# IBM/TM-GCN

Measured on AMD Instinct MI355X. Metric: TM-GCN layer fwd+bwd throughput (edges x T)/s, higher is better.
Workload: dtype f32

## Files before the change

include/tmgcn.h:

```cpp
#ifndef TMGCN_H
#define TMGCN_H

#include <stdint.h>

#ifdef __cplusplus
extern "C" {
#endif

typedef enum {
  TMGCN_OK = 0,
  TMGCN_ERR_INVALID = -1,
  TMGCN_ERR_LAUNCH = -2,
  TMGCN_ERR_WORKSPACE = -3
} tmgcn_status;

enum { TMGCN_ACT_NONE = 0, TMGCN_ACT_RELU = 1, TMGCN_ACT_LEAKY = 2, TMGCN_ACT_SELU = 3 };

int tmgcn_abi_version(void);
const char* tmgcn_last_error(void);
int tmgcn_pool_stats(int64_t* out, int32_t n);

enum {
  TMGCN_GEMM_AUTO = 0,
  TMGCN_GEMM_F32MFMA = 1
};

enum {
  TMGCN_DW_AUTO = 0,
  TMGCN_DW_F32MFMA = 1
};

int tmgcn_mtransform_f32(const float* M, int32_t Tm, int32_t ldm, int32_t transpose,
                         int32_t row_off, int32_t col_off, int32_t T_out, int32_t T_in,
                         int32_t band_lo, int32_t band_hi,
                         const float* X, float* Y, int64_t C,
                         int32_t x_group_rows, int32_t y_group_rows, void* stream);
int tmgcn_mtransform_ld_f32(const float* M, int32_t Tm, int32_t ldm, int32_t transpose,
                            int32_t row_off, int32_t col_off, int32_t T_out, int32_t T_in,
                            int32_t band_lo, int32_t band_hi,
                            const float* X, int64_t ldx, float* Y, int64_t ldy, int64_t C,
                            int32_t x_group_rows, int32_t y_group_rows, void* stream);

#define TMGCN_GIANT_ROW 32768
#define TMGCN_GIANT_CHUNK 4096
int64_t tmgcn_spmm_giant_workspace_bytes(int32_t n_giant_chunks, int32_t F);
int tmgcn_spmm_csr_batched_f32(const int64_t* rowptr, const int32_t* col, const float* val,
                               const float* X, float* Y, int64_t n_rows, int32_t N, int32_t F,
                               void* stream);
int tmgcn_spmm_csr_batched_f32_hint(const int64_t* rowptr, const int32_t* col, const float* val,
                                    const float* X, float* Y, int64_t n_rows, int32_t N,
                                    int32_t F, float avg_nnz_per_row, void* stream);
int tmgcn_spmm_csr_batched_f32_plan(const int64_t* rowptr, const int32_t* col, const float* val,
                                    const float* X, float* Y, int64_t n_rows, int32_t N,
                                    int32_t F, float avg_nnz_per_row, const int64_t* giant_rows,
                                    const int32_t* giant_chunks, int32_t n_giant, int32_t n_giant_chunks,
                                    float* giant_ws, int64_t giant_ws_bytes, void* stream);

int tmgcn_spmm_gemm_supported(int32_t K, int32_t Nf);
int tmgcn_spmm_gemm_f32(const int64_t* rowptr, const int32_t* col, const float* val,
                        const float* X, int64_t n_rows, int32_t N, int32_t K,
                        const float* W, int32_t Nf, int32_t trans_w,
                        int64_t rows_per_batch, int64_t w_batch_stride, int32_t act,
                        float* Y, float* AX, float* pre_act, int32_t grid_reserve, void* stream);
int tmgcn_spmm_gemm_f32_hint(const int64_t* rowptr, const int32_t* col, const float* val,
                             const float* X, int64_t n_rows, int32_t N, int32_t K,
                             const float* W, int32_t Nf, int32_t trans_w,
                             int64_t rows_per_batch, int64_t w_batch_stride, int32_t act,
                             float* Y, float* AX, float* pre_act, int32_t grid_reserve,
                             float avg_nnz_per_row, void* stream);
int tmgcn_spmm_gemm_f32_plan(const int64_t* rowptr, const int32_t* col, const float* val,
                             const float* X, int64_t n_rows, int32_t N, int32_t K,
                             const float* W, int32_t Nf, int32_t trans_w,
                             int64_t rows_per_batch, int64_t w_batch_stride, int32_t act,
                             float* Y, float* AX, float* pre_act, int32_t grid_reserve,
                             float avg_nnz_per_row, const int64_t* giant_rows, const int32_t* giant_chunks,
                             int32_t n_giant, int32_t n_giant_chunks, float* giant_ws, int64_t giant_ws_bytes,
                             void* stream);

int tmgcn_spmm_gemm_bf16_supported(int32_t K, int32_t Nf);
int tmgcn_spmm_gemm_bf16(const int64_t* rowptr, const int32_t* col, const float* val,
                         const uint16_t* X_bf16, int64_t n_rows, int32_t N, int32_t K,
                         const float* W, int32_t Nf, int32_t trans_w,
                         int64_t rows_per_batch, int64_t w_batch_stride, int32_t act,
                         void* Y, int32_t y_bf16, float* AX, float* pre_act, int32_t grid_reserve,
                         float avg_nnz_per_row, void* stream);

int tmgcn_gemm_f32(const float* A, const float* W, float* Y, float* pre_act,
                   int64_t R, int32_t K, int32_t Nf, int32_t trans_w,
                   int64_t rows_per_batch, int64_t w_batch_stride, int32_t act, int32_t algo, void* stream);

int tmgcn_gemm_bf16w_f32(const float* A, const uint16_t* W_bf16, float* Y, float* pre_act,
                         int64_t R, int32_t K, int32_t Nf, int32_t trans_w,
                         int64_t rows_per_batch, int64_t w_batch_stride, int32_t act, int32_t algo,
                         void* stream);

int64_t tmgcn_gemm_dw_workspace_bytes(int64_t R, int32_t K, int32_t Nf, int64_t rows_per_batch);
int tmgcn_gemm_dw_f32(const float* A, const float* dY, float* dW,
                      int64_t R, int32_t K, int32_t Nf, int64_t rows_per_batch, int32_t algo,
                      void* workspace, int64_t workspace_bytes, void* stream);
int tmgcn_gemm_dw_act_supported(int32_t K, int32_t Nf);
int tmgcn_gemm_dw_act_f32(const float* A, const float* dY, const float* pre_act, int32_t act, float* dW,
                          int64_t R, int32_t K, int32_t Nf, int64_t rows_per_batch,
                          void* workspace, int64_t workspace_bytes, void* stream);

#define TMGCN_L12_RUNS 16
int tmgcn_layer12_supported(int32_t K0, int32_t F, int32_t Nf);
int tmgcn_layer12_fwd_f32(const int64_t* rowptr, const int32_t* col, const float* val, const float* H,
                          const float* W1, int32_t act1, const float* W2, int32_t act2, int64_t n_rows,
                          int32_t N, int32_t K0, int32_t F, int32_t Nf, float* Z, float* AX, float* pre2,
                          float avg_nnz_per_row, const int64_t* row_blocks, int32_t n_row_blocks, void* stream);
int tmgcn_layer12_fwd_pays(int64_t n_rows, int32_t N, int32_t F, float avg_nnz_per_row);
int64_t tmgcn_layer12_bwd_workspace_bytes(int32_t K0, int32_t F, int32_t Nf, int64_t n_rows, int32_t n_row_blocks);
int tmgcn_layer12_bwd_forms_dw2(int64_t n_rows, int32_t N, int32_t F, int32_t Nf, float avg_nnz_per_row, int32_t n_row_blocks);
int tmgcn_layer12_bwd_f32(const int64_t* t_rowptr, const int32_t* t_col, const float* t_val, const float* dZ,
                          const float* pre2, const float* H, const float* W1, int32_t act1, const float* W2,
                          int32_t act2, int64_t n_rows, int32_t N, int32_t K0, int32_t F, int32_t Nf,
                          float* dW1, const float* AX, float* dW2, float avg_nnz_per_row, const int64_t* row_blocks,
                          int32_t n_row_blocks, void* workspace, int64_t workspace_bytes, void* stream);

int tmgcn_act_fwd_f32(const float* x, float* y, int64_t n, int32_t act, void* stream);
int tmgcn_act_bwd_f32(const float* x, const float* dy, float* dx, int64_t n, int32_t act,
                      void* stream);

int tmgcn_edge_head_supported(int32_t F, int32_t C);
int tmgcn_edge_head_fwd_f32(const float* Z, const int64_t* src, const int64_t* dst,
                            const float* U, float* out, int64_t E, int32_t F, int32_t C,
                            void* stream);
int64_t tmgcn_edge_head_bwd_workspace_bytes(int64_t E, int32_t F, int32_t C);
int tmgcn_edge_head_bwd_f32(const float* Z, const int64_t* src, const int64_t* dst,
                            const float* U, const float* dout,
                            const int64_t* eptr, const int64_t* eidx,
                            float* dZ, float* dU, int64_t R, int64_t E, int32_t F, int32_t C,
                            void* workspace, int64_t workspace_bytes, void* stream);
int tmgcn_edge_head_fwd_i32_f32(const float* Z, const int32_t* src, const int32_t* dst,
                                const float* U, float* out, int64_t E, int32_t F, int32_t C,
                                void* stream);
int tmgcn_edge_head_bwd_i32_f32(const float* Z, const int32_t* src, const int32_t* dst,
                                const float* U, const float* dout,
                                const int32_t* eptr, const int32_t* eidx,
                                float* dZ, float* dU, int64_t R, int64_t E, int32_t F, int32_t C,
                                void* workspace, int64_t workspace_bytes, void* stream);

int64_t tmgcn_wce_workspace_bytes(int64_t E);
int tmgcn_wce_fwd_f32(const float* logits, const int64_t* target, const float* weight, int64_t E,
                      int32_t C, int64_t ignore_index, float* loss_out, double* stats_out, void* workspace,
                      int64_t workspace_bytes, void* stream);
int tmgcn_wce_bwd_f32(const float* logits, const int64_t* target, const float* weight,
                      const double* stats, const float* grad_loss, int64_t E, int32_t C,
                      int64_t ignore_index, float* dlogits, void* stream);

#define TMGCN_SYNC_INTS 272
int tmgcn_head_loss_supported(int32_t F, int32_t C, int32_t K);
int tmgcn_head_loss_lanes(int64_t E, int64_t n_active);
int tmgcn_head_loss_combine_f32(const int32_t* srow, int32_t n_split, float* dZ, int64_t R, int32_t F, void* stream);
int64_t tmgcn_head_loss_workspace_bytes(int32_t F, int32_t C, int32_t K);
int tmgcn_head_loss_f32(const float* Z, const float* W_fold, int32_t K, const float* U,
                        const int32_t* eptr, const int32_t* arow, int64_t n_active, const int32_t* ent,
                        const int32_t* other, const uint8_t* meta, const int64_t* class_count,
                        const float* weight, const float* grad_scale, int64_t R, int64_t E, int32_t F,
                        int32_t C, float* logits, float* loss, float* dZ, float* dU, float* dW,
                        void* workspace, int64_t workspace_bytes, int32_t* sync, void* stream);
typedef struct TmgcnSgd {
  float* buf_U;
  float* buf_W;
  float lr, momentum, dampening, weight_decay;
  int32_t nesterov, maximize, first_step;
} TmgcnSgd;
int tmgcn_head_loss_sgd_f32(const float* Z, float* W_fold, int32_t K, float* U, const int32_t* eptr, const int32_t* arow,
                            int64_t n_active, const int32_t* other, const uint8_t* meta, const int64_t* class_count,
                            const float* weight, int64_t R, int64_t E, int32_t F, int32_t C, float* loss, float* dU,
                            float* dW, const TmgcnSgd* sgd, void* workspace, int64_t workspace_bytes, int32_t* sync,
                            void* stream);

int tmgcn_sgd_step(void* const* params, const void* const* grads, void* const* momentum_bufs, const int64_t* numel,
                   int32_t n, int32_t bf16, float lr, float momentum, float dampening, float weight_decay,
                   int32_t nesterov, int32_t maximize, int32_t first_step, void* stream);
int tmgcn_cast_multi(const void* const* src, void* const* dst, const int64_t* numel, int32_t n, int32_t to_bf16,
                     void* stream);
int tmgcn_scale2_f32(const float* g, const float* a, float* out_a, int64_t na, const float* b, float* out_b,
                     int64_t nb, void* stream);

int tmgcn_adj_make_keys(const int64_t* slice, const int64_t* row, const int64_t* col, int64_t n,
                        int64_t N, uint64_t* key, void* stream);
int64_t tmgcn_coo_sort_reduce_workspace_bytes(int64_t n);
int tmgcn_coo_sort_reduce(const uint64_t* keys_in, const float* vals_in, int64_t n, int32_t key_bits,
                          uint64_t* keys_out, float* vals_out, int64_t* n_out_dev,
                          void* workspace, int64_t workspace_bytes, void* stream);
int tmgcn_adj_symmetrise(const uint64_t* key, const float* val, int64_t n, int64_t N,
                         uint64_t* okey, float* oval, void* stream);
int tmgcn_adj_edge_life(const uint64_t* key, const float* val, int64_t n, int64_t N, int32_t T,
                        int32_t window, uint64_t* okey, float* oval, void* stream);
int tmgcn_adj_identity(int64_t TN, int64_t N, uint64_t* okey, float* oval, void* stream);
int tmgcn_adj_normalise(const uint64_t* key, float* val, int64_t n, int64_t N, int64_t TN,
                        int64_t* rowptr, float* dinv, void* stream);
int tmgcn_adj_mproduct_expand(const uint64_t* key, const float* val, int64_t n, int64_t N, int32_t T,
                              const float* M, int32_t ldm, int32_t band_lo, int32_t band_hi,
                              uint64_t* okey, float* oval, void* stream);
int tmgcn_adj_mproduct_merge_count(const int64_t* rowptr, const int32_t* col, int64_t TN, int32_t N, int32_t T,
                                   const float* M, int32_t ldm, int32_t band_lo, int32_t band_hi,
                                   int64_t* out_count, void* stream);
int tmgcn_adj_mproduct_merge_fill(const int64_t* rowptr, const int32_t* col, const float* val, int64_t TN,
                                  int32_t N, int32_t T, const float* M, int32_t ldm, int32_t band_lo,
                                  int32_t band_hi, const int64_t* out_rowptr, int32_t* out_col, float* out_val,
                                  void* stream);
int tmgcn_adj_keys_to_csr(const uint64_t* key, int64_t n, int64_t N, int64_t TN, int64_t* rowptr,
                          int32_t* col, void* stream);
int tmgcn_adj_transpose_keys(const int64_t* rowptr, const int32_t* col, int64_t TN, int64_t N,
                             uint64_t* okey, void* stream);

int tmgcn_wdgcn_supported(int32_t F0, int32_t H);
int64_t tmgcn_wdgcn_param_count(int32_t F0, int32_t H);
int tmgcn_wdgcn_fwd_f32(const float* AX, const float* P, const float* h0, const float* c0, float* Z, float* C,
                        int64_t N, int32_t T_run, int32_t F0, int32_t H, void* stream);
int64_t tmgcn_wdgcn_bwd_workspace_bytes(int64_t N, int32_t F0, int32_t H);
int tmgcn_wdgcn_bwd_f32(const float* AX, const float* P, const float* h0, const float* c0, const float* Z,
                        const float* C, const float* dZ, float* dP, int64_t N, int32_t T_run, int32_t F0,
                        int32_t H, void* workspace, int64_t workspace_bytes, void* stream);

int tmgcn_wdgcn_wide_supported(int32_t F0, int32_t H);
int64_t tmgcn_wdgcn_wide_saved_bytes(int64_t N, int32_t T_run, int32_t F0, int32_t H);
int tmgcn_wdgcn_wide_fwd_f32(const float* AX, const float* P, const float* h0, const float* c0, float* Z, void* saved,
                             int64_t N, int32_t T_run, int32_t F0, int32_t H, void* stream);
int64_t tmgcn_wdgcn_wide_bwd_workspace_bytes(int64_t N, int32_t T_run, int32_t F0, int32_t H);
int tmgcn_wdgcn_wide_bwd_f32(const float* AX, const float* P, const float* h0, const float* c0, const float* Z,
                             const void* saved, const float* dZ, float* dP, int64_t N, int32_t T_run, int32_t F0,
                             int32_t H, void* workspace, int64_t workspace_bytes, void* stream);

int tmgcn_egcn_supported(int32_t F, int32_t k);
int64_t tmgcn_egcn_param_count(int32_t F, int32_t k);
int64_t tmgcn_egcn_fwd_workspace_bytes(int64_t N, int32_t T_run, int32_t F, int32_t k);
// ... 27 lines not shown
```

tm-gcn_amd/_lib.py:

```python
import ctypes as C
import os

_HERE = os.path.dirname(os.path.abspath(__file__))
LIB_PATH = os.path.join(_HERE, "libtmgcn_hip.so")
HEADER_PATH = os.path.join(os.path.dirname(_HERE), "include", "tmgcn.h")

ACT_IDS = {None: 0, "none": 0, "relu": 1, "leaky": 2, "selu": 3}
DW_ALGOS = {None: 0, "auto": 0, "f32mfma": 1}
GEMM_ALGOS = {None: 0, "auto": 0, "f32mfma": 1}
ABI_VERSION = 5
SYNC_INTS = 272


class TmgcnLibraryError(RuntimeError):
    pass


_p = C.c_void_p
_i32 = C.c_int32
_i64 = C.c_int64

SIGNATURES = {
    "tmgcn_abi_version": (C.c_int, []),
    "tmgcn_last_error": (C.c_char_p, []),
    "tmgcn_pool_stats": (C.c_int, [_p, _i32]),
    "tmgcn_mtransform_f32": (C.c_int, [_p, _i32, _i32, _i32, _i32, _i32, _i32, _i32, _i32, _i32, _p, _p, _i64, _i32, _i32, _p]),
    "tmgcn_mtransform_ld_f32": (C.c_int, [_p, _i32, _i32, _i32, _i32, _i32, _i32, _i32, _i32, _i32, _p, _i64, _p, _i64, _i64, _i32, _i32, _p]),
    "tmgcn_spmm_csr_batched_f32": (C.c_int, [_p, _p, _p, _p, _p, _i64, _i32, _i32, _p]),
    "tmgcn_spmm_csr_batched_f32_hint": (C.c_int, [_p, _p, _p, _p, _p, _i64, _i32, _i32, C.c_float, _p]),
    "tmgcn_spmm_giant_workspace_bytes": (_i64, [_i32, _i32]),
    "tmgcn_spmm_csr_batched_f32_plan": (C.c_int, [_p, _p, _p, _p, _p, _i64, _i32, _i32, C.c_float, _p, _p, _i32, _i32, _p, _i64, _p]),
    "tmgcn_spmm_gemm_f32_plan": (C.c_int, [_p, _p, _p, _p, _i64, _i32, _i32, _p, _i32, _i32, _i64, _i64, _i32, _p, _p, _p, _i32, C.c_float,
                                           _p, _p, _i32, _i32, _p, _i64, _p]),
    "tmgcn_spmm_gemm_supported": (C.c_int, [_i32, _i32]),
    "tmgcn_spmm_gemm_f32": (C.c_int, [_p, _p, _p, _p, _i64, _i32, _i32, _p, _i32, _i32, _i64, _i64, _i32, _p, _p, _p, _i32, _p]),
    "tmgcn_spmm_gemm_f32_hint": (C.c_int, [_p, _p, _p, _p, _i64, _i32, _i32, _p, _i32, _i32, _i64, _i64, _i32, _p, _p, _p, _i32, C.c_float, _p]),
    "tmgcn_spmm_gemm_bf16_supported": (C.c_int, [_i32, _i32]),
    "tmgcn_spmm_gemm_bf16": (C.c_int, [_p, _p, _p, _p, _i64, _i32, _i32, _p, _i32, _i32, _i64, _i64, _i32, _p, _i32, _p, _p, _i32,
                                       C.c_float, _p]),
    "tmgcn_gemm_f32": (C.c_int, [_p, _p, _p, _p, _i64, _i32, _i32, _i32, _i64, _i64, _i32, _i32, _p]),
    "tmgcn_gemm_bf16w_f32": (C.c_int, [_p, _p, _p, _p, _i64, _i32, _i32, _i32, _i64, _i64, _i32, _i32, _p]),
    "tmgcn_gemm_dw_workspace_bytes": (_i64, [_i64, _i32, _i32, _i64]),
    "tmgcn_gemm_dw_f32": (C.c_int, [_p, _p, _p, _i64, _i32, _i32, _i64, _i32, _p, _i64, _p]),
    "tmgcn_gemm_dw_act_supported": (C.c_int, [_i32, _i32]),
    "tmgcn_gemm_dw_act_f32": (C.c_int, [_p, _p, _p, _i32, _p, _i64, _i32, _i32, _i64, _p, _i64, _p]),
    "tmgcn_layer12_supported": (C.c_int, [_i32, _i32, _i32]),
    "tmgcn_layer12_fwd_f32": (C.c_int, [_p, _p, _p, _p, _p, _i32, _p, _i32, _i64, _i32, _i32, _i32, _i32, _p, _p, _p, C.c_float, _p, _i32, _p]),
    "tmgcn_layer12_fwd_pays": (C.c_int, [_i64, _i32, _i32, C.c_float]),
    "tmgcn_layer12_bwd_workspace_bytes": (_i64, [_i32, _i32, _i32, _i64, _i32]),
    "tmgcn_layer12_bwd_forms_dw2": (C.c_int, [_i64, _i32, _i32, _i32, C.c_float, _i32]),
    "tmgcn_layer12_bwd_f32": (C.c_int, [_p, _p, _p, _p, _p, _p, _p, _i32, _p, _i32, _i64, _i32, _i32, _i32, _i32, _p, _p, _p, C.c_float, _p, _i32, _p, _i64, _p]),
    "tmgcn_edge_head_supported": (C.c_int, [_i32, _i32]),
    "tmgcn_edge_head_fwd_f32": (C.c_int, [_p, _p, _p, _p, _p, _i64, _i32, _i32, _p]),
    "tmgcn_edge_head_bwd_workspace_bytes": (_i64, [_i64, _i32, _i32]),
    "tmgcn_edge_head_bwd_f32": (C.c_int, [_p, _p, _p, _p, _p, _p, _p, _p, _p, _i64, _i64, _i32, _i32, _p, _i64, _p]),
    "tmgcn_edge_head_fwd_i32_f32": (C.c_int, [_p, _p, _p, _p, _p, _i64, _i32, _i32, _p]),
    "tmgcn_edge_head_bwd_i32_f32": (C.c_int, [_p, _p, _p, _p, _p, _p, _p, _p, _p, _i64, _i64, _i32, _i32, _p, _i64, _p]),
    "tmgcn_wce_workspace_bytes": (_i64, [_i64]),
    "tmgcn_wce_fwd_f32": (C.c_int, [_p, _p, _p, _i64, _i32, _i64, _p, _p, _p, _i64, _p]),
    "tmgcn_wce_bwd_f32": (C.c_int, [_p, _p, _p, _p, _p, _i64, _i32, _i64, _p, _p]),
    "tmgcn_head_loss_supported": (C.c_int, [_i32, _i32, _i32]),
    "tmgcn_head_loss_combine_f32": (C.c_int, [_p, _i32, _p, _i64, _i32, _p]),
    "tmgcn_head_loss_lanes": (C.c_int, [_i64, _i64]),
    "tmgcn_head_loss_workspace_bytes": (_i64, [_i32, _i32, _i32]),
    "tmgcn_head_loss_sgd_f32": (C.c_int, [_p, _p, _i32, _p, _p, _p, _i64, _p, _p, _p, _p, _i64, _i64, _i32, _i32, _p, _p, _p, _p, _p, _i64, _p, _p]),
    "tmgcn_head_loss_f32": (C.c_int, [_p, _p, _i32, _p, _p, _p, _i64, _p, _p, _p, _p, _p, _p, _i64, _i64, _i32, _i32, _p, _p, _p, _p, _p, _p, _i64, _p, _p]),
    "tmgcn_sgd_step": (C.c_int, [_p, _p, _p, _p, _i32, _i32, C.c_float, C.c_float, C.c_float, C.c_float, _i32, _i32, _i32, _p]),
    "tmgcn_cast_multi": (C.c_int, [_p, _p, _p, _i32, _i32, _p]),
    "tmgcn_scale2_f32": (C.c_int, [_p, _p, _p, _i64, _p, _p, _i64, _p]),
    "tmgcn_adj_make_keys": (C.c_int, [_p, _p, _p, _i64, _i64, _p, _p]),
    "tmgcn_coo_sort_reduce_workspace_bytes": (_i64, [_i64]),
    "tmgcn_coo_sort_reduce": (C.c_int, [_p, _p, _i64, _i32, _p, _p, _p, _p, _i64, _p]),
    "tmgcn_adj_symmetrise": (C.c_int, [_p, _p, _i64, _i64, _p, _p, _p]),
    "tmgcn_adj_edge_life": (C.c_int, [_p, _p, _i64, _i64, _i32, _i32, _p, _p, _p]),
    "tmgcn_adj_identity": (C.c_int, [_i64, _i64, _p, _p, _p]),
    "tmgcn_adj_normalise": (C.c_int, [_p, _p, _i64, _i64, _i64, _p, _p, _p]),
    "tmgcn_adj_mproduct_expand": (C.c_int, [_p, _p, _i64, _i64, _i32, _p, _i32, _i32, _i32, _p, _p, _p]),
    "tmgcn_adj_mproduct_merge_count": (C.c_int, [_p, _p, _i64, _i32, _i32, _p, _i32, _i32, _i32, _p, _p]),
    "tmgcn_adj_mproduct_merge_fill": (C.c_int, [_p, _p, _p, _i64, _i32, _i32, _p, _i32, _i32, _i32, _p, _p, _p, _p]),
    "tmgcn_adj_keys_to_csr": (C.c_int, [_p, _i64, _i64, _i64, _p, _p, _p]),
    "tmgcn_adj_transpose_keys": (C.c_int, [_p, _p, _i64, _i64, _p, _p]),
    "tmgcn_act_fwd_f32": (C.c_int, [_p, _p, _i64, _i32, _p]),
    "tmgcn_act_bwd_f32": (C.c_int, [_p, _p, _p, _i64, _i32, _p]),
    "tmgcn_wdgcn_supported": (C.c_int, [_i32, _i32]),
    "tmgcn_wdgcn_param_count": (_i64, [_i32, _i32]),
    "tmgcn_wdgcn_fwd_f32": (C.c_int, [_p, _p, _p, _p, _p, _p, _i64, _i32, _i32, _i32, _p]),
    "tmgcn_wdgcn_bwd_workspace_bytes": (_i64, [_i64, _i32, _i32]),
    "tmgcn_wdgcn_bwd_f32": (C.c_int, [_p, _p, _p, _p, _p, _p, _p, _p, _i64, _i32, _i32, _i32, _p, _i64, _p]),
    "tmgcn_wdgcn_wide_supported": (C.c_int, [_i32, _i32]),
    "tmgcn_wdgcn_wide_saved_bytes": (_i64, [_i64, _i32, _i32, _i32]),
    "tmgcn_wdgcn_wide_fwd_f32": (C.c_int, [_p, _p, _p, _p, _p, _p, _i64, _i32, _i32, _i32, _p]),
    "tmgcn_wdgcn_wide_bwd_workspace_bytes": (_i64, [_i64, _i32, _i32, _i32]),
    "tmgcn_wdgcn_wide_bwd_f32": (C.c_int, [_p, _p, _p, _p, _p, _p, _p, _p, _i64, _i32, _i32, _i32, _p, _i64, _p]),
    "tmgcn_egcn_supported": (C.c_int, [_i32, _i32]),
    "tmgcn_egcn_param_count": (_i64, [_i32, _i32]),
    "tmgcn_egcn_fwd_workspace_bytes": (_i64, [_i64, _i32, _i32, _i32]),
    "tmgcn_egcn_fwd": (C.c_int, [_p, _p, _p, _p, _p, _p, _p, _p, _i32, _p, _p, _p, _p, _p, _p, _p, _i64, _i32, _i32, _i32,
                                 _p, _i64, _p]),
    "tmgcn_egcn_bwd_workspace_bytes": (_i64, [_i32, _i32, _i32]),
    "tmgcn_egcn_bwd": (C.c_int, [_p, _p, _p, _p, _p, _p, _p, _p, _p, _p, _p, _p, _i64, _i32, _i32, _i32, _p, _i64, _p]),
    "tmgcn_egcn_wide_supported": (C.c_int, [_i32, _i32]),
    "tmgcn_egcn_wide_fwd_workspace_bytes": (_i64, [_i64, _i32, _i32, _i32]),
    "tmgcn_egcn_wide_fwd": (C.c_int, [_p, _p, _p, _p, _p, _p, _p, _p, _i32, _p, _p, _p, _p, _p, _p, _p, _i64, _i32, _i32,
                                      _i32, _p, _i64, _p]),
    "tmgcn_egcn_wide_bwd_workspace_bytes": (_i64, [_i32, _i32, _i32]),
    "tmgcn_egcn_wide_bwd": (C.c_int, [_p, _p, _p, _p, _p, _p, _p, _p, _p, _p, _p, _p, _i64, _i32, _i32, _i32, _p, _i64,
                                      _p]),
}

_lib = None


def load():
    global _lib
    if _lib is not None:
        return _lib
    if not os.path.exists(LIB_PATH):
        raise TmgcnLibraryError(
            f"{LIB_PATH} not found: build the HIP library first "
            "(make -C tm-gcn_amd/csrc, or __graft_entry__.build()). "
            "There is no CPU fallback for the TM-GCN layer."
        )
    try:
        lib = C.CDLL(LIB_PATH)
    except OSError as e:
        raise TmgcnLibraryError(f"cannot load {LIB_PATH}: {e}") from e
    for name, (res, args) in SIGNATURES.items():
        try:
            fn = getattr(lib, name)
        except AttributeError as e:
            raise TmgcnLibraryError(f"{LIB_PATH} does not export {name}") from e
        fn.restype = res
        fn.argtypes = args
    _lib = lib
    return lib


TORCH_LIB_PATH = os.path.join(_HERE, "libtmgcn_torch.so")
_torch_ops = None


def load_torch_ops():
    global _torch_ops
    if _torch_ops is not None:
        return _torch_ops
    load()
    if not os.path.exists(TORCH_LIB_PATH):
        raise TmgcnLibraryError(
            f"{TORCH_LIB_PATH} not found: build the torch extension layer first "
            "(make -C tm-gcn_amd/csrc torch, or __graft_entry__.build()).")
    import torch
    try:
        torch.ops.load_library(TORCH_LIB_PATH)
    except OSError as e:
        raise TmgcnLibraryError(f"cannot load {TORCH_LIB_PATH}: {e}") from e
    ops = torch.ops.tmgcn
    if int(ops.abi_version()) != ABI_VERSION:
        raise TmgcnLibraryError(f"{TORCH_LIB_PATH} was built against ABI {int(ops.abi_version())}, expected {ABI_VERSION}")
    _torch_ops = ops
    return ops


def check(rc, what):
    if rc != 0:
        msg = load().tmgcn_last_error().decode("utf-8", "replace")
        raise RuntimeError(f"{what} failed (status {rc}): {msg}")
```

tm-gcn_amd/csrc/common.h:

```cpp
#pragma once
#include <hip/hip_runtime.h>
#include <stdint.h>
#include <stdio.h>
#include <type_traits>
#include "tmgcn.h"

namespace tmgcn {

void set_error(const char* fmt, ...);

inline int check_launch(const char* what) {
  hipError_t e = hipGetLastError();
  if (e != hipSuccess) {
    set_error("%s: %s", what, hipGetErrorString(e));
    return TMGCN_ERR_LAUNCH;
  }
  return TMGCN_OK;
}

const char* pool_error();
unsigned int* acquire_tile_counters(hipStream_t stream, int n);
inline unsigned int* acquire_tile_counter(hipStream_t stream) { return acquire_tile_counters(stream, 1); }

int32_t* acquire_sync_word(hipStream_t stream);

constexpr int kSyncGroups = 16, kSyncStride = 16;
constexpr int kSyncInts = (1 + kSyncGroups) * kSyncStride;
static_assert(kSyncInts == TMGCN_SYNC_INTS, "include/tmgcn.h states the size of a hand-off block");
__device__ __forceinline__ bool last_block_ticket(int32_t* sync, int n_blocks, int* lds_flag) {
  asm volatile("s_waitcnt vmcnt(0)" ::: "memory");
  __syncthreads();
  if (threadIdx.x == 0) {
    const int g = blockIdx.x % kSyncGroups;
    const int members = (n_blocks - g + kSyncGroups - 1) / kSyncGroups;
    int32_t* mine = sync + (1 + g) * kSyncStride;
    bool last = false;
    if (__hip_atomic_fetch_add(mine, 1, __ATOMIC_RELAXED, __HIP_MEMORY_SCOPE_AGENT) == members - 1) {
      __hip_atomic_store(mine, 0, __ATOMIC_RELAXED, __HIP_MEMORY_SCOPE_AGENT);
      const int groups = n_blocks < kSyncGroups ? n_blocks : kSyncGroups;
      last = __hip_atomic_fetch_add(sync, 1, __ATOMIC_RELAXED, __HIP_MEMORY_SCOPE_AGENT) == groups - 1;
    }
    *lds_flag = last;
  }
  __syncthreads();
  return *lds_flag != 0;
}

int launch_giant_partial(const char* who, const int64_t* rowptr, const int32_t* col, const float* val, const float* X, int32_t N,
                         int32_t F, const int64_t* giant_rows, const int32_t* giant_chunks, int32_t n_giant, int32_t n_giant_chunks,
                         float* ws, int64_t ws_bytes, hipStream_t st);

#define TMGCN_REQUIRE(cond, ...)            \
  do {                                      \
    if (!(cond)) {                          \
      ::tmgcn::set_error(__VA_ARGS__);      \
      return TMGCN_ERR_INVALID;             \
    }                                       \
  } while (0)

constexpr int kWave = 64;


inline int device_cu_count(int dev) {
  thread_local int cus[16] = {0};
  if (dev >= 0 && dev < 16 && cus[dev]) return cus[dev];
  int n = 0;
  if (hipDeviceGetAttribute(&n, hipDeviceAttributeMultiprocessorCount, dev) != hipSuccess || n <= 0) n = 256;
  if (dev >= 0 && dev < 16) cus[dev] = n;
  return n;
}

template <typename K>
inline int persistent_grid(K kernel, int block_threads, size_t dyn_smem = 0, int max_per_cu = 4) {
  struct Entry { const void* k; int dev, threads, blocks_per_cu; };
  constexpr int kSlots = 16;
  thread_local Entry table[kSlots] = {};
  thread_local int next = 0;
  const void* key = reinterpret_cast<const void*>(kernel);
  int dev = 0;
  if (hipGetDevice(&dev) != hipSuccess) dev = 0;
  const int cus = device_cu_count(dev);
  if (dyn_smem == 0)
    for (int i = 0; i < kSlots; ++i)
      if (table[i].k == key && table[i].dev == dev && table[i].threads == block_threads)
        return cus * table[i].blocks_per_cu;
  int per_cu = 1;
  if (hipOccupancyMaxActiveBlocksPerMultiprocessor(&per_cu, kernel, block_threads, dyn_smem) != hipSuccess ||
      per_cu < 1)
    per_cu = 1;
  if (per_cu > max_per_cu) per_cu = max_per_cu;
  (void)hipGetLastError();
  if (dyn_smem == 0) {
    table[next] = Entry{key, dev, block_threads, per_cu};
    next = (next + 1) % kSlots;
  }
  return cus * per_cu;
}

template <typename K>
inline int persistent_grid_reserved(K kernel, int block_threads, int reserve, size_t dyn_smem = 0) {
  int g = persistent_grid(kernel, block_threads, dyn_smem) - reserve;
  return g < 64 ? 64 : g;
}

inline int check_workspace(const char* who, const void* workspace, int64_t bytes, int64_t need) {
  if (workspace && bytes >= need) return TMGCN_OK;
  set_error("%s: workspace of %lld bytes, %lld needed", who, (long long)bytes, (long long)need);
  return TMGCN_ERR_WORKSPACE;
}

template <typename K>
inline int allow_large_lds(K kernel, size_t bytes, const char* what) {
  if (bytes <= 64 * 1024) return TMGCN_OK;
  struct Entry { const void* k; int dev; size_t bytes; };
  constexpr int kSlots = 32;
  thread_local Entry table[kSlots] = {};
  thread_local int next = 0;
  const void* key = reinterpret_cast<const void*>(kernel);
  int dev = 0;
  if (hipGetDevice(&dev) != hipSuccess) dev = 0;
  Entry* e = nullptr;
  for (int i = 0; i < kSlots && !e; ++i)
    if (table[i].k == key && table[i].dev == dev) e = &table[i];
  if (e && e->bytes >= bytes) return TMGCN_OK;
  if (hipFuncSetAttribute(key, hipFuncAttributeMaxDynamicSharedMemorySize, (int)bytes) != hipSuccess) {
    (void)hipGetLastError();
    set_error("%s: %zu bytes of LDS per block refused", what, bytes);
    return TMGCN_ERR_LAUNCH;
  }
  if (!e) {
    e = &table[next];
    next = (next + 1) % kSlots;
  }
  *e = Entry{key, dev, bytes};
  return TMGCN_OK;
}

__device__ __forceinline__ void quad_transpose4(float (&v)[4], int j) {
  const bool odd = j & 1, hi = j & 2;
  {
    const float s0 = odd ? v[0] : v[1], s1 = odd ? v[2] : v[3];
    const float r0 = __builtin_bit_cast(float, __builtin_amdgcn_mov_dpp(__builtin_bit_cast(int, s0), 0xB1, 0xF, 0xF, true));
    const float r1 = __builtin_bit_cast(float, __builtin_amdgcn_mov_dpp(__builtin_bit_cast(int, s1), 0xB1, 0xF, 0xF, true));
    if (odd) {
      v[0] = r0;
      v[2] = r1;
    } else {
      v[1] = r0;
      v[3] = r1;
    }
  }
  {
    const float s0 = hi ? v[0] : v[2], s1 = hi ? v[1] : v[3];
    const float r0 = __builtin_bit_cast(float, __builtin_amdgcn_mov_dpp(__builtin_bit_cast(int, s0), 0x4E, 0xF, 0xF, true));
    const float r1 = __builtin_bit_cast(float, __builtin_amdgcn_mov_dpp(__builtin_bit_cast(int, s1), 0x4E, 0xF, 0xF, true));
    if (hi) {
      v[0] = r0;
      v[1] = r1;
    } else {
      v[2] = r0;
      v[3] = r1;
    }
  }
}

__device__ __forceinline__ int64_t readlane64(int64_t v, int l) {
  const unsigned lo = (unsigned)__builtin_amdgcn_readlane((int)(unsigned)(v & 0xffffffff), l);
  const int hi = __builtin_amdgcn_readlane((int)(v >> 32), l);
  return ((int64_t)hi << 32) | lo;
}

template <int N, typename T>
__device__ __forceinline__ T pick(const T (&v)[N], int i) {
  T r = v[0];
#pragma unroll
  for (int q = 1; q < N; ++q) r = (i == q) ? v[q] : r;
  return r;
}

template <int CTRL>
__device__ __forceinline__ float dpp_lane_f32(float v) {
  return __builtin_bit_cast(float, __builtin_amdgcn_mov_dpp(__builtin_bit_cast(int, v), CTRL, 0xF, 0xF, true));
}
__device__ __forceinline__ float wave_sum_f32(float v) {
  v += dpp_lane_f32<0xB1>(v);
  v += dpp_lane_f32<0x4E>(v);
  v += dpp_lane_f32<0x141>(v);
  v += dpp_lane_f32<0x140>(v);
  const float r0 = __builtin_bit_cast(float, __builtin_amdgcn_readlane(__builtin_bit_cast(int, v), 0));
  const float r1 = __builtin_bit_cast(float, __builtin_amdgcn_readlane(__builtin_bit_cast(int, v), 16));
  const float r2 = __builtin_bit_cast(float, __builtin_amdgcn_readlane(__builtin_bit_cast(int, v), 32));
  const float r3 = __builtin_bit_cast(float, __builtin_amdgcn_readlane(__builtin_bit_cast(int, v), 48));
  return ((r0 + r1) + r2) + r3;
}

template <int CTRL>
__device__ __forceinline__ double dpp_add_f64(double x) {
  const long long b = __builtin_bit_cast(long long, x);
  const int lo = __builtin_amdgcn_mov_dpp((int)b, CTRL, 0xF, 0xF, true);
// ... 214 lines not shown
```

tm-gcn_amd/csrc/gemm.hip:

```cpp
#include <type_traits>
#include "common.h"
#include "async_stage.h"

namespace tmgcn {

typedef float f32x16 __attribute__((ext_vector_type(16)));
typedef float f32x4 __attribute__((ext_vector_type(4)));

constexpr int BM = 64;
constexpr int KC = 128;
constexpr int LDA = KC + 4;

struct GemmArgs {
  const float* A;
  const float* W;
  float* Y;
  float* pre;
  int64_t R;
  int32_t K, Nf;
  int32_t trans_w;
  int64_t rows_per_batch;
  int64_t w_batch_stride;
  int32_t act;
  int64_t tiles_per_batch;
// ... 1104 lines not shown
  const bool x3 = algo == TMGCN_GEMM_AUTO && K % 4 == 0 && K >= 16 && K <= 128 &&
                  reinterpret_cast<uintptr_t>(A) % 16 == 0;
  const bool x3_chunked = algo == TMGCN_GEMM_AUTO && K % 4 == 0 && K > 128 && K <= 512 &&
                          reinterpret_cast<uintptr_t>(A) % 16 == 0;
  if (x3_chunked) {
    int64_t gx = w_bf16 ? persistent_grid(gemm_bf16x3_kernel<1, true>, 256) : persistent_grid(gemm_bf16x3_kernel<3, true>, 256);
    if (gx > a.n_tiles) gx = a.n_tiles;
    for (int k0 = 0; k0 < K; k0 += 128) {
      GemmArgs c = a;
      const bool last = k0 + 128 >= K;
      c.K = last ? K - k0 : 128;
      c.lda = K;
      c.k0 = k0;
      c.accum = k0 > 0;
      c.act = last ? act : TMGCN_ACT_NONE;
      c.pre = last ? pre_act : nullptr;
      if (w_bf16)
        hipLaunchKernelGGL((gemm_bf16x3_kernel<1, true>), dim3((unsigned)gx, gy), dim3(256), 0, st, c);
      else
        hipLaunchKernelGGL((gemm_bf16x3_kernel<3, true>), dim3((unsigned)gx, gy), dim3(256), 0, st, c);
    }
    return check_launch("gemm_bf16x3 (k-chunks)");
  }
  if (x3) {
    int64_t gx = w_bf16 ? persistent_grid(gemm_bf16x3_kernel<1>, 256) : persistent_grid(gemm_bf16x3_kernel<3>, 256);
    if (gx > a.n_tiles) gx = a.n_tiles;
    if (w_bf16)
      hipLaunchKernelGGL(gemm_bf16x3_kernel<1>, dim3((unsigned)gx, gy), dim3(256), 0, st, a);
    else
      hipLaunchKernelGGL(gemm_bf16x3_kernel<3>, dim3((unsigned)gx, gy), dim3(256), 0, st, a);
    return check_launch("gemm_bf16x3");
  }
  a.tile_counter = acquire_tile_counters(st, (int)gy);
  TMGCN_REQUIRE(a.tile_counter, "gemm: no tile counters: %s", pool_error());
  int64_t gx = persistent_grid(gemm_mfma_kernel, 256);
  if (gx > a.n_tiles) gx = a.n_tiles;
  hipLaunchKernelGGL(gemm_mfma_kernel, dim3((unsigned)gx, gy), dim3(256), 0, st, a);
  return check_launch("gemm_mfma");
}

extern "C" int tmgcn_gemm_f32(const float* A, const float* W, float* Y, float* pre_act, int64_t R,
                               int32_t K, int32_t Nf, int32_t trans_w, int64_t rows_per_batch,
                               int64_t w_batch_stride, int32_t act, int32_t algo, void* stream) {
  return gemm_launch(A, W, false, Y, pre_act, R, K, Nf, trans_w, rows_per_batch, w_batch_stride, act, algo, stream);
}

extern "C" int tmgcn_gemm_bf16w_f32(const float* A, const uint16_t* W_bf16, float* Y, float* pre_act, int64_t R,
                                     int32_t K, int32_t Nf, int32_t trans_w, int64_t rows_per_batch,
                                     int64_t w_batch_stride, int32_t act, int32_t algo, void* stream) {
  return gemm_launch(A, W_bf16, true, Y, pre_act, R, K, Nf, trans_w, rows_per_batch, w_batch_stride, act, algo,
                     stream);
}

extern "C" int64_t tmgcn_gemm_dw_workspace_bytes(int64_t R, int32_t K, int32_t Nf,
                                                  int64_t rows_per_batch) {
  if (R <= 0 || K <= 0 || Nf <= 0) return 0;
  int64_t nb, rpc;
  int chunks;
  dw_plan(R, rows_per_batch, &nb, &chunks, &rpc);
  return (nb * chunks + kSyncGroups) * (int64_t)K * Nf * (int64_t)sizeof(float);
}

static int gemm_dw_launch(const float* A, const float* dY, const float* pre, int32_t act, float* dW, int64_t R, int32_t K,
                          int32_t Nf, int64_t rows_per_batch, int32_t algo, void* workspace, int64_t workspace_bytes,
                          void* stream) {
  TMGCN_REQUIRE(R >= 0 && K > 0 && Nf > 0, "gemm_dw: bad shape");
  TMGCN_REQUIRE(algo == TMGCN_DW_AUTO || algo == TMGCN_DW_F32MFMA, "gemm_dw: unknown algo %d", algo);
  TMGCN_REQUIRE(rows_per_batch >= 0, "gemm_dw: negative rows_per_batch");
  TMGCN_REQUIRE(dW, "gemm_dw: null dW");
  hipStream_t st = (hipStream_t)stream;
  int64_t nb, rpc;
  int chunks;
  dw_plan(R, rows_per_batch, &nb, &chunks, &rpc);
  if (R == 0) {
    (void)hipMemsetAsync(dW, 0, (size_t)K * Nf * sizeof(float), st);
    return check_launch("gemm_dw memset");
  }
  TMGCN_REQUIRE(A && dY, "gemm_dw: null pointer");
  const int64_t need = (nb * chunks + kSyncGroups) * (int64_t)K * Nf * (int64_t)sizeof(float);
  if (!workspace || workspace_bytes < need) {
    set_error("gemm_dw: workspace %lld B < required %lld B", (long long)workspace_bytes,
              (long long)need);
    return TMGCN_ERR_WORKSPACE;
  }
  const bool narrow = K % 2 == 0 && Nf % 2 == 0 && K <= 8 && Nf <= 8 && reinterpret_cast<uintptr_t>(A) % 8 == 0 &&
                      reinterpret_cast<uintptr_t>(dY) % 8 == 0;
  TMGCN_REQUIRE(!pre || narrow, "gemm_dw_act: the fused activation gradient needs the narrow kernel (even K, Nf <= 8, 8-byte "
                                 "aligned operands); use tmgcn_act_bwd_f32 + tmgcn_gemm_dw_f32");
  if (narrow) {
    const int64_t br = rows_per_batch ? rows_per_batch : R;
    int64_t target = (R < (4ll << 20) ? 512 : 1024) / nb;
    if (target < 1) target = 1;
    int64_t fat = (br + target - 1) / target;
    fat = (fat + 31) & ~(int64_t)31;
    if (fat < 256) fat = 256;
    if (fat > rpc) {
      rpc = fat;
      chunks = (int)((br + rpc - 1) / rpc);
    }
  }
  DwArgs a{A, dY, (float*)workspace, R, K, Nf, rows_per_batch ? rows_per_batch : R, chunks, rpc};
  const unsigned gx = (unsigned)(nb * chunks);
  if (narrow) {
    a.dW = dW;
    a.pre = pre;
    a.act = act;
    a.n_batch = (int32_t)nb;
    a.sync = acquire_sync_word(st);
    TMGCN_REQUIRE(a.sync, "gemm_dw: no hand-off block: %s", pool_error());
#define TMGCN_DWN_L(KT_, NT_)                                                                          \
  if (pre) hipLaunchKernelGGL((gemm_dw_narrow_kernel<KT_, NT_, true>), dim3(gx), dim3(256), 0, st, a); \
  else hipLaunchKernelGGL((gemm_dw_narrow_kernel<KT_, NT_, false>), dim3(gx), dim3(256), 0, st, a);
#define TMGCN_DWN_N(KT_)                \
  switch (Nf) {                         \
    case 2: TMGCN_DWN_L(KT_, 2) break;  \
    case 4: TMGCN_DWN_L(KT_, 4) break;  \
    case 6: TMGCN_DWN_L(KT_, 6) break;  \
    default: TMGCN_DWN_L(KT_, 8)        \
  }
    switch (K) {
      case 2: TMGCN_DWN_N(2) break;
      case 4: TMGCN_DWN_N(4) break;
      case 6: TMGCN_DWN_N(6) break;
      default: TMGCN_DWN_N(8)
    }
#undef TMGCN_DWN_N
#undef TMGCN_DWN_L
    return check_launch("gemm_dw_narrow");
  } else if (use_small(K, Nf)) {
    const size_t smem = (size_t)DW_ROWS * (K + Nf) * sizeof(float);
    hipLaunchKernelGGL(gemm_dw_small_kernel, dim3(gx), dim3(256), smem, st, a);
  } else {
    const unsigned gy = (unsigned)(((K + 127) / 128) * ((Nf + 127) / 128));
    const bool x3 = algo == TMGCN_DW_AUTO && K % 4 == 0 && Nf % 4 == 0 &&
                    reinterpret_cast<uintptr_t>(A) % 16 == 0 && reinterpret_cast<uintptr_t>(dY) % 16 == 0;
    if (x3)
      hipLaunchKernelGGL(gemm_dw_bf16x3_kernel, dim3(gx, gy), dim3(256), 0, st, a);
    else
      hipLaunchKernelGGL(gemm_dw_lds_kernel, dim3(gx, gy), dim3(256), 0, st, a);
  }
  int rc = check_launch("gemm_dw");
  if (rc) return rc;
  const int64_t n_out = (int64_t)K * Nf;
  const int64_t total = nb * n_out;
  if (total <= 1024 && chunks >= 64)
    hipLaunchKernelGGL(gemm_dw_reduce_narrow_kernel, dim3((unsigned)total), dim3(256), 0, st, (const float*)workspace,
                       dW, n_out, chunks);
  else
    hipLaunchKernelGGL(gemm_dw_reduce_kernel, dim3((unsigned)((total + 63) / 64)), dim3(DWR_WAVES * 64), 0, st,
                       (const float*)workspace, dW, n_out, chunks, total);
  return check_launch("gemm_dw_reduce");
}

extern "C" int tmgcn_gemm_dw_f32(const float* A, const float* dY, float* dW, int64_t R, int32_t K, int32_t Nf,
                                  int64_t rows_per_batch, int32_t algo, void* workspace, int64_t workspace_bytes,
                                  void* stream) {
  return gemm_dw_launch(A, dY, nullptr, TMGCN_ACT_NONE, dW, R, K, Nf, rows_per_batch, algo, workspace, workspace_bytes, stream);
}

extern "C" int tmgcn_gemm_dw_act_supported(int32_t K, int32_t Nf) {
  return (K >= 2 && Nf >= 2 && K % 2 == 0 && Nf % 2 == 0 && K <= 8 && Nf <= 8) ? 1 : 0;
}

extern "C" int tmgcn_gemm_dw_act_f32(const float* A, const float* dY, const float* pre_act, int32_t act, float* dW,
                                      int64_t R, int32_t K, int32_t Nf, int64_t rows_per_batch, void* workspace,
                                      int64_t workspace_bytes, void* stream) {
  TMGCN_REQUIRE(tmgcn_gemm_dw_act_supported(K, Nf), "gemm_dw_act: even K, Nf <= 8 only (got %d x %d)", K, Nf);
  TMGCN_REQUIRE(act >= TMGCN_ACT_NONE && act <= TMGCN_ACT_SELU, "gemm_dw_act: unknown activation %d", act);
  TMGCN_REQUIRE(pre_act && reinterpret_cast<uintptr_t>(pre_act) % 8 == 0, "gemm_dw_act: pre_act must be given, 8-byte aligned");
  return gemm_dw_launch(A, dY, pre_act, act, dW, R, K, Nf, rows_per_batch, TMGCN_DW_AUTO, workspace, workspace_bytes, stream);
}
```

tm-gcn_amd/csrc/spmm_gemm.hip:

```cpp
#include "common.h"
#include "spmm_row.h"
#include "spmm_gemm_tile.h"

namespace tmgcn {

#ifndef TMGCN_FUSED_US
#define TMGCN_FUSED_US 1
#endif
#ifndef TMGCN_BX3_US
#define TMGCN_BX3_US 4
#endif
#ifndef TMGCN_BX3_MAX_DEG
#define TMGCN_BX3_MAX_DEG 14
#endif

struct FusedArgs {
  const int64_t* rowptr;
  const int32_t* col;
  const float* val;
  const float4* X;
  int64_t n_rows;
  int32_t N;
  int32_t K;
  const float* W;
  int32_t Nf;
  int32_t trans_w;
  int64_t rows_per_batch;
  int64_t w_batch_stride;
  float* Y;
  float* AX;
  float* pre;
  int32_t act;
  TileMap tiles;
  int64_t n_tiles;
  unsigned int* tile_counter;
  GiantPlan giant;
};

#ifdef TMGCN_FUSED_TRACE
__device__ unsigned long long fused_trace_words[4096 * 16];
#define FT_WORDS fused_trace_words
#else
#define FT_WORDS nullptr
#endif

template <int LPR, int U, int NJ, int US = TMGCN_FUSED_US * U>
__global__ __launch_bounds__(256, TMGCN_FUSED_OCC) void spmm_gemm_kernel(FusedArgs a) {
  __shared__ float As[FBM * FLDA];
  __shared__ float4 s_part[4 * LPR];
  __shared__ unsigned int s_tile, s_row;
  fused_tile_loop<FusedF32, LPR, U, NJ, US, false>(a, As, s_part, &s_tile, &s_row, FT_WORDS);
}


typedef __bf16 bx_bf16x8 __attribute__((ext_vector_type(8)));
typedef __bf16 bx_bf16x2 __attribute__((ext_vector_type(2)));
typedef float bx_f32x2 __attribute__((ext_vector_type(2)));
typedef float bx_f32x4 __attribute__((ext_vector_type(4)));
constexpr int BX_PITCH = 272;
constexpr int BX_PLANE = FBM * BX_PITCH;
constexpr int BX_YPITCH = 132;

__device__ __forceinline__ unsigned bx_pack(float a, float b) {
  bx_f32x2 v = {a, b};
  return __builtin_bit_cast(unsigned, __builtin_convertvector(v, bx_bf16x2));
}
__device__ __forceinline__ void bx_split3(float a, float b, unsigned& h, unsigned& m, unsigned& l) {
  h = bx_pack(a, b);
  a -= __uint_as_float(h << 16);
  b -= __uint_as_float(h & 0xffff0000u);
  m = bx_pack(a, b);
  a -= __uint_as_float(m << 16);
  b -= __uint_as_float(m & 0xffff0000u);
  l = bx_pack(a, b);
}

template <int LPR, int U, int NKS, int US>
__global__ __launch_bounds__(512, 4) void spmm_gemm_bx3_kernel(FusedArgs a) {
  __shared__ __attribute__((aligned(16))) unsigned char sm[3 * BX_PLANE];
  __shared__ float4 s_part[4 * LPR];
  __shared__ unsigned int s_tile, s_row;
  const int lane0 = threadIdx.x & 63;
  const int wave = __builtin_amdgcn_readfirstlane(threadIdx.x >> 6);
  const int n0 = wave * 16;
  const int F4 = a.K / 4;
  const TileMap tm = a.tiles;
  unsigned bw[NKS][3][4];
  int64_t cur_batch = -1;
  if (threadIdx.x == 0) s_row = 8;
  const bool staged = a.Nf % 4 == 0 && reinterpret_cast<uintptr_t>(a.Y) % 16 == 0 && reinterpret_cast<uintptr_t>(a.pre) % 16 == 0;
  HeavyScan heavy;
  heavy.init(a.rowptr, tm);
  bool have_next = false;
  for (;;) {
    int lane = lane0;
    asm volatile("" : "+v"(lane));
    int64_t tile = -1;
    if (heavy.scanning) tile = heavy.next(a.rowptr, tm, a.tile_counter + 1, &s_tile, lane);
    const bool scanning = heavy.scanning;
    if (!scanning) {
      if (!have_next) {
        if (threadIdx.x == 0) s_tile = atomicAdd(a.tile_counter, 1u);
        __syncthreads();
      }
      tile = s_tile;
      have_next = false;
      if (tile >= a.n_tiles) break;
    }
    int64_t unit, row0, row_end;
    tile_extent(tm, tile, unit, row0, row_end);
    const int64_t batch = a.rows_per_batch ? row0 / a.rows_per_batch : 0;
    TileRows rows;
    rows.load(a.rowptr, row0, row_end, lane);
    if (!scanning && rows.entries > heavy.thr) {
      __syncthreads();
      continue;
    }
    const int n_tile_rows = row_end - row0 < FBM ? (int)(row_end - row0) : FBM;
    const int64_t slice0 = row0 / a.N;
    const float4* Xs = a.X + slice0 * (int64_t)a.N * F4;
    auto flush = [&](int rr, const float4& acc, int fl) __attribute__((always_inline)) {
      if (fl < F4) {
        unsigned h0, m0, l0, h1, m1, l1;
        bx_split3(acc.x, acc.y, h0, m0, l0);
        bx_split3(acc.z, acc.w, h1, m1, l1);
        unsigned char* w = sm + rr * BX_PITCH + fl * 8;
        *reinterpret_cast<uint2*>(w) = make_uint2(h0, h1);
        *reinterpret_cast<uint2*>(w + BX_PLANE) = make_uint2(m0, m1);
        *reinterpret_cast<uint2*>(w + 2 * BX_PLANE) = make_uint2(l0, l1);
        if (a.AX && rr < n_tile_rows) store_f4(&reinterpret_cast<float4*>(a.AX)[(row0 + rr) * F4 + fl], acc);
      }
    };
    if (short_tile(rows, row0 + n_tile_rows <= (slice0 + 1) * a.N)) {
      gather_short_tile<LPR, US, 8>(a.col, a.val, Xs, rows, n_tile_rows, F4, lane, wave, F4, flush);
    } else {
      for (int rr = wave; rr < FBM;) {
        unsigned int nxt = 0;
        if (lane == 0) nxt = atomicAdd(&s_row, 1u);
        const bool lng = (rows.long_mask >> rr) & 1;
        if (!lng) {
          float4 acc = make_float4(0.f, 0.f, 0.f, 0.f);
          if (rr < n_tile_rows) acc = gather_row<LPR, U>(a.col, a.val, Xs, readlane64(rows.beg, rr), readlane64(rows.end, rr), F4, lane);
          if (lane < LPR) flush(rr, acc, lane);
        }
        rr = (int)__builtin_amdgcn_readfirstlane(nxt);
      }
      for (uint64_t m = rows.long_mask; m; m &= m - 1) {
        const int rr = __builtin_ctzll(m);
        const int64_t beg = readlane64(rows.beg, rr), end = readlane64(rows.end, rr);
        if (wave < 4) {
          const float4 acc = gather_long_row<LPR, U>(a.col, a.val, Xs, beg, end, F4, lane, wave, s_part);
          if (wave == (rr & 3) && lane < LPR) flush(rr, acc, lane);
        } else {
          __syncthreads();
          __syncthreads();
        }
      }
    }
    if (batch != cur_batch) {
      const float* Wb = a.W + (a.rows_per_batch ? batch * a.w_batch_stride : 0);
      const int n = n0 + (lane & 15);
      const int nc = n < a.Nf ? n : 0;
      const float zn = n < a.Nf ? 1.f : 0.f;
      const int64_t sk = a.trans_w ? 1 : a.Nf, sn = a.trans_w ? a.K : 1;
      const float* Wl = Wb + (int64_t)nc * sn + (int64_t)(8 * (lane >> 4)) * sk;
#pragma unroll
      for (int ks = 0; ks < NKS; ++ks)
#pragma unroll
        for (int j = 0; j < 4; ++j) {
          const float w0 = Wl[(int64_t)(32 * ks + 2 * j) * sk] * zn;
          const float w1 = Wl[(int64_t)(32 * ks + 2 * j + 1) * sk] * zn;
          bx_split3(w0, w1, bw[ks][0][j], bw[ks][1][j], bw[ks][2][j]);
        }
      cur_batch = batch;
    }
    __syncthreads();
    if (threadIdx.x == 0) s_row = 8;
    unsigned int drawn = 0;
    if (!scanning && threadIdx.x == 0) drawn = atomicAdd(a.tile_counter, 1u);
    __builtin_amdgcn_s_setprio(TMGCN_FUSED_MFMA_PRIO);
    int lane_p = lane0;
    asm volatile("" : "+v"(lane_p));
    const int lm = lane_p & 15, lg = lane_p >> 4;
    bx_f32x4 acc[4];
#pragma unroll
    for (int rb = 0; rb < 4; ++rb) acc[rb] = bx_f32x4{0.f, 0.f, 0.f, 0.f};
    if (n0 < a.Nf) {
      const unsigned char* rd = sm + lm * BX_PITCH + lg * 16;
#pragma unroll
      for (int ks = 0; ks < NKS; ++ks) {
        const bx_bf16x8 bh = __builtin_bit_cast(bx_bf16x8, make_uint4(bw[ks][0][0], bw[ks][0][1], bw[ks][0][2], bw[ks][0][3]));
        const bx_bf16x8 bm = __builtin_bit_cast(bx_bf16x8, make_uint4(bw[ks][1][0], bw[ks][1][1], bw[ks][1][2], bw[ks][1][3]));
        const bx_bf16x8 bl = __builtin_bit_cast(bx_bf16x8, make_uint4(bw[ks][2][0], bw[ks][2][1], bw[ks][2][2], bw[ks][2][3]));
#pragma unroll
        for (int rb = 0; rb < 4; ++rb) {
          const unsigned char* p = rd + rb * 16 * BX_PITCH + ks * 64;
          const bx_bf16x8 ah = __builtin_bit_cast(bx_bf16x8, *reinterpret_cast<const uint4*>(p));
          const bx_bf16x8 am = __builtin_bit_cast(bx_bf16x8, *reinterpret_cast<const uint4*>(p + BX_PLANE));
          const bx_bf16x8 al = __builtin_bit_cast(bx_bf16x8, *reinterpret_cast<const uint4*>(p + 2 * BX_PLANE));
          bx_f32x4 c = acc[rb];
          c = __builtin_amdgcn_mfma_f32_16x16x32_bf16(al, bh, c, 0, 0, 0);
          c = __builtin_amdgcn_mfma_f32_16x16x32_bf16(ah, bl, c, 0, 0, 0);
          c = __builtin_amdgcn_mfma_f32_16x16x32_bf16(am, bm, c, 0, 0, 0);
          c = __builtin_amdgcn_mfma_f32_16x16x32_bf16(am, bh, c, 0, 0, 0);
          c = __builtin_amdgcn_mfma_f32_16x16x32_bf16(ah, bm, c, 0, 0, 0);
          c = __builtin_amdgcn_mfma_f32_16x16x32_bf16(ah, bh, c, 0, 0, 0);
          acc[rb] = c;
        }
      }
    }
    __builtin_amdgcn_s_setprio(0);
    if (!staged) {
      const int n = n0 + lm;
      if (n < a.Nf) {
        const ActApply act(a.act);
#pragma unroll
        for (int rb = 0; rb < 4; ++rb)
#pragma unroll
          for (int i = 0; i < 4; ++i) {
            const int rr = 16 * rb + 4 * lg + i;
            if (rr < n_tile_rows) {
              const float v = acc[rb][i];
              const int64_t o = (row0 + rr) * a.Nf + n;
              if (a.pre) store_f1(&a.pre[o], v);
              store_f1(&a.Y[o], a.act == TMGCN_ACT_NONE ? v : act(v));
            }
          }
      }
    } else {
      __syncthreads();
      float* yt = reinterpret_cast<float*>(sm);
      if (n0 < a.Nf) {
#pragma unroll
        for (int rb = 0; rb < 4; ++rb)
#pragma unroll
          for (int i = 0; i < 4; ++i) yt[(16 * rb + 4 * lg + i) * BX_YPITCH + n0 + lm] = acc[rb][i];
      }
      __syncthreads();
      int lane_s = lane0;
      asm volatile("" : "+v"(lane_s));
      const int c4 = lane_s & 31;
      if (4 * c4 < a.Nf) {
        const ActApply act(a.act);
        float* __restrict__ Yb = a.Y + row0 * a.Nf;
        float* __restrict__ Pb = a.pre ? a.pre + row0 * a.Nf : nullptr;
#pragma unroll
        for (int k = 0; k < FBM / 16; ++k) {
          const int rr = 16 * k + 2 * wave + (lane_s >> 5);
          if (rr < n_tile_rows) {
            float4 v = *reinterpret_cast<const float4*>(&yt[rr * BX_YPITCH + 4 * c4]);
            if (Pb) store_f4(reinterpret_cast<float4*>(&Pb[rr * a.Nf + 4 * c4]), v);
            if (a.act != TMGCN_ACT_NONE) v = make_float4(act(v.x), act(v.y), act(v.z), act(v.w));
            store_f4(reinterpret_cast<float4*>(&Yb[rr * a.Nf + 4 * c4]), v);
          }
        }
      }
    }
    if (!scanning) {
      if (threadIdx.x == 0) s_tile = drawn;
      have_next = true;
    }
    __syncthreads();
  }
}

template <int F, int G>
__global__ __launch_bounds__(256) void spmm_gemm_small_kernel(FusedArgs a) {
  const int64_t gid = (int64_t)blockIdx.x * blockDim.x + threadIdx.x;
  const int64_t r = gid / G;
  const int gl = (int)(gid % G);
  const bool live = r < a.n_rows;
  const float* X = reinterpret_cast<const float*>(a.X);
  const ActApply act(a.act);
  float acc[F];
#pragma unroll
  for (int f = 0; f < F; ++f) acc[f] = 0.f;
  int64_t beg = 0, end = 0;
  if (live) {
    beg = a.rowptr[r];
    end = a.rowptr[r + 1];
  }
  const bool is_long = G < kWave && end - beg > (int64_t)kNarrowLong * G;
  if (live && !is_long) {
    const int64_t xoff = (r / a.N) * (int64_t)a.N;
    for (int64_t p = beg + gl; p < end; p += G) {
      const float* x = X + (xoff + a.col[p]) * F;
      const float v = a.val[p];
#pragma unroll
      for (int f = 0; f < F; ++f) acc[f] = fmaf(v, x[f], acc[f]);
    }
  }
#pragma unroll
  for (int o = G >> 1; o > 0; o >>= 1)
#pragma unroll
    for (int f = 0; f < F; ++f) acc[f] += __shfl_xor(acc[f], o);
  auto epilogue = [&](int64_t row, int first, int lanes) {
    if (a.AX && first == 0) {
#pragma unroll
      for (int f = 0; f < F; ++f) a.AX[row * F + f] = acc[f];
    }
    const float* Wb = a.W + (a.rows_per_batch ? (row / a.rows_per_batch) * a.w_batch_stride : 0);
    for (int n = first; n < a.Nf; n += lanes) {
      float s = 0.f;
#pragma unroll
      for (int f = 0; f < F; ++f) s = fmaf(acc[f], a.trans_w ? Wb[(int64_t)n * F + f] : Wb[(int64_t)f * a.Nf + n], s);
      if (a.pre) a.pre[row * a.Nf + n] = s;
      a.Y[row * a.Nf + n] = act(s);
    }
  };
  if (live && !is_long) epilogue(r, gl, G);
  if constexpr (G < kWave) {
    const int lane = threadIdx.x & 63;
    for (uint64_t m = __ballot(is_long && gl == 0); m; m &= m - 1) {
      const int src = __builtin_ctzll(m);
      const int64_t r2 = readlane64(r, src), b2 = readlane64(beg, src), e2 = readlane64(end, src);
      narrow_wave_row<F>(acc, a.col, a.val, X, (r2 / a.N) * (int64_t)a.N, b2, e2, lane);
      epilogue(r2, lane, kWave);
    }
  }
}

template <int F>
static int launch_fused_small(const FusedArgs& a, int G, hipStream_t st) {
  const unsigned grid = (unsigned)((a.n_rows * G + 255) / 256);
  switch (G) {
    case 1: hipLaunchKernelGGL((spmm_gemm_small_kernel<F, 1>), dim3(grid), dim3(256), 0, st, a); break;
    case 2: hipLaunchKernelGGL((spmm_gemm_small_kernel<F, 2>), dim3(grid), dim3(256), 0, st, a); break;
    case 4: hipLaunchKernelGGL((spmm_gemm_small_kernel<F, 4>), dim3(grid), dim3(256), 0, st, a); break;
    case 8: hipLaunchKernelGGL((spmm_gemm_small_kernel<F, 8>), dim3(grid), dim3(256), 0, st, a); break;
    case 16: hipLaunchKernelGGL((spmm_gemm_small_kernel<F, 16>), dim3(grid), dim3(256), 0, st, a); break;
    case 32: hipLaunchKernelGGL((spmm_gemm_small_kernel<F, 32>), dim3(grid), dim3(256), 0, st, a); break;
    default: hipLaunchKernelGGL((spmm_gemm_small_kernel<F, 64>), dim3(grid), dim3(256), 0, st, a);
  }
  return check_launch("spmm_gemm_small");
}

static bool fused_small_ok(int K, int Nf) {
  return (K == 1 || K == 2 || K == 3 || K == 4 || K == 6 || K == 8) && Nf >= 1 && Nf <= 16;
}

}

using namespace tmgcn;

extern "C" int tmgcn_spmm_gemm_supported(int32_t K, int32_t Nf) {
  return ((K % 8 == 0 && K >= 16 && K <= FKC && Nf >= 1 && Nf <= 128) || fused_small_ok(K, Nf)) ? 1 : 0;
}

extern "C" int tmgcn_spmm_gemm_f32_plan(const int64_t* rowptr, const int32_t* col, const float* val,
                                         const float* X, int64_t n_rows, int32_t N, int32_t K,
                                         const float* W, int32_t Nf, int32_t trans_w,
                                         int64_t rows_per_batch, int64_t w_batch_stride, int32_t act,
                                         float* Y, float* AX, float* pre_act, int32_t grid_reserve,
                                         float avg_nnz_per_row, const int64_t* giant_rows, const int32_t* giant_chunks,
                                         int32_t n_giant, int32_t n_giant_chunks, float* giant_ws, int64_t giant_ws_bytes,
                                         void* stream) {
  const int bad = fused_check_args("spmm_gemm", grid_reserve, n_rows, N, K, Nf, tmgcn_spmm_gemm_supported(K, Nf),
                                   "(need K a multiple of 8 in [16,128] with Nf <= 128, or K in {1,2,3,4,6,8} with Nf <= 16); "
                                   "use tmgcn_spmm_csr_batched_f32 + tmgcn_gemm_f32", act, 0, rows_per_batch);
  if (bad) return bad;
  if (n_rows == 0) return TMGCN_OK;
  TMGCN_REQUIRE(rowptr && X && W && Y, "spmm_gemm: null pointer");
  TMGCN_REQUIRE(n_rows % N == 0, "spmm_gemm: n_rows=%lld is not a multiple of N=%d", (long long)n_rows, N);
  if (fused_small_ok(K, Nf)) {
    FusedArgs s{rowptr, col, val, reinterpret_cast<const float4*>(X), n_rows, N, K, W, Nf, trans_w,
                rows_per_batch, w_batch_stride, Y, AX, pre_act, act, TileMap{0, 0, 0, 0}, 0, nullptr, GiantPlan{nullptr, nullptr, nullptr, 0}};
    int G = 8;
    if (avg_nnz_per_row >= 0.f) {
      G = 1;
      while (G < 64 && (float)(2 * G) <= avg_nnz_per_row) G <<= 1;
    }
    hipStream_t st2 = (hipStream_t)stream;
    switch (K) {
      case 1: return launch_fused_small<1>(s, G, st2);
      case 2: return launch_fused_small<2>(s, G, st2);
      case 3: return launch_fused_small<3>(s, G, st2);
      case 4: return launch_fused_small<4>(s, G, st2);
      case 6: return launch_fused_small<6>(s, G, st2);
      default: return launch_fused_small<8>(s, G, st2);
    }
  }
  TMGCN_REQUIRE(reinterpret_cast<uintptr_t>(X) % 16 == 0 && (!AX || reinterpret_cast<uintptr_t>(AX) % 16 == 0),
                "spmm_gemm: X / AX must be 16-byte aligned");
  FusedArgs a{rowptr, col, val, reinterpret_cast<const float4*>(X), n_rows, N, K, W, Nf, trans_w,
              rows_per_batch, w_batch_stride, Y, AX, pre_act, act, TileMap{0, 0, 0, 0}, 0, nullptr, GiantPlan{nullptr, nullptr, nullptr, 0}};
  if (n_giant > 0) {
    const int rc = launch_giant_partial("spmm_gemm (giant rows)", rowptr, col, val, X, N, K, giant_rows, giant_chunks, n_giant,
                                        n_giant_chunks, giant_ws, giant_ws_bytes, (hipStream_t)stream);
    if (rc != TMGCN_OK) return rc;
    a.giant = GiantPlan{giant_rows, giant_chunks, reinterpret_cast<const float4*>(giant_ws), n_giant};
  }
  hipStream_t st = (hipStream_t)stream;
  const int no_tiles = fused_plan_tiles("spmm_gemm", a, st);
  if (no_tiles) return no_tiles;
  if (avg_nnz_per_row >= 0.f && avg_nnz_per_row < (float)TMGCN_BX3_MAX_DEG && n_giant == 0 && (K == 128 || K == 64)) {
    if (K == 128) {
      int64_t gx = persistent_grid(spmm_gemm_bx3_kernel<32, TMGCN_FUSED_U, 4, TMGCN_BX3_US>, 512, 0, 2) - grid_reserve / 2;
      if (gx < 64) gx = 64;
      if (gx > a.n_tiles) gx = a.n_tiles;
      hipLaunchKernelGGL((spmm_gemm_bx3_kernel<32, TMGCN_FUSED_U, 4, TMGCN_BX3_US>), dim3((unsigned)gx), dim3(512), 0, st, a);
    } else {
      int64_t gx = persistent_grid(spmm_gemm_bx3_kernel<16, TMGCN_FUSED_U, 2, TMGCN_BX3_US>, 512, 0, 2) - grid_reserve / 2;
      if (gx < 64) gx = 64;
      if (gx > a.n_tiles) gx = a.n_tiles;
      hipLaunchKernelGGL((spmm_gemm_bx3_kernel<16, TMGCN_FUSED_U, 2, TMGCN_BX3_US>), dim3((unsigned)gx), dim3(512), 0, st, a);
    }
    return check_launch("spmm_gemm (bf16-split products)");
  }
#define TMGCN_FUSED_CASE(KK, L, UU)                                                              \
  case KK: {                                                                                     \
    int64_t gx = persistent_grid_reserved(spmm_gemm_kernel<L, UU, KK / 8>, 256, grid_reserve);                 \
    if (gx > a.n_tiles) gx = a.n_tiles;                                                          \
    hipLaunchKernelGGL((spmm_gemm_kernel<L, UU, KK / 8>), dim3((unsigned)gx), dim3(256), 0, st, a); \
    break;                                                                                       \
  }
  switch (K) {
    TMGCN_FUSED_CASE(16, 4, 2)
    TMGCN_FUSED_CASE(24, 8, 2)
    TMGCN_FUSED_CASE(32, 8, 2)
    TMGCN_FUSED_CASE(40, 16, TMGCN_FUSED_U)
    TMGCN_FUSED_CASE(48, 16, TMGCN_FUSED_U)
    TMGCN_FUSED_CASE(56, 16, TMGCN_FUSED_U)
    TMGCN_FUSED_CASE(64, 16, TMGCN_FUSED_U)
    TMGCN_FUSED_CASE(72, 32, TMGCN_FUSED_U)
    TMGCN_FUSED_CASE(80, 32, TMGCN_FUSED_U)
    TMGCN_FUSED_CASE(88, 32, TMGCN_FUSED_U)
    TMGCN_FUSED_CASE(96, 32, TMGCN_FUSED_U)
    TMGCN_FUSED_CASE(104, 32, TMGCN_FUSED_U)
    TMGCN_FUSED_CASE(112, 32, TMGCN_FUSED_U)
    TMGCN_FUSED_CASE(120, 32, TMGCN_FUSED_U)
    TMGCN_FUSED_CASE(128, 32, TMGCN_FUSED_U)
  }
#undef TMGCN_FUSED_CASE
  return check_launch("spmm_gemm");
}

extern "C" int tmgcn_spmm_gemm_f32_hint(const int64_t* rowptr, const int32_t* col, const float* val,
                                         const float* X, int64_t n_rows, int32_t N, int32_t K,
                                         const float* W, int32_t Nf, int32_t trans_w,
                                         int64_t rows_per_batch, int64_t w_batch_stride, int32_t act,
                                         float* Y, float* AX, float* pre_act, int32_t grid_reserve,
                                         float avg_nnz_per_row, void* stream) {
  return tmgcn_spmm_gemm_f32_plan(rowptr, col, val, X, n_rows, N, K, W, Nf, trans_w, rows_per_batch, w_batch_stride, act, Y, AX,
                                  pre_act, grid_reserve, avg_nnz_per_row, nullptr, nullptr, 0, 0, nullptr, 0, stream);
}

extern "C" int tmgcn_spmm_gemm_f32(const int64_t* rowptr, const int32_t* col, const float* val,
                                    const float* X, int64_t n_rows, int32_t N, int32_t K,
                                    const float* W, int32_t Nf, int32_t trans_w,
                                    int64_t rows_per_batch, int64_t w_batch_stride, int32_t act,
                                    float* Y, float* AX, float* pre_act, int32_t grid_reserve,
                                    void* stream) {
  return tmgcn_spmm_gemm_f32_hint(rowptr, col, val, X, n_rows, N, K, W, Nf, trans_w, rows_per_batch, w_batch_stride,
                                  act, Y, AX, pre_act, grid_reserve, -1.f, stream);
}

#ifdef TMGCN_FUSED_TRACE
extern "C" int tmgcn_debug_fused_trace(unsigned long long* dst, long n_words, int clear) {
  void* p = nullptr;
  hipError_t e = hipGetSymbolAddress(&p, HIP_SYMBOL(tmgcn::fused_trace_words));
  if (e == hipSuccess && n_words > 0) e = hipMemcpy(dst, p, (size_t)n_words * 8, hipMemcpyDeviceToHost);
  if (e == hipSuccess && clear) e = hipMemset(p, 0, sizeof(unsigned long long) * 4096 * 16);
  return (int)e;
}
#endif
```

tm-gcn_amd/csrc/spmm_gemm_tile.h:

```cpp
#pragma once
#include "common.h"
#include "spmm_row.h"

namespace tmgcn {

typedef float f32x16 __attribute__((ext_vector_type(16)));

#ifndef TMGCN_FUSED_OCC
#define TMGCN_FUSED_OCC 4
#endif
#ifndef TMGCN_FUSED_U
#define TMGCN_FUSED_U 4
#endif
#ifndef TMGCN_FUSED_MFMA_PRIO
#define TMGCN_FUSED_MFMA_PRIO 3
#endif

constexpr int FBM = 64;
constexpr int FKC = 128;
constexpr int FLDA = FKC + 4;

__device__ __forceinline__ void store_y(float* p, float v) { store_f1(p, v); }
__device__ __forceinline__ void store_y(uint16_t* p, float v) {
  __builtin_nontemporal_store(__builtin_bit_cast(uint16_t, (__bf16)v), p);
}

template <int NJ, class Args>
__device__ __forceinline__ void fused_load_w(const Args& a, int64_t batch, int n0, int li, int lh, float (&wreg)[NJ][4]) {
  const float* Wb = a.W + (a.rows_per_batch ? batch * a.w_batch_stride : 0);
  const int n = n0 + li;
  const int nc = n < a.Nf ? n : 0;
  const float* Wl = a.trans_w ? Wb + (int64_t)nc * a.K + 4 * lh : Wb + (int64_t)(4 * lh) * a.Nf + nc;
  const int64_t sk = a.trans_w ? 1 : a.Nf;
#pragma unroll
  for (int j = 0; j < NJ; ++j)
#pragma unroll
    for (int s = 0; s < 4; ++s) {
      const float w = Wl[(int64_t)(8 * j + s) * sk];
      wreg[j][s] = n < a.Nf ? w : 0.f;
    }
}

template <bool GUARD, bool PRE, bool ACT, class YT>
__device__ __forceinline__ void fused_store_half(const f32x16& acc, const ActApply& act, YT* __restrict__ Yb, float* __restrict__ Pb,
                                                 int Nf, int lane_off, int rows_left) {
#pragma unroll
  for (int i = 0; i < 16; ++i) {
    const int k = (i & 3) + 8 * (i >> 2);
    const float s = acc[i];
    if (GUARD && k >= rows_left) continue;
    if (PRE) store_f1(&Pb[k * Nf + lane_off], s);
    store_y(&Yb[k * Nf + lane_off], ACT ? act(s) : s);
  }
}
template <bool GUARD, class YT>
__device__ __forceinline__ void fused_store_half(const f32x16& acc, int act_id, YT* __restrict__ Yb, float* __restrict__ Pb, int Nf,
                                                 int lane_off, int rows_left) {
  const ActApply act(act_id);
  if (act_id == TMGCN_ACT_NONE) {
    if (Pb) fused_store_half<GUARD, true, false>(acc, act, Yb, Pb, Nf, lane_off, rows_left);
    else fused_store_half<GUARD, false, false>(acc, act, Yb, Pb, Nf, lane_off, rows_left);
  } else {
    if (Pb) fused_store_half<GUARD, true, true>(acc, act, Yb, Pb, Nf, lane_off, rows_left);
    else fused_store_half<GUARD, false, true>(acc, act, Yb, Pb, Nf, lane_off, rows_left);
  }
}
template <int NJ, class Args>
__device__ __forceinline__ void fused_mfma_tile(const Args& a, const float* As, const float (&wreg)[NJ][4], int64_t row0,
                                                int64_t row_end, int n0, int li, int lh) {
  if (n0 >= a.Nf) return;
  const float* Arow = &As[li * FLDA + 4 * lh];
  const int n = n0 + li;
#pragma unroll
  for (int mb = 0; mb < FBM / 32; ++mb) {
    f32x16 acc;
#pragma unroll
    for (int i = 0; i < 16; ++i) acc[i] = 0.f;
    float4 av_next = *reinterpret_cast<const float4*>(Arow + mb * 32 * FLDA);
#pragma unroll
    for (int j = 0; j < NJ; ++j) {
      const float4 av = av_next;
      if (j + 1 < NJ) av_next = *reinterpret_cast<const float4*>(Arow + mb * 32 * FLDA + 8 * (j + 1));
      acc = __builtin_amdgcn_mfma_f32_32x32x2f32(av.x, wreg[j][0], acc, 0, 0, 0);
      acc = __builtin_amdgcn_mfma_f32_32x32x2f32(av.y, wreg[j][1], acc, 0, 0, 0);
      acc = __builtin_amdgcn_mfma_f32_32x32x2f32(av.z, wreg[j][2], acc, 0, 0, 0);
      acc = __builtin_amdgcn_mfma_f32_32x32x2f32(av.w, wreg[j][3], acc, 0, 0, 0);
      __builtin_amdgcn_sched_barrier(0);
    }
    if (n < a.Nf) {
      const int64_t rbase = row0 + mb * 32;
      if constexpr (std::is_same<decltype(a.Y), float*>::value) {
        float* __restrict__ Yb = a.Y + rbase * a.Nf;
        float* __restrict__ Pb = a.pre ? a.pre + rbase * a.Nf : nullptr;
        const int lane_off = (4 * lh) * a.Nf + n;
        if (rbase + 32 <= row_end) fused_store_half<false>(acc, a.act, Yb, Pb, a.Nf, lane_off, 32);
        else fused_store_half<true>(acc, a.act, Yb, Pb, a.Nf, lane_off, (int)(row_end - rbase) - 4 * lh);
      } else {
        float* __restrict__ Pb = a.pre ? a.pre + rbase * a.Nf : nullptr;
        const int lane_off = (4 * lh) * a.Nf + n;
        const int rows_left = rbase + 32 <= row_end ? 32 : (int)(row_end - rbase) - 4 * lh;
        if (a.y_bf16) fused_store_half<true>(acc, a.act, static_cast<uint16_t*>(a.Y) + rbase * a.Nf, Pb, a.Nf, lane_off, rows_left);
        else fused_store_half<true>(acc, a.act, static_cast<float*>(a.Y) + rbase * a.Nf, Pb, a.Nf, lane_off, rows_left);
      }
    }
  }
}

struct FusedF32 {
  using Piece = PieceF32;
  static constexpr bool kShortTiles = true, kGiantPlan = true;
};
struct FusedBf16 {
  using Piece = PieceBf16;
  static constexpr bool kShortTiles = false, kGiantPlan = false;
};

#ifdef TMGCN_FUSED_TRACE
#define FT_NOW() wall_clock64()
#define FT_WAIT() asm volatile("s_waitcnt vmcnt(0) lgkmcnt(0)" ::: "memory")
#define FT_STAMP(name) const unsigned long long name = FT_NOW()
#else
#define FT_STAMP(name) do { } while (0)
#define FT_WAIT() do { } while (0)
#endif

template <class Pol, int LPR, int U, int US, bool OFF32, class Args>
__device__ __forceinline__ void fused_gather_tile(const Args& a, float* As, typename Pol::Piece::Sum* s_part, const TileRows& rows,
                                                  int64_t row0, int64_t row_end, int lane, int wave, unsigned int* s_row) {
  using P = typename Pol::Piece;
  using Sum = typename P::Sum;
  constexpr int Q = P::kFloats / 4;
  const int F = a.K / P::kFloats;
  auto flush = [&](int rr, int64_t r, const Sum& acc, int fl, bool to_ax) __attribute__((always_inline)) {
    float4* d = reinterpret_cast<float4*>(&As[rr * FLDA + P::kFloats * fl]);
#pragma unroll
    for (int j = 0; j < Q; ++j) d[j] = P::quad(acc, j);
    if (to_ax) {
      float4* ax = &reinterpret_cast<float4*>(a.AX)[r * (Q * F) + Q * fl];
#pragma unroll
      for (int j = 0; j < Q; ++j) store_f4(ax + j, P::quad(acc, j));
    }
  };
  if constexpr (Pol::kShortTiles) {
    const int n_tile_rows = row_end - row0 < FBM ? (int)(row_end - row0) : FBM;
    const int64_t slice0 = row0 / a.N;
    const bool is_short = short_tile(rows, row0 + n_tile_rows <= (slice0 + 1) * a.N);
    if (is_short) {
      gather_short_tile<LPR, US>(a.col, a.val, a.X + slice0 * (int64_t)a.N * F, rows, n_tile_rows, F, lane, wave, F,
                                 [&](int rr, const float4& acc, int fl) {
                                   if (fl < F) {
                                     *reinterpret_cast<float4*>(&As[rr * FLDA + 4 * fl]) = acc;
                                     if (a.AX) store_f4(&reinterpret_cast<float4*>(a.AX)[(row0 + rr) * F + fl], acc);
                                   }
                                 });
      return;
    }
  }
  for (int rr = wave; rr < FBM;) {
    unsigned int nxt = 0;
    if (lane == 0) nxt = atomicAdd(s_row, 1u);
    const int64_t r = row0 + rr;
    const bool lng = (rows.long_mask >> rr) & 1;
    Sum acc = P::zero();
    if (r < row_end && !lng) {
      const int64_t slice = r / a.N;
      acc = gather_row<LPR, U, P, OFF32>(a.col, a.val, a.X + slice * (int64_t)a.N * F, readlane64(rows.beg, rr),
                                         readlane64(rows.end, rr), F, lane);
    }
    if (!lng && lane < LPR && lane < F) flush(rr, r, acc, lane, a.AX && r < row_end);
    rr = (int)__builtin_amdgcn_readfirstlane(nxt);
  }
  for (uint64_t m = rows.long_mask; m; m &= m - 1) {
    const int rr = __builtin_ctzll(m);
    const int64_t r = row0 + rr;
    const int64_t slice = r / a.N;
    const int64_t beg = readlane64(rows.beg, rr), end = readlane64(rows.end, rr);
    Sum acc;
    int gi = -1;
    if constexpr (Pol::kGiantPlan) gi = (a.giant.rows && end - beg > kGiantRow) ? giant_find(a.giant, r) : -1;
    if (gi >= 0) {
      if (wave != (rr & 3)) continue;
      if constexpr (Pol::kGiantPlan) acc = giant_row_sum(a.giant, gi, F, lane, 0, F);
    } else {
      acc = gather_long_row<LPR, U, P, OFF32>(a.col, a.val, a.X + slice * (int64_t)a.N * F, beg, end, F, lane, wave, s_part);
    }
    if (wave == (rr & 3) && lane < LPR && lane < F) flush(rr, r, acc, lane, a.AX != nullptr);
  }
}

template <class Pol, int LPR, int U, int NJ, int US, bool OFF32, class Args>
__device__ __forceinline__ void fused_tile_loop(const Args a, float* As, typename Pol::Piece::Sum* s_part, unsigned int* s_tile,
                                                unsigned int* s_row, unsigned long long* trace_words = nullptr) {
  const int lane0 = threadIdx.x & 63;
  const int wave = __builtin_amdgcn_readfirstlane(threadIdx.x >> 6);
  const int n0 = wave * 32;
  const TileMap tm = a.tiles;

  float wreg[NJ][4];
  int64_t cur_batch = -1;
  if (threadIdx.x == 0) *s_row = 4;
  HeavyScan heavy;
  heavy.init(a.rowptr, tm);

#ifdef TMGCN_FUSED_TRACE
  unsigned long long ft[16] = {0};
#endif
  for (;;) {
    int lane = lane0;
    asm volatile("" : "+v"(lane));
    FT_STAMP(ft_a);
    int64_t tile = -1;
    if (heavy.scanning) tile = heavy.next(a.rowptr, tm, a.tile_counter + 1, s_tile, lane);
    const bool scanning = heavy.scanning;
    if (!scanning) {
      if (threadIdx.x == 0) *s_tile = atomicAdd(a.tile_counter, 1u);
      __syncthreads();
      tile = *s_tile;
      if (tile >= a.n_tiles) break;
    }
    int64_t unit, row0, row_end;
    tile_extent(tm, tile, unit, row0, row_end);
    const int64_t batch = a.rows_per_batch ? row0 / a.rows_per_batch : 0;
    FT_STAMP(ft_b);
    TileRows rows;
    rows.load(a.rowptr, row0, row_end, lane);
    if (!scanning && rows.entries > heavy.thr) {
      __syncthreads();
      continue;
    }
    FT_WAIT();
    FT_STAMP(ft_c);
    if (batch != cur_batch) {
      fused_load_w<NJ>(a, batch, n0, lane & 31, lane >> 5, wreg);
      cur_batch = batch;
    }
    fused_gather_tile<Pol, LPR, U, US, OFF32>(a, As, s_part, rows, row0, row_end, lane, wave, s_row);
    FT_WAIT();
    FT_STAMP(ft_d);
    __syncthreads();
    if (threadIdx.x == 0) *s_row = 4;
    FT_STAMP(ft_e);
    __builtin_amdgcn_s_setprio(TMGCN_FUSED_MFMA_PRIO);
    {
      int lane_p = lane0;
      asm volatile("" : "+v"(lane_p));
      fused_mfma_tile<NJ>(a, As, wreg, row0, row_end, n0, lane_p & 31, lane_p >> 5);
    }
    __builtin_amdgcn_s_setprio(0);
    FT_STAMP(ft_f);
    __syncthreads();
#ifdef TMGCN_FUSED_TRACE
    {
      const int n_tile_rows = row_end - row0 < FBM ? (int)(row_end - row0) : FBM;
      const int k = Pol::kShortTiles && short_tile(rows, row0 + n_tile_rows <= (row0 / a.N + 1) * a.N) ? 8 : 0;
      const unsigned long long ft_g = FT_NOW();
      ft[k + 0] += ft_b - ft_a;
      ft[k + 1] += ft_c - ft_b;
      ft[k + 2] += ft_d - ft_c;
      ft[k + 3] += ft_e - ft_d;
      ft[k + 4] += ft_f - ft_e;
      ft[k + 5] += ft_g - ft_f;
      ft[k + 6] += 1;
    }
#endif
  }
#ifdef TMGCN_FUSED_TRACE
  if (trace_words && threadIdx.x == 0 && blockIdx.x < 4096)
    for (int i = 0; i < 16; ++i) trace_words[blockIdx.x * 16 + i] = ft[i];
#endif
}

inline int fused_check_args(const char* who, int32_t grid_reserve, int64_t n_rows, int32_t N, int32_t K, int32_t Nf, bool widths_ok,
                            const char* widths_need, int32_t act, int32_t y_bf16, int64_t rows_per_batch) {
  TMGCN_REQUIRE(grid_reserve >= 0 && grid_reserve <= 4096, "%s: grid_reserve %d out of range [0, 4096]", who, grid_reserve);
  TMGCN_REQUIRE(n_rows >= 0 && N > 0, "%s: bad shape n_rows=%lld N=%d", who, (long long)n_rows, N);
  TMGCN_REQUIRE(widths_ok, "%s: unsupported widths K=%d Nf=%d %s", who, K, Nf, widths_need);
  TMGCN_REQUIRE(act >= TMGCN_ACT_NONE && act <= TMGCN_ACT_SELU, "%s: unknown activation %d", who, act);
  TMGCN_REQUIRE(y_bf16 == 0 || y_bf16 == 1, "%s: y_bf16=%d is neither 0 (fp32 Y) nor 1 (bf16 Y)", who, y_bf16);
  TMGCN_REQUIRE(rows_per_batch >= 0, "%s: negative rows_per_batch", who);
  return TMGCN_OK;
}

template <class Args>
inline int fused_plan_tiles(const char* who, Args& a, hipStream_t st) {
  a.tiles = make_tile_map(a.n_rows, (a.rows_per_batch == 0 || a.rows_per_batch % a.N == 0) ? (int64_t)a.N : a.rows_per_batch);
  a.n_tiles = a.tiles.n_tiles;
  TMGCN_REQUIRE(a.n_tiles < (int64_t)0x7fffffff, "%s: too many row tiles", who);
  a.tile_counter = acquire_tile_counters(st, 2);
  TMGCN_REQUIRE(a.tile_counter, "%s: no tile counter: %s", who, pool_error());
  return TMGCN_OK;
}

}
```

tm-gcn_amd/csrc/torch_ops.cpp:

```cpp
#include <ATen/ATen.h>
#include <c10/core/DeviceGuard.h>
#include <c10/hip/HIPStream.h>
#include <torch/csrc/autograd/custom_function.h>
#include <torch/library.h>

#include <mutex>
#include <tuple>
#include <vector>

#include "tmgcn.h"

namespace {

using at::Tensor;
using torch::autograd::AutogradContext;
using torch::autograd::variable_list;
using OptTensor = c10::optional<Tensor>;

inline void* ptr(const Tensor& t) {
  return (t.defined() && t.numel()) ? const_cast<void*>(t.const_data_ptr()) : nullptr;
}
inline void* stream_of(const Tensor& t) {
  return (void*)c10::hip::getCurrentHIPStream(t.device().index()).stream();
}
// ... 11 lines not shown
inline Tensor aligned16(const Tensor& t) {
  return (!t.defined() || reinterpret_cast<uintptr_t>(t.const_data_ptr()) % 16 == 0) ? t : t.clone();
}
inline bool has(const Tensor& t) { return t.defined() && t.numel() > 0; }

Tensor mtransform(const Tensor& M, const Tensor& X, bool transpose, int64_t row_off, int64_t col_off,
                  int64_t T_out, int64_t band_lo, int64_t band_hi, int64_t x_group_rows,
                  int64_t y_group_rows) {
  want(M, "mtransform M");
  want(X, "mtransform X");
  TORCH_CHECK(M.dim() == 2 && M.size(0) == M.size(1), "mtransform: M must be square");
  TORCH_CHECK(X.dim() >= 1, "mtransform: X needs a leading time mode");
  c10::DeviceGuard g(X.device());
  const int64_t T_in = X.size(0);
  if (T_out < 0) T_out = T_in;
  const int64_t C = T_in ? X.numel() / T_in : 0;
  auto sizes = X.sizes().vec();
  sizes[0] = T_out;
  Tensor Y = at::empty(sizes, X.options());
  ok(tmgcn_mtransform_f32((const float*)ptr(M), (int32_t)M.size(0), (int32_t)M.size(0), transpose ? 1 : 0,
                          (int32_t)row_off, (int32_t)col_off, (int32_t)T_out, (int32_t)T_in,
                          (int32_t)band_lo, (int32_t)band_hi, (const float*)ptr(X), (float*)ptr(Y), C,
                          (int32_t)x_group_rows, (int32_t)y_group_rows, stream_of(X)),
     "tmgcn_mtransform_f32");
  return Y;
}

void mtransform_out(const Tensor& M, const Tensor& X, Tensor Y, bool transpose, int64_t row_off, int64_t col_off,
                    int64_t band_lo, int64_t band_hi, int64_t x_group_rows, int64_t y_group_rows) {
  want(M, "mtransform M");
  auto window = [](const Tensor& t, const char* name) {
    TORCH_CHECK(t.defined() && t.is_cuda() && t.scalar_type() == at::kFloat, name, ": expected an fp32 ROCm tensor");
    TORCH_CHECK(t.dim() == 3, name, ": expected [T, n, F]");
    TORCH_CHECK(t.size(0) == 0 || t.numel() == 0 ||
                    (t.stride(2) == 1 && t.stride(1) == t.size(2) && (t.size(0) == 1 || t.stride(0) >= t.size(1) * t.size(2))),
                name, ": slices must be dense [n, F] blocks (strides ", t.strides(), ")");
  };
  window(X, "mtransform_out X");
  window(Y, "mtransform_out Y");
  TORCH_CHECK(M.dim() == 2 && M.size(0) == M.size(1), "mtransform: M must be square");
  TORCH_CHECK(X.size(1) == Y.size(1) && X.size(2) == Y.size(2), "mtransform_out: X ", X.sizes(), " and Y ", Y.sizes(),
              " differ in their column extent");
  c10::DeviceGuard g(X.device());
  const int64_t T_in = X.size(0), T_out = Y.size(0), C = X.size(1) * X.size(2);
  const int64_t ldx = T_in > 1 ? X.stride(0) : C, ldy = T_out > 1 ? Y.stride(0) : C;
  ok(tmgcn_mtransform_ld_f32((const float*)ptr(M), (int32_t)M.size(0), (int32_t)M.size(0), transpose ? 1 : 0,
                             (int32_t)row_off, (int32_t)col_off, (int32_t)T_out, (int32_t)T_in, (int32_t)band_lo,
                             (int32_t)band_hi, (const float*)ptr(X), ldx, (float*)ptr(Y), ldy, C, (int32_t)x_group_rows,
                             (int32_t)y_group_rows, stream_of(X)),
     "tmgcn_mtransform_ld_f32");
}

void check_csr(const Tensor& rowptr, const Tensor& col, const Tensor& val, const Tensor& X, int64_t N,
               const char* who) {
  want(rowptr, "rowptr", at::kLong);
  want(col, "col", at::kInt);
  want(val, "val");
  TORCH_CHECK(X.dim() == 3 && X.size(1) == N && (X.size(0) * N + 1) == rowptr.numel(), who, ": X ",
              X.sizes(), " does not match adjacency T=", N ? (rowptr.numel() - 1) / N : 0, " N=", N);
  TORCH_CHECK(val.device() == X.device(), who, ": adjacency and X live on different devices");
}

struct Giant {
  const int64_t* rows = nullptr;
  const int32_t* chunks = nullptr;
  int32_t n = 0, m = 0;
  Tensor ws;
  float* ws_ptr() const { return ws.defined() ? (float*)ws.data_ptr() : nullptr; }
  int64_t ws_bytes() const { return ws.defined() ? ws.numel() * 4 : 0; }
};
Giant giant_of(const OptTensor& g_rows, const OptTensor& g_chunks, const Tensor& X, const char* who) {
  Giant g;
  if (!g_rows.has_value() || !g_chunks.has_value() || g_rows->numel() == 0) return g;
  TORCH_CHECK(g_rows->is_cuda() && g_chunks->is_cuda() && g_rows->scalar_type() == at::kLong && g_chunks->scalar_type() == at::kInt &&
                  g_rows->is_contiguous() && g_chunks->is_contiguous() && g_chunks->numel() > 2 * g_rows->numel(),
              who, ": a giant-row plan is (int64 rows [n], int32 chunks [n + 1 + m]) on the device");
  g.rows = (const int64_t*)g_rows->const_data_ptr();
  g.chunks = (const int32_t*)g_chunks->const_data_ptr();
  g.n = (int32_t)g_rows->numel();
  g.m = (int32_t)(g_chunks->numel() - g_rows->numel() - 1);
  g.ws = at::empty({(int64_t)g.m, X.size(2)}, X.options());
  return g;
}

Tensor spmm_csr_batched(const Tensor& rowptr, const Tensor& col, const Tensor& val, const Tensor& X,
                        int64_t N, double avg_nnz_per_row, const OptTensor& giant_rows, const OptTensor& giant_chunks) {
  want(X, "spmm X");
  check_csr(rowptr, col, val, X, N, "spmm");
  c10::DeviceGuard g(X.device());
  Tensor Y = at::empty_like(X);
  const Giant gi = giant_of(giant_rows, giant_chunks, X, "spmm");
  ok(tmgcn_spmm_csr_batched_f32_plan((const int64_t*)ptr(rowptr), (const int32_t*)ptr(col),
                                     (const float*)ptr(val), (const float*)ptr(X), (float*)ptr(Y),
                                     X.size(0) * N, (int32_t)N, (int32_t)X.size(2), (float)avg_nnz_per_row,
                                     gi.rows, gi.chunks, gi.n, gi.m, gi.ws_ptr(), gi.ws_bytes(), stream_of(X)),
     "tmgcn_spmm_csr_batched_f32");
  return Y;
}

struct WShape {
  bool per_slice;
  int64_t wk, wn, stride;
};
WShape w_shape(const Tensor& W, bool trans_w, int64_t T, int64_t K, const char* who) {
  TORCH_CHECK(W.dim() == 2 || W.dim() == 3, who, ": W must be [K,Nf] or [T,K,Nf]");
  WShape s;
  s.per_slice = W.dim() == 3;
  const int64_t a = W.size(-2), b = W.size(-1);
  s.wk = trans_w ? b : a;
  s.wn = trans_w ? a : b;
  s.stride = s.per_slice ? a * b : 0;
  TORCH_CHECK(s.wk == K && (!s.per_slice || W.size(0) == T), who, ": size mismatch, operand [", T, ",*,", K,
              "] W ", W.sizes(), " trans_w=", trans_w);
  return s;
}

void spmm_gemm_launch(const Tensor& rowptr, const Tensor& col, const Tensor& val, const Tensor& X, int64_t N,
                      const Tensor& W, bool trans_w, int64_t act, const Tensor& Y, const Tensor& AX,
                      const Tensor& pre, int64_t grid_reserve, double avg_nnz_per_row, const OptTensor& giant_rows,
                      const OptTensor& giant_chunks) {
  const WShape s = w_shape(W, trans_w, X.size(0), X.size(2), "spmm_gemm");
  const Giant gi = giant_of(giant_rows, giant_chunks, X, "spmm_gemm");
  const int64_t n_rows = X.size(0) * N;
  const float avg = (float)avg_nnz_per_row;
  ok(tmgcn_spmm_gemm_f32_plan((const int64_t*)ptr(rowptr), (const int32_t*)ptr(col), (const float*)ptr(val),
                              (const float*)ptr(X), n_rows, (int32_t)N, (int32_t)X.size(2),
                              (const float*)ptr(W), (int32_t)s.wn, trans_w ? 1 : 0, s.per_slice ? N : 0, s.stride,
                              (int32_t)act, (float*)ptr(Y), (float*)ptr(AX), (float*)ptr(pre), (int32_t)grid_reserve,
                              avg, gi.rows, gi.chunks, gi.n, gi.m, gi.ws_ptr(), gi.ws_bytes(), stream_of(X)),
     "tmgcn_spmm_gemm_f32");
}

static std::tuple<Tensor, Tensor, Tensor> fused_outputs(const Tensor& X, int64_t N, int64_t wn, at::ScalarType y_dt, bool want_ax,
                                                        bool want_pre) {
  const auto f32 = X.options().dtype(at::kFloat);
  return {at::empty({X.size(0), N, wn}, f32.dtype(y_dt)), want_ax ? at::empty(X.sizes(), f32) : at::empty({0}, f32),
          want_pre ? at::empty({X.size(0), N, wn}, f32) : at::empty({0}, f32)};
}

std::tuple<Tensor, Tensor, Tensor> spmm_gemm(const Tensor& rowptr, const Tensor& col, const Tensor& val,
                                             const Tensor& X, int64_t N, const Tensor& W, bool trans_w,
                                             int64_t act, bool want_ax, bool want_pre, int64_t grid_reserve,
                                             double avg_nnz_per_row, const OptTensor& giant_rows,
                                             const OptTensor& giant_chunks) {
  want(X, "spmm_gemm X");
  want(W, "spmm_gemm W");
  check_csr(rowptr, col, val, X, N, "spmm_gemm");
  c10::DeviceGuard g(X.device());
  const WShape s = w_shape(W, trans_w, X.size(0), X.size(2), "spmm_gemm");
  auto [Y, AX, pre] = fused_outputs(X, N, s.wn, at::kFloat, want_ax, want_pre && act != TMGCN_ACT_NONE);
  spmm_gemm_launch(rowptr, col, val, aligned16(X), N, W, trans_w, act, Y, AX, pre, grid_reserve, avg_nnz_per_row, giant_rows,
                   giant_chunks);
  return {Y, AX, pre};
}

void spmm_gemm_out(const Tensor& rowptr, const Tensor& col, const Tensor& val, const Tensor& X, int64_t N,
                   const Tensor& W, bool trans_w, int64_t act, Tensor Y, const OptTensor& AX,
                   const OptTensor& pre, int64_t grid_reserve, double avg_nnz_per_row, const OptTensor& giant_rows,
                   const OptTensor& giant_chunks) {
  want(X, "spmm_gemm X");
  want(W, "spmm_gemm W");
  want(Y, "spmm_gemm out Y");
  check_csr(rowptr, col, val, X, N, "spmm_gemm");
  c10::DeviceGuard g(X.device());
  const WShape s = w_shape(W, trans_w, X.size(0), X.size(2), "spmm_gemm");
  TORCH_CHECK(Y.dim() == 3 && Y.size(0) == X.size(0) && Y.size(1) == N && Y.size(2) == s.wn,
              "spmm_gemm: out Y ", Y.sizes(), " != [", X.size(0), ",", N, ",", s.wn, "]");
  Tensor ax = AX.has_value() ? *AX : Tensor(), pr = pre.has_value() ? *pre : Tensor();
  if (ax.defined()) want(ax, "spmm_gemm out AX");
  if (pr.defined()) want(pr, "spmm_gemm out pre");
  TORCH_CHECK(!ax.defined() || reinterpret_cast<uintptr_t>(ax.const_data_ptr()) % 16 == 0,
              "spmm_gemm: the AX output view must start 16-byte aligned");
  spmm_gemm_launch(rowptr, col, val, aligned16(X), N, W, trans_w, act, Y, ax, pr, grid_reserve, avg_nnz_per_row, giant_rows,
                   giant_chunks);
}

std::tuple<Tensor, Tensor> bgemm(const Tensor& A, const Tensor& W, bool trans_w, int64_t act, bool want_pre,
                                 int64_t algo) {
  want(A, "gemm A");
  const bool w_bf16 = W.defined() && W.scalar_type() == at::kBFloat16;
  want(W, "gemm W", w_bf16 ? at::kBFloat16 : at::kFloat);
  TORCH_CHECK(A.dim() == 3, "gemm: A must be [T,N,K]");
  c10::DeviceGuard g(A.device());
  const int64_t T = A.size(0), N = A.size(1), K = A.size(2);
  const WShape s = w_shape(W, trans_w, T, K, "gemm");
  Tensor Y = at::empty({T, N, s.wn}, A.options());
  Tensor pre = (want_pre && act != TMGCN_ACT_NONE) ? at::empty_like(Y) : Tensor();
  if (w_bf16)
    ok(tmgcn_gemm_bf16w_f32((const float*)ptr(A), (const uint16_t*)ptr(W), (float*)ptr(Y), (float*)ptr(pre), T * N,
                            (int32_t)K, (int32_t)s.wn, trans_w ? 1 : 0, s.per_slice ? N : 0, s.stride,
                            (int32_t)act, (int32_t)algo, stream_of(A)),
       "tmgcn_gemm_bf16w_f32");
  else
    ok(tmgcn_gemm_f32((const float*)ptr(A), (const float*)ptr(W), (float*)ptr(Y), (float*)ptr(pre), T * N,
                      (int32_t)K, (int32_t)s.wn, trans_w ? 1 : 0, s.per_slice ? N : 0, s.stride, (int32_t)act,
                      (int32_t)algo, stream_of(A)),
       "tmgcn_gemm_f32");
  return {Y, pre.defined() ? pre : none_like(A)};
}

Tensor bgemm_dW(const Tensor& A, const Tensor& dY, bool per_slice, int64_t algo) {
  want(A, "gemm_dw A");
  want(dY, "gemm_dw dY");
  TORCH_CHECK(A.dim() == 3 && dY.dim() == 3 && A.size(0) == dY.size(0) && A.size(1) == dY.size(1),
              "gemm_dw: A ", A.sizes(), " and dY ", dY.sizes(), " do not match");
  c10::DeviceGuard g(A.device());
  const int64_t T = A.size(0), N = A.size(1), K = A.size(2), Nf = dY.size(2), R = T * N;
  const int64_t rpb = per_slice ? N : 0;
  const int64_t need = tmgcn_gemm_dw_workspace_bytes(R, (int32_t)K, (int32_t)Nf, rpb);
  Tensor ws = at::empty({need > 0 ? need : 1}, A.options().dtype(at::kByte));
  Tensor dW = per_slice ? at::empty({T, K, Nf}, A.options()) : at::empty({K, Nf}, A.options());
  ok(tmgcn_gemm_dw_f32((const float*)ptr(A), (const float*)ptr(dY), (float*)ptr(dW), R, (int32_t)K, (int32_t)Nf,
                       rpb, (int32_t)algo, ptr(ws), ws.numel(), stream_of(A)),
     "tmgcn_gemm_dw_f32");
  return dW;
}

Tensor bgemm_dW_act(const Tensor& A, const Tensor& dY, const Tensor& pre, int64_t act, bool per_slice) {
  want(A, "gemm_dw A");
  want(dY, "gemm_dw dY");
  want(pre, "gemm_dw pre-activation");
  TORCH_CHECK(A.dim() == 3 && dY.dim() == 3 && A.size(0) == dY.size(0) && A.size(1) == dY.size(1) && pre.sizes() == dY.sizes(),
              "gemm_dw_act: A ", A.sizes(), ", dY ", dY.sizes(), " and pre ", pre.sizes(), " do not match");
  c10::DeviceGuard g(A.device());
  const int64_t T = A.size(0), N = A.size(1), K = A.size(2), Nf = dY.size(2), R = T * N;
  const int64_t rpb = per_slice ? N : 0;
  const int64_t need = tmgcn_gemm_dw_workspace_bytes(R, (int32_t)K, (int32_t)Nf, rpb);
  Tensor ws = at::empty({need > 0 ? need : 1}, A.options().dtype(at::kByte));
  Tensor dW = per_slice ? at::empty({T, K, Nf}, A.options()) : at::empty({K, Nf}, A.options());
  ok(tmgcn_gemm_dw_act_f32((const float*)ptr(A), (const float*)ptr(dY), (const float*)ptr(pre), (int32_t)act, (float*)ptr(dW), R,
                           (int32_t)K, (int32_t)Nf, rpb, ptr(ws), ws.numel(), stream_of(A)),
     "tmgcn_gemm_dw_act_f32");
  return dW;
}

Tensor edge_head_fwd(const Tensor& Z2, const Tensor& src, const Tensor& dst, const Tensor& U) {
  want(Z2, "edge_head Z");
  want(U, "edge_head U");
  const bool i32 = src.defined() && src.scalar_type() == at::kInt;
  want(src, "edge_head src", i32 ? at::kInt : at::kLong);
  want(dst, "edge_head dst", i32 ? at::kInt : at::kLong);
  TORCH_CHECK(Z2.dim() == 2 && U.dim() == 2 && U.size(0) == 2 * Z2.size(1), "edge_head: U ", U.sizes(),
              " does not match F=", Z2.size(1));
  TORCH_CHECK(src.numel() == dst.numel(), "edge_head: src and dst differ in length");
  c10::DeviceGuard g(Z2.device());
  const int64_t E = src.numel(), F = Z2.size(1), C = U.size(1);
  Tensor out = at::empty({E, C}, Z2.options());
  if (i32)
    ok(tmgcn_edge_head_fwd_i32_f32((const float*)ptr(Z2), (const int32_t*)ptr(src), (const int32_t*)ptr(dst),
                                   (const float*)ptr(U), (float*)ptr(out), E, (int32_t)F, (int32_t)C, stream_of(Z2)),
       "tmgcn_edge_head_fwd_i32_f32");
  else
    ok(tmgcn_edge_head_fwd_f32((const float*)ptr(Z2), (const int64_t*)ptr(src), (const int64_t*)ptr(dst),
                               (const float*)ptr(U), (float*)ptr(out), E, (int32_t)F, (int32_t)C, stream_of(Z2)),
       "tmgcn_edge_head_fwd_f32");
  return out;
}

std::tuple<Tensor, Tensor> edge_head_bwd(const Tensor& Z2, const Tensor& src, const Tensor& dst, const Tensor& U,
                                         const Tensor& dout, const Tensor& eptr, const Tensor& eidx, bool need_dz,
                                         bool need_du) {
  want(Z2, "edge_head Z");
  want(U, "edge_head U");
  want(dout, "edge_head dout");
  const bool i32 = src.defined() && src.scalar_type() == at::kInt;
  const auto it = i32 ? at::kInt : at::kLong;
  want(src, "edge_head src", it);
  want(dst, "edge_head dst", it);
  want(eptr, "edge_head eptr", it);
  want(eidx, "edge_head eidx", it);
  c10::DeviceGuard g(Z2.device());
  TORCH_CHECK(Z2.dim() == 2 && U.dim() == 2 && U.size(0) == 2 * Z2.size(1), "edge_head_bwd: U ", U.sizes(),
              " does not match F=", Z2.dim() == 2 ? Z2.size(1) : -1);
  TORCH_CHECK(src.numel() == dst.numel(), "edge_head_bwd: src and dst differ in length");
  const int64_t R = Z2.size(0), F = Z2.size(1), C = U.size(1), E = src.numel();
  TORCH_CHECK(dout.dim() == 2 && dout.size(0) == E && dout.size(1) == C, "edge_head_bwd: dout ", dout.sizes(),
              " is not [E=", E, ", C=", C, "]");
  TORCH_CHECK(eptr.numel() == R + 1 && eidx.numel() == 2 * E, "edge_head_bwd: inverted index does not match R=", R,
              " E=", E);
  Tensor dZ = need_dz ? at::empty_like(Z2) : Tensor();
  Tensor dU = need_du ? at::empty_like(U) : Tensor();
  const int64_t need = tmgcn_edge_head_bwd_workspace_bytes(E, (int32_t)F, (int32_t)C);
  Tensor ws = at::empty({need > 0 ? need : 1}, Z2.options().dtype(at::kByte));
  if (i32)
    ok(tmgcn_edge_head_bwd_i32_f32((const float*)ptr(Z2), (const int32_t*)ptr(src), (const int32_t*)ptr(dst),
                                   (const float*)ptr(U), (const float*)ptr(dout), (const int32_t*)ptr(eptr),
                                   (const int32_t*)ptr(eidx), (float*)ptr(dZ), (float*)ptr(dU), R, E, (int32_t)F,
                                   (int32_t)C, ptr(ws), ws.numel(), stream_of(Z2)),
       "tmgcn_edge_head_bwd_i32_f32");
  else
    ok(tmgcn_edge_head_bwd_f32((const float*)ptr(Z2), (const int64_t*)ptr(src), (const int64_t*)ptr(dst),
                               (const float*)ptr(U), (const float*)ptr(dout), (const int64_t*)ptr(eptr),
                               (const int64_t*)ptr(eidx), (float*)ptr(dZ), (float*)ptr(dU), R, E, (int32_t)F,
                               (int32_t)C, ptr(ws), ws.numel(), stream_of(Z2)),
       "tmgcn_edge_head_bwd_f32");
  return {dZ.defined() ? dZ : none_like(Z2), dU.defined() ? dU : none_like(Z2)};
}

Tensor act_fwd(const Tensor& x, int64_t act) {
  want(x, "act x");
  c10::DeviceGuard g(x.device());
  Tensor y = at::empty_like(x);
  ok(tmgcn_act_fwd_f32((const float*)ptr(x), (float*)ptr(y), x.numel(), (int32_t)act, stream_of(x)),
     "tmgcn_act_fwd_f32");
  return y;
}
// ... 493 lines not shown
    TORCH_CHECK(dW32.numel() == T_run * F * k, "egcn_bwd: dW32 ", dW32.sizes(), " must be [", T_run, ", ", F, ", ", k, "]");
  }
  c10::DeviceGuard g(H.device());
  Tensor dP = at::empty({P.numel()}, P.options()), dW0 = at::empty({F, k}, P.options());
  Tensor dH = need_dH ? (H.size(0) == T_run ? at::empty(H.sizes(), H.options()) : at::zeros(H.sizes(), H.options()))
                      : Tensor();
  const int64_t need = (wide ? tmgcn_egcn_wide_bwd_workspace_bytes : tmgcn_egcn_bwd_workspace_bytes)((int32_t)T_run, (int32_t)F,
                                                                                                      (int32_t)k);
  Tensor ws = at::empty({need > 0 ? need : 1}, H.options().dtype(at::kByte));
  ok((wide ? tmgcn_egcn_wide_bwd : tmgcn_egcn_bwd)((const double*)ptr(P), (const double*)ptr(Xg), (const int32_t*)ptr(idx), (const double*)ptr(ysel),
                    (const double*)ptr(Hsel), (const double*)ptr(Wseq), (const double*)ptr(gates),
                    dW32.defined() ? (const float*)ptr(dW32) : nullptr,
                    dWseq.defined() ? (const double*)ptr(dWseq) : nullptr, (double*)ptr(dP), (double*)ptr(dW0),
                    need_dH ? (float*)ptr(dH) : nullptr, N, (int32_t)T_run, (int32_t)F, (int32_t)k, ptr(ws), ws.numel(),
                    stream_of(H)),
     wide ? "tmgcn_egcn_wide_bwd" : "tmgcn_egcn_bwd");
  return {dP, dW0.view(W0.sizes()), dH};
}
std::tuple<Tensor, Tensor, Tensor> egcn_bwd(const Tensor& H, const Tensor& P, const Tensor& W0, const Tensor& Xg,
                                            const Tensor& idx, const Tensor& ysel, const Tensor& Hsel, const Tensor& Wseq,
                                            const Tensor& gates, const OptTensor& dWseq_, const OptTensor& dW32_,
                                            bool need_dH) {
  return egcn_bwd_any(false, H, P, W0, Xg, idx, ysel, Hsel, Wseq, gates, dWseq_, dW32_, need_dH);
}
std::tuple<Tensor, Tensor, Tensor> egcn_wide_bwd(const Tensor& H, const Tensor& P, const Tensor& W0, const Tensor& Xg,
                                                 const Tensor& idx, const Tensor& ysel, const Tensor& Hsel,
                                                 const Tensor& Wseq, const Tensor& gates, const OptTensor& dWseq_,
                                                 const OptTensor& dW32_, bool need_dH) {
  return egcn_bwd_any(true, H, P, W0, Xg, idx, ysel, Hsel, Wseq, gates, dWseq_, dW32_, need_dH);
}

bool edge_head_supported(int64_t F, int64_t C) { return tmgcn_edge_head_supported((int32_t)F, (int32_t)C) != 0; }
bool head_loss_supported(int64_t F, int64_t C, int64_t K) { return tmgcn_head_loss_supported((int32_t)F, (int32_t)C, (int32_t)K) != 0; }
int64_t abi_version() { return tmgcn_abi_version(); }

struct MTransformFn : public torch::autograd::Function<MTransformFn> {
  static Tensor forward(AutogradContext* ctx, const Tensor& X, const Tensor& M, int64_t band_lo, int64_t band_hi,
                        int64_t row_off, int64_t col_off, int64_t T_out, int64_t xg, int64_t yg) {
    at::AutoDispatchBelowADInplaceOrView guard;
    ctx->save_for_backward({M});
    ctx->saved_data["lo"] = band_lo;
    ctx->saved_data["hi"] = band_hi;
    ctx->saved_data["ro"] = row_off;
    ctx->saved_data["co"] = col_off;
    ctx->saved_data["T_in"] = X.size(0);
    ctx->saved_data["xg"] = xg;
    ctx->saved_data["yg"] = yg;
    return mtransform(M, X, false, row_off, col_off, T_out, band_lo, band_hi, xg, yg);
  }
  static variable_list backward(AutogradContext* ctx, variable_list grads) {
    at::AutoDispatchBelowADInplaceOrView guard;
    const Tensor M = ctx->get_saved_variables()[0];
    auto& d = ctx->saved_data;
    Tensor dX = mtransform(M, grads[0].contiguous(), true, d["co"].toInt(), d["ro"].toInt(), d["T_in"].toInt(),
                           d["hi"].toInt(), d["lo"].toInt(), d["yg"].toInt(), d["xg"].toInt());
    return {dX, Tensor(), Tensor(), Tensor(), Tensor(), Tensor(), Tensor(), Tensor(), Tensor()};
  }
};

struct SpmmFn : public torch::autograd::Function<SpmmFn> {
  static Tensor forward(AutogradContext* ctx, const Tensor& X, const Tensor& rowptr, const Tensor& col,
                        const Tensor& val, const OptTensor& t_rowptr, const OptTensor& t_col, const OptTensor& t_val,
                        int64_t N, double avg, const OptTensor& g_rows, const OptTensor& g_chunks, const OptTensor& t_g_rows,
                        const OptTensor& t_g_chunks, bool need) {
    at::AutoDispatchBelowADInplaceOrView guard;
    if (need) {
      TORCH_CHECK(t_rowptr.has_value() && t_col.has_value() && t_val.has_value(),
                  "spmm: X requires grad but no transposed adjacency was passed");
      const bool tg = t_g_rows.has_value() && t_g_chunks.has_value();
      ctx->save_for_backward({*t_rowptr, *t_col, *t_val, tg ? *t_g_rows : none_like(X), tg ? *t_g_chunks : none_like(X)});
    }
    ctx->saved_data["N"] = N;
    ctx->saved_data["avg"] = avg;
    return spmm_csr_batched(rowptr, col, val, X, N, avg, g_rows, g_chunks);
  }
  static variable_list backward(AutogradContext* ctx, variable_list grads) {
    at::AutoDispatchBelowADInplaceOrView guard;
    auto sv = ctx->get_saved_variables();
    const bool tg = sv[3].numel() > 0;
    Tensor dX = spmm_csr_batched(sv[0], sv[1], sv[2], grads[0].contiguous(), ctx->saved_data["N"].toInt(),
                                 ctx->saved_data["avg"].toDouble(), tg ? OptTensor(sv[3]) : OptTensor(), tg ? OptTensor(sv[4]) : OptTensor());
    variable_list out(14);
    out[0] = dX;
    return out;
  }
};

struct FeatureGemmFn : public torch::autograd::Function<FeatureGemmFn> {
  static Tensor forward(AutogradContext* ctx, const Tensor& A, const Tensor& W, int64_t act) {
    at::AutoDispatchBelowADInplaceOrView guard;
    auto [Y, pre] = bgemm(A, W, false, act, act != TMGCN_ACT_NONE, TMGCN_GEMM_AUTO);
    ctx->saved_data["act"] = act;
    ctx->save_for_backward({A, W, pre});
    return Y;
  }
  static variable_list backward(AutogradContext* ctx, variable_list grads) {
    at::AutoDispatchBelowADInplaceOrView guard;
    auto sv = ctx->get_saved_variables();
    const Tensor &A = sv[0], &W = sv[1], &pre = sv[2];
    const int64_t act = ctx->saved_data["act"].toInt();
    Tensor dY = grads[0].contiguous();
    Tensor dA, dW;
    const bool fold_act = act != TMGCN_ACT_NONE && !ctx->needs_input_grad(0) && ctx->needs_input_grad(1) && A.dim() == 3 &&
                          tmgcn_gemm_dw_act_supported((int32_t)A.size(-1), (int32_t)dY.size(-1)) &&
                          reinterpret_cast<uintptr_t>(A.const_data_ptr()) % 8 == 0 &&
                          reinterpret_cast<uintptr_t>(dY.const_data_ptr()) % 8 == 0 &&
                          reinterpret_cast<uintptr_t>(pre.const_data_ptr()) % 8 == 0;
    if (fold_act) {
      dW = bgemm_dW_act(A, dY, pre, act, W.dim() == 3);
      if (dW.scalar_type() != W.scalar_type()) dW = dW.to(W.scalar_type());
      return {dA, dW, Tensor()};
    }
    if (act != TMGCN_ACT_NONE) dY = act_bwd(pre, dY, act);
    if (ctx->needs_input_grad(0)) dA = std::get<0>(bgemm(dY, W, true, TMGCN_ACT_NONE, false, TMGCN_GEMM_AUTO));
    if (ctx->needs_input_grad(1)) {
      dW = bgemm_dW(A, dY, W.dim() == 3, TMGCN_DW_AUTO);
      if (dW.scalar_type() != W.scalar_type()) dW = dW.to(W.scalar_type());
    }
    return {dA, dW, Tensor()};
  }
};

static void fused_save(AutogradContext* ctx, const char* who, const Tensor& W, const Tensor& AX, const Tensor& pre,
                       const OptTensor& t_rowptr, const OptTensor& t_col, const OptTensor& t_val, bool need_x, variable_list more,
                       int64_t N, double avg, int64_t act, int64_t grid_reserve) {
  if (need_x)
    TORCH_CHECK(t_rowptr.has_value() && t_col.has_value() && t_val.has_value(), who,
                ": X requires grad but no transposed adjacency was passed");
  more.insert(more.begin(), {W, AX, pre, need_x ? *t_rowptr : Tensor(), need_x ? *t_col : Tensor(), need_x ? *t_val : Tensor()});
  ctx->save_for_backward(more);
  ctx->saved_data["N"] = N;
  ctx->saved_data["avg"] = avg;
  ctx->saved_data["act"] = act;
  ctx->saved_data["reserve"] = grid_reserve;
}

static Tensor fused_dx_f32(AutogradContext* ctx, const variable_list& sv, const Tensor& dY, const OptTensor& gr, const OptTensor& gc) {
  const Tensor& W = sv[0];
  const int64_t N = ctx->saved_data["N"].toInt();
  const double avg = ctx->saved_data["avg"].toDouble();
  if (spmm_gemm_supported(dY.size(-1), W.size(-2)))
    return std::get<0>(spmm_gemm(sv[3], sv[4], sv[5], dY, N, W, true, TMGCN_ACT_NONE, false, false,
                                 ctx->saved_data["reserve"].toInt(), avg, gr, gc));
  return spmm_csr_batched(sv[3], sv[4], sv[5], std::get<0>(bgemm(dY, W, true, TMGCN_ACT_NONE, false, TMGCN_GEMM_AUTO)), N, avg, gr, gc);
}

struct SpmmFeatureGemmFn : public torch::autograd::Function<SpmmFeatureGemmFn> {
  static Tensor forward(AutogradContext* ctx, const Tensor& X, const Tensor& W, const Tensor& rowptr,
                        const Tensor& col, const Tensor& val, const OptTensor& t_rowptr, const OptTensor& t_col,
                        const OptTensor& t_val, int64_t N, double avg, int64_t act, int64_t grid_reserve,
                        const OptTensor& g_rows, const OptTensor& g_chunks, const OptTensor& t_g_rows,
                        const OptTensor& t_g_chunks, bool need_x, bool need_w) {
    at::AutoDispatchBelowADInplaceOrView guard;
    auto [Y, AX, pre] = spmm_gemm(rowptr, col, val, X, N, W, false, act, need_w, need_x || need_w, grid_reserve, avg, g_rows, g_chunks);
    const bool tg = need_x && t_g_rows.has_value() && t_g_chunks.has_value();
    fused_save(ctx, "spmm_feature_gemm", W, AX, pre, t_rowptr, t_col, t_val, need_x,
               {tg ? *t_g_rows : none_like(X), tg ? *t_g_chunks : none_like(X)}, N, avg, act, grid_reserve);
    return Y;
  }
  static variable_list backward(AutogradContext* ctx, variable_list grads) {
    at::AutoDispatchBelowADInplaceOrView guard;
    auto sv = ctx->get_saved_variables();
    const Tensor &W = sv[0], &AX = sv[1], &pre = sv[2];
    const int64_t act = ctx->saved_data["act"].toInt();
    Tensor dY = grads[0].contiguous();
    if (act != TMGCN_ACT_NONE) dY = act_bwd(pre, dY, act);
    Tensor dX, dW;
    if (ctx->needs_input_grad(0)) {
      const bool tg = sv[6].numel() > 0;
      dX = fused_dx_f32(ctx, sv, dY, tg ? OptTensor(sv[6]) : OptTensor(), tg ? OptTensor(sv[7]) : OptTensor());
    }
    if (ctx->needs_input_grad(1)) dW = bgemm_dW(AX, dY, W.dim() == 3, TMGCN_DW_AUTO);
    variable_list out(18);
    out[0] = dX;
    out[1] = dW;
    return out;
  }
};

struct SpmmFeatureGemmBf16Fn : public torch::autograd::Function<SpmmFeatureGemmBf16Fn> {
  static Tensor forward(AutogradContext* ctx, const Tensor& X, const Tensor& W, const Tensor& rowptr, const Tensor& col,
                        const Tensor& val, const OptTensor& t_rowptr, const OptTensor& t_col, const OptTensor& t_val, int64_t N,
                        double avg, int64_t act, bool y_bf16, int64_t grid_reserve, bool need_x, bool need_w) {
    at::AutoDispatchBelowADInplaceOrView guard;
    auto [Y, AX, pre] = spmm_gemm_bf16(rowptr, col, val, X, N, W, false, act, need_w, need_x || need_w, y_bf16, grid_reserve, avg);
    fused_save(ctx, "spmm_feature_gemm_bf16", W, AX, pre, t_rowptr, t_col, t_val, need_x, {}, N, avg, act, grid_reserve);
    return Y;
  }
  static variable_list backward(AutogradContext* ctx, variable_list grads) {
    at::AutoDispatchBelowADInplaceOrView guard;
    auto sv = ctx->get_saved_variables();
    const Tensor &W = sv[0], &AX = sv[1], &pre = sv[2];
    const int64_t N = ctx->saved_data["N"].toInt(), act = ctx->saved_data["act"].toInt();
    const double avg = ctx->saved_data["avg"].toDouble();
    Tensor dY = grads[0].contiguous(), dYb;
    if (dY.scalar_type() == at::kBFloat16) {
      if (act == TMGCN_ACT_NONE) dYb = dY;
      dY = cast_multi({dY}, false)[0];
    }
    if (act != TMGCN_ACT_NONE) dY = act_bwd(pre, dY, act);
    Tensor dX, dW;
    if (ctx->needs_input_grad(0)) {
      if (spmm_gemm_bf16_supported(dY.size(-1), W.size(-2))) {
        if (!dYb.defined()) dYb = cast_multi({dY}, true)[0];
        dX = std::get<0>(spmm_gemm_bf16(sv[3], sv[4], sv[5], dYb, N, W, true, TMGCN_ACT_NONE, false, false, true,
                                        ctx->saved_data["reserve"].toInt(), avg));
      } else {
        dX = cast_multi({fused_dx_f32(ctx, sv, dY, OptTensor(), OptTensor())}, true)[0];
      }
    }
    if (ctx->needs_input_grad(1)) dW = bgemm_dW(AX, dY, W.dim() == 3, TMGCN_DW_AUTO);
    variable_list out(15);
    out[0] = dX;
    out[1] = dW;
    return out;
  }
};

struct EdgeHeadFn : public torch::autograd::Function<EdgeHeadFn> {
  static Tensor forward(AutogradContext* ctx, const Tensor& Z, const Tensor& U, const Tensor& src, const Tensor& dst,
                        const OptTensor& eptr, const OptTensor& eidx, bool need) {
    at::AutoDispatchBelowADInplaceOrView guard;
    Tensor Z2 = Z.contiguous().reshape({-1, Z.size(-1)});
    if (need) {
      TORCH_CHECK(eptr.has_value() && eidx.has_value(), "edge_head: gradients needed but no inverted edge index passed");
      ctx->save_for_backward({Z2, U, src, dst, *eptr, *eidx});
    }
    ctx->saved_data["zshape"] = Z.sizes().vec();
    return edge_head_fwd(Z2, src, dst, U);
  }
  static variable_list backward(AutogradContext* ctx, variable_list grads) {
    at::AutoDispatchBelowADInplaceOrView guard;
    auto sv = ctx->get_saved_variables();
    const bool nz = ctx->needs_input_grad(0), nu = ctx->needs_input_grad(1);
    auto [dZ, dU] = edge_head_bwd(sv[0], sv[2], sv[3], sv[1], grads[0].contiguous(), sv[4], sv[5], nz, nu);
    Tensor gz = nz ? dZ.reshape(ctx->saved_data["zshape"].toIntVector()) : Tensor();
    return {gz, nu ? dU : Tensor(), Tensor(), Tensor(), Tensor(), Tensor(), Tensor()};
  }
};

static std::mutex g_unit_mutex;
static std::vector<Tensor> g_unit_grad(64);
Tensor unit_gradient(const Tensor& like) {
  TORCH_CHECK(like.is_cuda(), "unit_gradient: a ROCm tensor names the device");
  const int dev = like.device().index();
  std::lock_guard<std::mutex> lock(g_unit_mutex);
  TORCH_CHECK(dev >= 0 && dev < (int)g_unit_grad.size(), "unit_gradient: device index out of range");
  if (!g_unit_grad[dev].defined()) g_unit_grad[dev] = at::ones({}, like.options().dtype(at::kFloat));
  return g_unit_grad[dev];
}
static bool is_unit_gradient(const Tensor& g) {
  if (!g.defined() || !g.is_cuda()) return false;
  const int dev = g.device().index();
  std::lock_guard<std::mutex> lock(g_unit_mutex);
  return dev >= 0 && dev < (int)g_unit_grad.size() && g_unit_grad[dev].defined() && g.numel() == 1 &&
         g.const_data_ptr() == g_unit_grad[dev].const_data_ptr();
}

struct HeadLossFn : public torch::autograd::Function<HeadLossFn> {
  static variable_list forward(AutogradContext* ctx, const Tensor& Z, const OptTensor& W_fold, const Tensor& U,
                               const Tensor& eptr, const Tensor& arow, const Tensor& ent, const Tensor& other,
                               const Tensor& meta, const Tensor& counts, const Tensor& weight, const Tensor& sync,
                               bool want_logits, bool need, bool unit_grad, const OptTensor& srow, int64_t n_parts) {
    at::AutoDispatchBelowADInplaceOrView guard;
    const bool fold = W_fold.has_value() && W_fold->defined();
    Tensor Z2 = Z.contiguous().reshape({-1, Z.size(-1)});
    const int64_t R = Z2.size(0), F = fold ? W_fold->size(1) : Z2.size(1), E = ent.numel() / 2;
    const bool deferred = need && !fold && !unit_grad && R * F * 8 > E * 10;
    auto [loss, logits, dZ, dU] = head_loss_fwd(Z2, W_fold, U, eptr, arow, ent, other, meta, counts, weight, sync, OptTensor(),
                                                need && !deferred, want_logits, true, srow, n_parts);
    if (need && deferred)
      ctx->save_for_backward({Z2, U, eptr, arow, ent, other, meta, counts, weight, sync,
                              (srow.has_value() && srow->defined()) ? *srow : none_like(Z2)});
    else if (need)
      ctx->save_for_backward({dZ, dU});
    ctx->saved_data["n_parts"] = n_parts;
    ctx->saved_data["zshape"] = Z.sizes().vec();
    ctx->saved_data["fold"] = fold;
    ctx->saved_data["deferred"] = deferred;
    ctx->mark_non_differentiable({logits});
    return {loss, logits};
  }
  static variable_list backward(AutogradContext* ctx, variable_list grads) {
    at::AutoDispatchBelowADInplaceOrView guard;
    auto sv = ctx->get_saved_variables();
    const bool fold = ctx->saved_data["fold"].toBool(), deferred = ctx->saved_data["deferred"].toBool();
    Tensor g = grads[0].contiguous().to(at::kFloat);
    Tensor gz, gu;
    if (deferred) {
      TORCH_CHECK(sv.size() == 11, "head_loss: backward through a call made without gradients");
      auto out = head_loss_fwd(sv[0], OptTensor(), sv[1], sv[2], sv[3], sv[4], sv[5], sv[6], sv[7], sv[8], sv[9], g, true, false,
                               false, sv[10].numel() ? OptTensor(sv[10]) : OptTensor(), ctx->saved_data["n_parts"].toInt());
      gz = std::get<2>(out);
      gu = std::get<3>(out);
    } else {
      TORCH_CHECK(sv.size() == 2, "head_loss: backward through a call made without gradients");
      if (is_unit_gradient(grads[0])) {
        gz = sv[0];
        gu = sv[1];
      } else {
        std::tie(gz, gu) = scale2(g, sv[0], sv[1]);
      }
    }
    variable_list out(16);
    if (fold) out[1] = gz; else out[0] = gz.reshape(ctx->saved_data["zshape"].toIntVector());
    out[2] = gu;
    return out;
  }
};

struct Layer12Fn : public torch::autograd::Function<Layer12Fn> {
  static Tensor forward(AutogradContext* ctx, const Tensor& H, const Tensor& W1, const Tensor& W2, const Tensor& rowptr,
                        const Tensor& col, const Tensor& val, const OptTensor& t_rowptr, const OptTensor& t_col,
                        const OptTensor& t_val, int64_t N, double avg, int64_t act1, int64_t act2, const OptTensor& blk,
                        const OptTensor& t_blk, bool need1, bool need2) {
    at::AutoDispatchBelowADInplaceOrView guard;
    want(H, "layer12 H");
    for (const OptTensor* b : {&blk, &t_blk})
      TORCH_CHECK(!b->has_value() || ((*b)->is_cuda() && (*b)->scalar_type() == at::kLong && (*b)->is_contiguous() && (*b)->dim() == 2 &&
                                      (*b)->size(1) == 2 && (*b)->size(0) >= 1),
                  "layer12: a row-block partition is a contiguous int64 [n, 2] tensor of (first row, rows) pairs on the device");
    want(W1, "layer12 W1");
    want(W2, "layer12 W2");
    check_csr(rowptr, col, val, H, N, "layer12");
    TORCH_CHECK(W1.dim() == 2 && W2.dim() == 2 && W1.size(0) == H.size(2) && W2.size(0) == W1.size(1), "layer12: W1 ",
// ... 128 lines not shown
      for (int64_t d : shape) n *= d;
      Tensor v = dP.narrow(0, off, n).view(shape);
      off += n;
      return v;
    };
    out.push_back(take(ctx->saved_data["p_shape"].toIntVector()));
    for (int64_t i = 0; i < n_gates; ++i) out.push_back(take(ctx->saved_data["g" + std::to_string(i)].toIntVector()));
    out.push_back(dW0);
    const int64_t n_rows = ctx->saved_data["n_rows"].toInt();
    for (int64_t i = 0; i < n_rows + 5; ++i) out.push_back(Tensor());
    return out;
  }
};

struct ActivationFn : public torch::autograd::Function<ActivationFn> {
  static Tensor forward(AutogradContext* ctx, const Tensor& x, int64_t act) {
    at::AutoDispatchBelowADInplaceOrView guard;
    ctx->save_for_backward({x});
    ctx->saved_data["act"] = act;
    return act_fwd(x, act);
  }
  static variable_list backward(AutogradContext* ctx, variable_list grads) {
    at::AutoDispatchBelowADInplaceOrView guard;
    return {act_bwd(ctx->get_saved_variables()[0], grads[0].contiguous(), ctx->saved_data["act"].toInt()), Tensor()};
  }
};

struct WeightedCeFn : public torch::autograd::Function<WeightedCeFn> {
  static Tensor forward(AutogradContext* ctx, const Tensor& logits, const Tensor& target, const Tensor& weight,
                        int64_t ignore_index) {
    at::AutoDispatchBelowADInplaceOrView guard;
    auto [loss, stats] = wce_fwd(logits, target, weight, ignore_index);
    ctx->save_for_backward({logits, target, weight, stats});
    ctx->saved_data["ign"] = ignore_index;
    return loss;
  }
  static variable_list backward(AutogradContext* ctx, variable_list grads) {
    at::AutoDispatchBelowADInplaceOrView guard;
    auto sv = ctx->get_saved_variables();
    Tensor g = grads[0].contiguous().to(at::kFloat);
    return {wce_bwd(sv[0], sv[1], sv[2], sv[3], g, ctx->saved_data["ign"].toInt()), Tensor(), Tensor(), Tensor()};
  }
};

Tensor m_transform_ad(const Tensor& X, const Tensor& M, int64_t band_lo, int64_t band_hi, int64_t row_off,
                      int64_t col_off, int64_t T_out, int64_t xg, int64_t yg) {
  return MTransformFn::apply(X, M, band_lo, band_hi, row_off, col_off, T_out, xg, yg);
}
Tensor spmm_ad(const Tensor& X, const Tensor& rowptr, const Tensor& col, const Tensor& val, const OptTensor& t_rowptr,
               const OptTensor& t_col, const OptTensor& t_val, int64_t N, double avg, const OptTensor& g_rows,
               const OptTensor& g_chunks, const OptTensor& t_g_rows, const OptTensor& t_g_chunks) {
  return SpmmFn::apply(X, rowptr, col, val, t_rowptr, t_col, t_val, N, avg, g_rows, g_chunks, t_g_rows, t_g_chunks,
                       at::GradMode::is_enabled() && X.requires_grad());
}
Tensor feature_gemm_ad(const Tensor& A, const Tensor& W, int64_t act) { return FeatureGemmFn::apply(A, W, act); }
Tensor spmm_feature_gemm_ad(const Tensor& X, const Tensor& W, const Tensor& rowptr, const Tensor& col,
                            const Tensor& val, const OptTensor& t_rowptr, const OptTensor& t_col,
                            const OptTensor& t_val, int64_t N, double avg, int64_t act, int64_t grid_reserve,
                            const OptTensor& g_rows, const OptTensor& g_chunks, const OptTensor& t_g_rows,
                            const OptTensor& t_g_chunks) {
  const bool grad = at::GradMode::is_enabled();
  return SpmmFeatureGemmFn::apply(X, W, rowptr, col, val, t_rowptr, t_col, t_val, N, avg, act, grid_reserve, g_rows, g_chunks,
                                  t_g_rows, t_g_chunks, grad && X.requires_grad(), grad && W.requires_grad());
}
Tensor spmm_feature_gemm_bf16_ad(const Tensor& X, const Tensor& W, const Tensor& rowptr, const Tensor& col, const Tensor& val,
                                 const OptTensor& t_rowptr, const OptTensor& t_col, const OptTensor& t_val, int64_t N, double avg,
                                 int64_t act, bool y_bf16, int64_t grid_reserve) {
  const bool grad = at::GradMode::is_enabled();
  return SpmmFeatureGemmBf16Fn::apply(X, W, rowptr, col, val, t_rowptr, t_col, t_val, N, avg, act, y_bf16, grid_reserve,
                                      grad && X.requires_grad(), grad && W.requires_grad());
}
Tensor round_bf16_ad(const Tensor& x) { return RoundBf16Fn::apply(x); }
Tensor edge_head_ad(const Tensor& Z, const Tensor& U, const Tensor& src, const Tensor& dst, const OptTensor& eptr,
                    const OptTensor& eidx) {
  return EdgeHeadFn::apply(Z, U, src, dst, eptr, eidx,
                           at::GradMode::is_enabled() && (Z.requires_grad() || U.requires_grad()));
}
std::tuple<Tensor, Tensor> head_loss_ad(const Tensor& Z, const OptTensor& W_fold, const Tensor& U, const Tensor& eptr,
                                        const Tensor& arow, const Tensor& ent, const Tensor& other, const Tensor& meta,
                                        const Tensor& counts, const Tensor& weight, const Tensor& sync, bool want_logits,
                                        bool unit_grad, const OptTensor& srow, int64_t n_parts) {
  const bool fold = W_fold.has_value() && W_fold->defined();
  const bool need = at::GradMode::is_enabled() && (U.requires_grad() || (fold ? W_fold->requires_grad() : Z.requires_grad()));
  auto out = HeadLossFn::apply(Z, W_fold, U, eptr, arow, ent, other, meta, counts, weight, sync, want_logits, need, unit_grad, srow,
                               n_parts);
  return {out[0], out[1]};
}
Tensor layer12_ad(const Tensor& H, const Tensor& W1, const Tensor& W2, const Tensor& rowptr, const Tensor& col, const Tensor& val,
                  const OptTensor& t_rowptr, const OptTensor& t_col, const OptTensor& t_val, int64_t N, double avg,
                  int64_t act1, int64_t act2, const OptTensor& blk, const OptTensor& t_blk) {
  TORCH_CHECK(!(at::GradMode::is_enabled() && H.requires_grad()), "layer12: H is the model's constant input (no gradient is formed for it)");
  const bool grad = at::GradMode::is_enabled();
  return Layer12Fn::apply(H, W1, W2, rowptr, col, val, t_rowptr, t_col, t_val, N, avg, act1, act2, blk, t_blk,
                          grad && W1.requires_grad(), grad && W2.requires_grad());
}
Tensor activation_ad(const Tensor& x, int64_t act) { return ActivationFn::apply(x, act); }
static Tensor wdgcn_lstm_any(bool wide, const Tensor& AX, const Tensor& P, const Tensor& h0, const Tensor& c0, int64_t H,
                             int64_t T_run) {
  const bool grad = at::GradMode::is_enabled();
  TORCH_CHECK(!(grad && (AX.requires_grad() || h0.requires_grad() || c0.requires_grad())),
              wide ? "wdgcn_lstm_wide" : "wdgcn_lstm", ": AX, h_init and c_init are constants (no gradient is formed for them)");
  return WdgcnLstmFn::apply(AX, P, h0, c0, H, T_run, grad && P.requires_grad(), wide);
}
Tensor wdgcn_lstm_ad(const Tensor& AX, const Tensor& P, const Tensor& h0, const Tensor& c0, int64_t H, int64_t T_run) {
  return wdgcn_lstm_any(false, AX, P, h0, c0, H, T_run);
}
Tensor wdgcn_lstm_wide_ad(const Tensor& AX, const Tensor& P, const Tensor& h0, const Tensor& c0, int64_t H, int64_t T_run) {
  return wdgcn_lstm_any(true, AX, P, h0, c0, H, T_run);
}
static std::tuple<Tensor, Tensor> egcn_evolve_any(bool wide, const Tensor& H, const Tensor& p, at::TensorList gates,
                                                  const Tensor& W0, int64_t k, int64_t T_run, const OptTensor& rowptr,
                                                  const OptTensor& col, const OptTensor& val, const OptTensor& X_prev,
                                                  const OptTensor& W_prev) {
  TORCH_CHECK(gates.size() == 9, "egcn_evolve: expected the nine gate matrices W_Z U_Z B_Z W_R U_R B_R W_H U_H B_H, got ",
              gates.size());
  const bool grad = at::GradMode::is_enabled();
  bool any = p.requires_grad() || W0.requires_grad() || H.requires_grad();
  for (const Tensor& q : gates) any = any || q.requires_grad();
  std::vector<Tensor> rows;
  if (rowptr.has_value() && rowptr->defined()) {
    TORCH_CHECK(col.has_value() && val.has_value() && X_prev.has_value() && W_prev.has_value(),
                "egcn_evolve: the fp64 rows of layer 2 need rowptr, col, val, X_prev and W_prev together");
    rows = {*rowptr, *col, *val, *X_prev, *W_prev};
  }
  auto r = EgcnEvolveFn::apply(H, p, gates, W0, at::TensorList(rows), k, T_run, grad && any, grad && H.requires_grad(), wide);
  return {r[0], r[1]};
}
std::tuple<Tensor, Tensor> egcn_evolve_ad(const Tensor& H, const Tensor& p, at::TensorList gates, const Tensor& W0,
                                          int64_t k, int64_t T_run, const OptTensor& rowptr, const OptTensor& col,
                                          const OptTensor& val, const OptTensor& X_prev, const OptTensor& W_prev) {
  return egcn_evolve_any(false, H, p, gates, W0, k, T_run, rowptr, col, val, X_prev, W_prev);
}
std::tuple<Tensor, Tensor> egcn_evolve_wide_ad(const Tensor& H, const Tensor& p, at::TensorList gates, const Tensor& W0,
                                               int64_t k, int64_t T_run, const OptTensor& rowptr, const OptTensor& col,
                                               const OptTensor& val, const OptTensor& X_prev, const OptTensor& W_prev) {
  return egcn_evolve_any(true, H, p, gates, W0, k, T_run, rowptr, col, val, X_prev, W_prev);
}
Tensor weighted_ce_ad(const Tensor& logits, const Tensor& target, const Tensor& weight, int64_t ignore_index) {
  return WeightedCeFn::apply(logits, target, weight, ignore_index);
}

}

TORCH_LIBRARY(tmgcn, m) {
  m.def("mtransform(Tensor M, Tensor X, bool transpose, int row_off, int col_off, int T_out, int band_lo, int band_hi, "
        "int x_group_rows, int y_group_rows) -> Tensor");
  m.def("mtransform_out(Tensor M, Tensor X, Tensor(a!) Y, bool transpose, int row_off, int col_off, int band_lo, "
        "int band_hi, int x_group_rows, int y_group_rows) -> ()");
  m.def("spmm_csr_batched(Tensor rowptr, Tensor col, Tensor val, Tensor X, int N, float avg_nnz_per_row, "
        "Tensor? giant_rows=None, Tensor? giant_chunks=None) -> Tensor");
  m.def("spmm_gemm(Tensor rowptr, Tensor col, Tensor val, Tensor X, int N, Tensor W, bool trans_w, int act, "
        "bool want_ax, bool want_pre, int grid_reserve, float avg_nnz_per_row=-1.0, Tensor? giant_rows=None, "
        "Tensor? giant_chunks=None) -> (Tensor, Tensor, Tensor)");
  m.def("spmm_gemm_out(Tensor rowptr, Tensor col, Tensor val, Tensor X, int N, Tensor W, bool trans_w, int act, "
        "Tensor(a!) Y, Tensor(b!)? AX, Tensor(c!)? pre, int grid_reserve, float avg_nnz_per_row=-1.0, Tensor? giant_rows=None, "
        "Tensor? giant_chunks=None) -> ()");
  m.def("spmm_gemm_bf16(Tensor rowptr, Tensor col, Tensor val, Tensor X, int N, Tensor W, bool trans_w, int act, "
        "bool want_ax, bool want_pre, bool y_bf16, int grid_reserve, float avg_nnz_per_row=-1.0) -> (Tensor, Tensor, Tensor)");
  m.def("spmm_gemm_bf16_supported(int K, int Nf) -> bool", &spmm_gemm_bf16_supported);
  m.def("bgemm(Tensor A, Tensor W, bool trans_w, int act, bool want_pre, int algo) -> (Tensor, Tensor)");
  m.def("bgemm_dW(Tensor A, Tensor dY, bool per_slice, int algo) -> Tensor");
  m.def("bgemm_dW_act(Tensor A, Tensor dY, Tensor pre, int act, bool per_slice) -> Tensor");
  m.def("edge_head_fwd(Tensor Z2, Tensor src, Tensor dst, Tensor U) -> Tensor");
  m.def("edge_head_bwd(Tensor Z2, Tensor src, Tensor dst, Tensor U, Tensor dout, Tensor eptr, Tensor eidx, "
        "bool need_dz, bool need_du) -> (Tensor, Tensor)");
  m.def("act_fwd(Tensor x, int act) -> Tensor");
  m.def("act_bwd(Tensor x, Tensor dy, int act) -> Tensor");
  m.def("wce_fwd(Tensor logits, Tensor target, Tensor weight, int ignore_index) -> (Tensor, Tensor)");
  m.def("wce_bwd(Tensor logits, Tensor target, Tensor weight, Tensor stats, Tensor g, int ignore_index) -> Tensor");
  m.def("head_loss_fwd(Tensor Z, Tensor? W_fold, Tensor U, Tensor eptr, Tensor arow, Tensor ent, Tensor other, Tensor meta, "
        "Tensor counts, Tensor weight, Tensor(a!) sync, Tensor? gscale, bool grad, bool want_logits, bool want_loss, "
        "Tensor? srow=None, int n_parts=0) -> (Tensor, Tensor, Tensor, Tensor)");
  m.def("scale2(Tensor g, Tensor a, Tensor b) -> (Tensor, Tensor)");
  m.def("sgd_step(Tensor(a!)[] params, Tensor[] grads, Tensor(b!)[] bufs, float lr, float momentum, float dampening, "
        "float weight_decay, bool nesterov, bool maximize, bool first_step) -> ()");
  m.def("head_loss_supported(int F, int C, int K) -> bool", &head_loss_supported);
  m.def("spmm_gemm_supported(int K, int Nf) -> bool", &spmm_gemm_supported);
  m.def("edge_head_supported(int F, int C) -> bool", &edge_head_supported);
  m.def("abi_version() -> int", &abi_version);
  m.def("m_transform(Tensor X, Tensor M, int band_lo, int band_hi, int row_off, int col_off, int T_out, "
        "int x_group_rows, int y_group_rows) -> Tensor");
  m.def("spmm(Tensor X, Tensor rowptr, Tensor col, Tensor val, Tensor? t_rowptr, Tensor? t_col, Tensor? t_val, "
        "int N, float avg_nnz_per_row, Tensor? giant_rows=None, Tensor? giant_chunks=None, Tensor? t_giant_rows=None, "
        "Tensor? t_giant_chunks=None) -> Tensor");
  m.def("feature_gemm(Tensor A, Tensor W, int act) -> Tensor");
  m.def("spmm_feature_gemm(Tensor X, Tensor W, Tensor rowptr, Tensor col, Tensor val, Tensor? t_rowptr, "
        "Tensor? t_col, Tensor? t_val, int N, float avg_nnz_per_row, int act, int grid_reserve, Tensor? giant_rows=None, "
        "Tensor? giant_chunks=None, Tensor? t_giant_rows=None, Tensor? t_giant_chunks=None) -> Tensor");
  m.def("spmm_feature_gemm_bf16(Tensor X, Tensor W, Tensor rowptr, Tensor col, Tensor val, Tensor? t_rowptr, "
        "Tensor? t_col, Tensor? t_val, int N, float avg_nnz_per_row, int act, bool y_bf16, int grid_reserve) -> Tensor");
  m.def("round_bf16(Tensor x) -> Tensor");
  m.def("edge_head(Tensor Z, Tensor U, Tensor src, Tensor dst, Tensor? eptr, Tensor? eidx) -> Tensor");
  m.def("activation(Tensor x, int act) -> Tensor");
  m.def("layer12(Tensor H, Tensor W1, Tensor W2, Tensor rowptr, Tensor col, Tensor val, Tensor? t_rowptr, Tensor? t_col, "
        "Tensor? t_val, int N, float avg_nnz_per_row, int act1, int act2, Tensor? row_blocks=None, Tensor? t_row_blocks=None) -> Tensor");
  m.def("layer12_supported(int K0, int F, int Nf) -> bool", &layer12_supported);
  m.def("weighted_ce(Tensor logits, Tensor target, Tensor weight, int ignore_index) -> Tensor");
  m.def("head_loss(Tensor Z, Tensor? W_fold, Tensor U, Tensor eptr, Tensor arow, Tensor ent, Tensor other, Tensor meta, "
        "Tensor counts, Tensor weight, Tensor(a!) sync, bool want_logits, bool unit_grad, Tensor? srow=None, int n_parts=0) -> "
        "(Tensor, Tensor)");
  m.def("head_loss_sgd(Tensor Z, Tensor(a!) W_fold, Tensor(b!) U, Tensor eptr, Tensor arow, Tensor other, Tensor meta, Tensor counts, "
        "Tensor weight, Tensor(c!) sync, Tensor(d!)? buf_W, Tensor(e!)? buf_U, float lr, float momentum, float dampening, "
        "float weight_decay, bool nesterov, bool maximize, bool first_step) -> (Tensor, Tensor, Tensor)");
  m.def("unit_gradient(Tensor like) -> Tensor");
  m.def("widen_params(Tensor[] params) -> Tensor[]");
  m.def("wdgcn_fwd(Tensor AX, Tensor P, Tensor h0, Tensor c0, int H, int T_run, bool need_c) -> (Tensor, Tensor)");
  m.def("wdgcn_bwd(Tensor AX, Tensor P, Tensor h0, Tensor c0, Tensor Z, Tensor C, Tensor dZ) -> Tensor");
  m.def("wdgcn_supported(int F0, int H) -> bool", &wdgcn_supported);
  m.def("wdgcn_lstm(Tensor AX, Tensor P, Tensor h0, Tensor c0, int H, int T_run) -> Tensor");
  m.def("wdgcn_wide_fwd(Tensor AX, Tensor P, Tensor h0, Tensor c0, int H, int T_run, bool need_saved) -> (Tensor, Tensor)");
  m.def("wdgcn_wide_bwd(Tensor AX, Tensor P, Tensor h0, Tensor c0, Tensor Z, Tensor saved, Tensor dZ) -> Tensor");
  m.def("wdgcn_wide_supported(int F0, int H) -> bool", &wdgcn_wide_supported);
  m.def("wdgcn_lstm_wide(Tensor AX, Tensor P, Tensor h0, Tensor c0, int H, int T_run) -> Tensor");
  m.def("egcn_fwd(Tensor H, Tensor P, Tensor W0, int k, int T_run, bool need_gates, Tensor? rowptr=None, Tensor? col=None, "
        "Tensor? val=None, Tensor? X_prev=None, Tensor? W_prev=None) -> (Tensor, Tensor, Tensor, Tensor, Tensor, Tensor, Tensor)");
  m.def("egcn_bwd(Tensor H, Tensor P, Tensor W0, Tensor X_g, Tensor idx, Tensor y_sel, Tensor H_sel, Tensor W_seq, "
        "Tensor gates, Tensor? dW_seq, Tensor? dW32, bool need_dH) -> (Tensor, Tensor, Tensor)");
  m.def("egcn_supported(int F, int k) -> bool", &egcn_supported);
  m.def("egcn_wide_fwd(Tensor H, Tensor P, Tensor W0, int k, int T_run, bool need_gates, Tensor? rowptr=None, Tensor? col=None, "
        "Tensor? val=None, Tensor? X_prev=None, Tensor? W_prev=None) -> (Tensor, Tensor, Tensor, Tensor, Tensor, Tensor, Tensor)");
  m.def("egcn_wide_bwd(Tensor H, Tensor P, Tensor W0, Tensor X_g, Tensor idx, Tensor y_sel, Tensor H_sel, Tensor W_seq, "
        "Tensor gates, Tensor? dW_seq, Tensor? dW32, bool need_dH) -> (Tensor, Tensor, Tensor)");
  m.def("egcn_wide_supported(int F, int k) -> bool", &egcn_wide_supported);
  m.def("egcn_evolve_wide(Tensor H, Tensor p, Tensor[] gate_params, Tensor W_init, int k, int T_run, Tensor? rowptr=None, "
        "Tensor? col=None, Tensor? val=None, Tensor? X_prev=None, Tensor? W_prev=None) -> (Tensor, Tensor)");
  m.def("egcn_evolve(Tensor H, Tensor p, Tensor[] gate_params, Tensor W_init, int k, int T_run, Tensor? rowptr=None, "
        "Tensor? col=None, Tensor? val=None, Tensor? X_prev=None, Tensor? W_prev=None) -> (Tensor, Tensor)");
}

static void impl_differentiable(torch::Library& m) {
  m.impl("m_transform", &m_transform_ad);
  m.impl("spmm", &spmm_ad);
  m.impl("feature_gemm", &feature_gemm_ad);
  m.impl("spmm_feature_gemm", &spmm_feature_gemm_ad);
  m.impl("spmm_feature_gemm_bf16", &spmm_feature_gemm_bf16_ad);
  m.impl("round_bf16", &round_bf16_ad);
  m.impl("edge_head", &edge_head_ad);
  m.impl("activation", &activation_ad);
  m.impl("layer12", &layer12_ad);
  m.impl("widen_params", &widen_params_ad);
  m.impl("weighted_ce", &weighted_ce_ad);
  m.impl("head_loss", &head_loss_ad);
  m.impl("wdgcn_lstm", &wdgcn_lstm_ad);
  m.impl("wdgcn_lstm_wide", &wdgcn_lstm_wide_ad);
  m.impl("egcn_evolve", &egcn_evolve_ad);
  m.impl("egcn_evolve_wide", &egcn_evolve_wide_ad);
}

TORCH_LIBRARY_IMPL(tmgcn, CUDA, m) {
  m.impl("mtransform", &mtransform);
  m.impl("mtransform_out", &mtransform_out);
  m.impl("spmm_csr_batched", &spmm_csr_batched);
  m.impl("spmm_gemm", &spmm_gemm);
  m.impl("spmm_gemm_out", &spmm_gemm_out);
  m.impl("spmm_gemm_bf16", &spmm_gemm_bf16);
  m.impl("bgemm", &bgemm);
  m.impl("bgemm_dW", &bgemm_dW);
  m.impl("bgemm_dW_act", &bgemm_dW_act);
  m.impl("edge_head_fwd", &edge_head_fwd);
  m.impl("edge_head_bwd", &edge_head_bwd);
  m.impl("act_fwd", &act_fwd);
  m.impl("act_bwd", &act_bwd);
  m.impl("wce_fwd", &wce_fwd);
  m.impl("wce_bwd", &wce_bwd);
  m.impl("head_loss_fwd", &head_loss_fwd);
  m.impl("head_loss_sgd", &head_loss_sgd);
  m.impl("scale2", &scale2);
  m.impl("sgd_step", &sgd_step);
  m.impl("unit_gradient", &unit_gradient);
  m.impl("wdgcn_fwd", &wdgcn_fwd);
  m.impl("wdgcn_bwd", &wdgcn_bwd);
  m.impl("wdgcn_wide_fwd", &wdgcn_wide_fwd);
  m.impl("wdgcn_wide_bwd", &wdgcn_wide_bwd);
  m.impl("egcn_fwd", &egcn_fwd);
  m.impl("egcn_bwd", &egcn_bwd);
  m.impl("egcn_wide_fwd", &egcn_wide_fwd);
  m.impl("egcn_wide_bwd", &egcn_wide_bwd);
  impl_differentiable(m);
}

TORCH_LIBRARY_IMPL(tmgcn, Autograd, m) {
  impl_differentiable(m);
}

TORCH_LIBRARY_IMPL(tmgcn, CPU, m) {
  m.impl("mtransform", &mtransform);
  m.impl("spmm_csr_batched", &spmm_csr_batched);
  m.impl("spmm_gemm", &spmm_gemm);
  m.impl("bgemm", &bgemm);
  m.impl("bgemm_dW", &bgemm_dW);
  m.impl("edge_head_fwd", &edge_head_fwd);
  m.impl("act_fwd", &act_fwd);
  m.impl("act_bwd", &act_bwd);
  impl_differentiable(m);
}
```

tm-gcn_amd/ops.py:

```python
from __future__ import annotations

import functools

import ctypes as C
from typing import Optional

import numpy as np
import torch

from . import _lib
from .csr import BatchedCSR


def _ptr(t: Optional[torch.Tensor]):
    return C.c_void_p(t.data_ptr()) if t is not None and t.numel() else C.c_void_p(0)


def _stream(t: torch.Tensor):
    return C.c_void_p(torch.cuda.current_stream(t.device).cuda_stream)


def _want(t: torch.Tensor, name: str, dtype=torch.float32):
    if not isinstance(t, torch.Tensor):
        raise RuntimeError(f"{name}: expected a torch.Tensor, got {type(t).__name__}")
# ... 88 lines not shown
        longest = int((end - beg).max()) if active.numel() else 0
        for _ in range(3):
            G = int(lanes(edges.E, max(1, n_arow)))
            split = self.SPLIT if self.SPLIT else 8 * (2 if G == 1 else 8) * G
            n_part = torch.clamp((end - beg + split - 1) // split, min=1)
            if not self.SPLIT and longest <= self.WORTH * split:
                n_part = torch.ones_like(n_part)
            n_new = int(n_part.sum()) if active.numel() else 0
            if n_new == n_arow or int(lanes(edges.E, max(1, n_new))) == G:
                break
            n_arow = n_new
        self.arow, self.srow, self.n_parts = self.split_rows(active, beg, end, n_part, split)
        self.counts = torch.bincount(t[~ignored], minlength=C)[:C].to(torch.int64).contiguous()
        self.sync = torch.zeros(_lib.SYNC_INTS, dtype=torch.int32, device=dev)
        self.R, self.C, self.ignore_index = R, C, ignore_index
        self._target, self._version = target, target._version

    @staticmethod
    def split_rows(active: torch.Tensor, beg: torch.Tensor, end: torch.Tensor, n_part: torch.Tensor, split: int):
        dev = active.device
        if not active.numel() or int(n_part.max()) <= 1:
            return torch.stack((active, beg, end, torch.zeros_like(active)), dim=1).to(torch.int32).contiguous(), None, 0
        own = torch.repeat_interleave(torch.arange(active.numel(), device=dev), n_part)
        k = torch.arange(own.numel(), device=dev) - (torch.cumsum(n_part, 0) - n_part)[own]
        is_split = n_part[own] > 1
        pid = torch.cumsum(is_split.long(), 0) * is_split
        pbeg = beg[own] + k * split
        pend = torch.minimum(pbeg + split, end[own])
        arow = torch.stack((active[own], pbeg, pend, pid), dim=1).to(torch.int32).contiguous()
        sp = n_part > 1
        first = (torch.cumsum(n_part * sp, 0) - n_part * sp)[sp]
        srow = torch.stack((active[sp], first, n_part[sp], torch.zeros_like(first)), dim=1).to(torch.int32).contiguous()
        return arow, srow, int((n_part * sp).sum())

    def matches(self, target: torch.Tensor, R: int, C: int, ignore_index: int) -> bool:
        return (self._target is target and self._version == target._version and self.R == R and self.C == C
                and self.ignore_index == ignore_index)


def head_loss_plan(edges: "EdgeIndex", R: int, target: torch.Tensor, C: int, ignore_index: int = -100) -> HeadLossPlan:
    plans = edges.__dict__.setdefault("_loss_plans", [])
    for p in plans:
        if p.matches(target, R, C, ignore_index):
            return p
    p = HeadLossPlan(edges, R, target, C, ignore_index)
    del plans[2:]
    plans.insert(0, p)
    return p


class MOperator:

    def __init__(self, M, device):
        M64 = torch.as_tensor(M).detach().to("cpu", torch.float64).contiguous()
        if M64.dim() != 2 or M64.shape[0] != M64.shape[1]:
            raise RuntimeError(f"M must be square, got {tuple(M64.shape)}")
        self.T = int(M64.shape[0])
        nz = torch.nonzero(M64)
        if nz.numel():
            d = nz[:, 1] - nz[:, 0]
            self.band_lo = int(max(0, -int(d.min())))
            self.band_hi = int(max(0, int(d.max())))
        else:
            self.band_lo = self.band_hi = 0
        self.M64 = M64
        self.M = M64.to(torch.float32).to(device).contiguous()
        self._inv: Optional["MOperator"] = None

    def inverse(self) -> "MOperator":
        if self._inv is None:
            self._inv = MOperator(torch.from_numpy(np.linalg.inv(self.M64.numpy())), self.M.device)
        return self._inv

    def window(self, k0: int, k1: int) -> "MOperator":
        return MOperator(self.M64[k0:k1, k0:k1], self.M.device)


class KernelTimer:

    def __init__(self):
        self.spans = {}

    def launch(self, tag, dev, fn):
        s = torch.cuda.Event(enable_timing=True)
        e = torch.cuda.Event(enable_timing=True)
        st = torch.cuda.current_stream(dev)
        s.record(st)
        rc = fn()
        e.record(st)
        self.spans.setdefault(tag, []).append((s, e))
        return rc

    def summary(self):
        torch.cuda.synchronize()
        out = {}
        for tag, spans in self.spans.items():
            ms = [a.elapsed_time(b) for a, b in spans]
            out[tag] = {"launches": len(ms), "avg_ms": sum(ms) / len(ms), "total_ms": sum(ms)}
        return out


class HipKernels:

    name = "hip"

    def __init__(self):
        self.timer: Optional[KernelTimer] = None
        self._ops = None

    @property
    def ops(self):
        if self._ops is None:
            self._ops = _lib.load_torch_ops()
        return self._ops

    def _run(self, tag, dev, fn):
        return self.timer.launch(tag, dev, fn) if self.timer is not None else fn()

    def mtransform(self, op: MOperator, X: torch.Tensor, transpose=False, row_off=0, col_off=0,
                   T_out: Optional[int] = None, x_group_rows=0, y_group_rows=0) -> torch.Tensor:
        lo, hi = (op.band_hi, op.band_lo) if transpose else (op.band_lo, op.band_hi)
        return self._run("mtransform_T" if transpose else "mtransform", X.device, lambda: self.ops.mtransform(
            op.M, X, bool(transpose), row_off, col_off, -1 if T_out is None else T_out, lo, hi, x_group_rows, y_group_rows))

    def mtransform_out(self, op: MOperator, X: torch.Tensor, Y: torch.Tensor, transpose=False, row_off=0, col_off=0,
                       x_group_rows=0, y_group_rows=0, tag=None) -> torch.Tensor:
        lo, hi = (op.band_hi, op.band_lo) if transpose else (op.band_lo, op.band_hi)
        tag = tag or ("mtransform_T" if transpose else "mtransform")
        self._run(tag, X.device, lambda: self.ops.mtransform_out(
            op.M, X, Y, bool(transpose), row_off, col_off, lo, hi, x_group_rows, y_group_rows))
        return Y

    def spmm(self, A: BatchedCSR, X: torch.Tensor, tag="spmm") -> torch.Tensor:
        return self._run(tag, X.device, lambda: self.ops.spmm_csr_batched(A.rowptr, A.col, A.val, X, A.N, A.avg_nnz_per_row,
                                                                          *A.giant_plan()))

    def spmm_gemm_supported(self, K: int, Nf: int) -> bool:
        return bool(_lib.load().tmgcn_spmm_gemm_supported(K, Nf))

    def spmm_gemm(self, A: BatchedCSR, X: torch.Tensor, W: torch.Tensor, trans_w=False, act=None,
                  want_ax=False, want_pre=False, tag="spmm_gemm", out=None, grid_reserve=0):
        act_id = _lib.ACT_IDS[act]
        if out is not None:
            Y, AX, pre = out
            self._run(tag, X.device, lambda: self.ops.spmm_gemm_out(
                A.rowptr, A.col, A.val, X, A.N, W, bool(trans_w), act_id, Y, AX, pre, int(grid_reserve),
                float(A.avg_nnz_per_row), *A.giant_plan()))
            return Y, AX, pre
        Y, AX, pre = self._run(tag, X.device, lambda: self.ops.spmm_gemm(
            A.rowptr, A.col, A.val, X, A.N, W, bool(trans_w), act_id, bool(want_ax), bool(want_pre), int(grid_reserve),
            float(A.avg_nnz_per_row), *A.giant_plan()))
        return Y, (AX if AX.numel() else None), (pre if pre.numel() else None)

    def spmm_gemm_bf16_supported(self, K: int, Nf: int) -> bool:
        return bool(_lib.load().tmgcn_spmm_gemm_bf16_supported(K, Nf))

    def spmm_gemm_bf16(self, A: BatchedCSR, X: torch.Tensor, W: torch.Tensor, trans_w=False, act=None, want_ax=False,
                       want_pre=False, out_dtype=None, tag="spmm_gemm_bf16", grid_reserve=0):
        Y, AX, pre = self._run(tag, X.device, lambda: self.ops.spmm_gemm_bf16(
            A.rowptr, A.col, A.val, X, A.N, W, bool(trans_w), _lib.ACT_IDS[act], bool(want_ax), bool(want_pre),
            _y_bf16(out_dtype), int(grid_reserve), float(A.avg_nnz_per_row)))
        return Y, (AX if AX.numel() else None), (pre if pre.numel() else None)

    def gemm(self, A: torch.Tensor, W: torch.Tensor, trans_w=False, act=None, want_pre=False, algo=None):
        Y, pre = self._run("gemm_dA" if trans_w else "gemm", A.device, lambda: self.ops.bgemm(
            A, W, bool(trans_w), _lib.ACT_IDS[act], bool(want_pre), _lib.GEMM_ALGOS[algo]))
        return (Y, pre if pre.numel() else None) if want_pre else Y

    def gemm_dw(self, A: torch.Tensor, dY: torch.Tensor, per_slice: bool, algo=None) -> torch.Tensor:
        return self._run("gemm_dW", A.device, lambda: self.ops.bgemm_dW(A, dY, bool(per_slice), _lib.DW_ALGOS[algo]))

    def edge_head_supported(self, F: int, Cn: int) -> bool:
        return bool(_lib.load().tmgcn_edge_head_supported(F, Cn))

    def edge_head_fwd(self, Z2: torch.Tensor, edges: "EdgeIndex", U: torch.Tensor) -> torch.Tensor:
        return self._run("edge_head", Z2.device, lambda: self.ops.edge_head_fwd(Z2, edges.src, edges.dst, U))

    def edge_head_bwd(self, Z2, edges: "EdgeIndex", U, dout, need_dz=True, need_du=True):
        eptr, eidx = edges.inverted(Z2.shape[0])
        dZ, dU = self._run("edge_head_bwd", Z2.device, lambda: self.ops.edge_head_bwd(
            Z2, edges.src, edges.dst, U, dout, eptr, eidx, bool(need_dz), bool(need_du)))
        return (dZ if need_dz else None), (dU if need_du else None)

    def act_fwd(self, x: torch.Tensor, act) -> torch.Tensor:
        return self.ops.act_fwd(x, _lib.ACT_IDS[act])

    def act_bwd(self, x: torch.Tensor, dy: torch.Tensor, act) -> torch.Tensor:
        return self.ops.act_bwd(x, dy, _lib.ACT_IDS[act])


kernels = HipKernels()


class _MTransform(torch.autograd.Function):
    @staticmethod
    def forward(ctx, X, op, row_off, col_off, T_out, x_group_rows, y_group_rows):
        ctx.op, ctx.row_off, ctx.col_off, ctx.T_in = op, row_off, col_off, X.shape[0]
        ctx.xg, ctx.yg = x_group_rows, y_group_rows
        return kernels.mtransform(op, X, False, row_off, col_off, T_out, x_group_rows, y_group_rows)

    @staticmethod
    def backward(ctx, dY):
        dX = kernels.mtransform(ctx.op, dY.contiguous(), True, ctx.col_off, ctx.row_off, ctx.T_in,
                                x_group_rows=ctx.yg, y_group_rows=ctx.xg)
        return dX, None, None, None, None, None, None


class _Spmm(torch.autograd.Function):
    @staticmethod
    def forward(ctx, X, A):
        ctx.A = A
        return kernels.spmm(A, X)

    @staticmethod
    def backward(ctx, dY):
        return kernels.spmm(ctx.A.transpose(), dY.contiguous(), tag="spmm_T"), None


class _FeatureGemm(torch.autograd.Function):
    @staticmethod
    def forward(ctx, A, W, act):
        ctx.act = act if _lib.ACT_IDS[act] else None
        if ctx.act is not None:
            Y, pre = kernels.gemm(A, W, act=act, want_pre=True)
            ctx.save_for_backward(A, W, pre)
        else:
            Y = kernels.gemm(A, W)
            ctx.save_for_backward(A, W)
        return Y

    @staticmethod
    def backward(ctx, dY):
        dY = dY.contiguous()
        if ctx.act is not None:
            A, W, pre = ctx.saved_tensors
            dY = kernels.act_bwd(pre, dY, ctx.act)
        else:
            A, W = ctx.saved_tensors
        dA = kernels.gemm(dY, W, trans_w=True) if ctx.needs_input_grad[0] else None
        dW = kernels.gemm_dw(A, dY, per_slice=W.dim() == 3) if ctx.needs_input_grad[1] else None
        if dW is not None and dW.dtype != W.dtype:
            dW = dW.to(W.dtype)
        return dA, dW, None


class _SpmmGemm(torch.autograd.Function):

    @staticmethod
    def forward(ctx, X, W, A, act):
        ctx.A = A
        ctx.act = act if _lib.ACT_IDS[act] else None
        need_w = ctx.needs_input_grad[1]
        Y, AX, pre = kernels.spmm_gemm(A, X, W, act=act, want_ax=need_w, want_pre=True)
        ctx.save_for_backward(W, AX if AX is not None else torch.empty(0, device=X.device),
                              pre if pre is not None else torch.empty(0, device=X.device))
        return Y

    @staticmethod
    def backward(ctx, dY):
        W, AX, pre = ctx.saved_tensors
        dY = dY.contiguous()
        if ctx.act is not None:
            dY = kernels.act_bwd(pre, dY, ctx.act)
        dX = dW = None
        if ctx.needs_input_grad[0]:
            if kernels.spmm_gemm_supported(dY.shape[-1], W.shape[-2]):
                dX, _, _ = kernels.spmm_gemm(ctx.A.transpose(), dY, W, trans_w=True, tag="spmm_gemm_T")
            else:
                dX = kernels.spmm(ctx.A.transpose(), kernels.gemm(dY, W, trans_w=True), tag="spmm_T")
        if ctx.needs_input_grad[1]:
            dW = kernels.gemm_dw(AX, dY, per_slice=W.dim() == 3)
        return dX, dW, None, None


class _EdgeHead(torch.autograd.Function):
    @staticmethod
    def forward(ctx, Z, U, edges):
        Z2 = Z.reshape(-1, Z.shape[-1])
        ctx.edges, ctx.zshape = edges, Z.shape
        ctx.save_for_backward(Z2, U)
        return kernels.edge_head_fwd(Z2, edges, U)

    @staticmethod
    def backward(ctx, dout):
        Z2, U = ctx.saved_tensors
        dZ, dU = kernels.edge_head_bwd(Z2, ctx.edges, U, dout.contiguous(), ctx.needs_input_grad[0],
                                       ctx.needs_input_grad[1])
        return (dZ.reshape(ctx.zshape) if dZ is not None else None), dU, None


class _Activation(torch.autograd.Function):
    @staticmethod
    def forward(ctx, x, act):
        ctx.act = act
        ctx.save_for_backward(x)
        return kernels.act_fwd(x, act)

    @staticmethod
    def backward(ctx, dy):
        (x,) = ctx.saved_tensors
        return kernels.act_bwd(x, dy.contiguous(), ctx.act), None


def _registered() -> bool:
    return kernels.name == "hip" and kernels.timer is None


def _csr_t(A: BatchedCSR, needed: bool):
    if not needed:
        return None, None, None
    At = A.transpose()
    return At.rowptr, At.col, At.val


def _giant(A: BatchedCSR, needed: bool):
    return (*A.giant_plan(), *(A.transpose().giant_plan() if needed else (None, None)))


def m_transform(X: torch.Tensor, op: MOperator, row_off=0, col_off=0, T_out=None, x_group_rows=0,
                y_group_rows=0) -> torch.Tensor:
    if _registered():
        return kernels.ops.m_transform(X, op.M, op.band_lo, op.band_hi, row_off, col_off,
                                       -1 if T_out is None else T_out, x_group_rows, y_group_rows)
    return _MTransform.apply(X, op, row_off, col_off, T_out, x_group_rows, y_group_rows)


def spmm(A: BatchedCSR, X: torch.Tensor) -> torch.Tensor:
    if _registered():
        need = X.requires_grad and torch.is_grad_enabled()
        return kernels.ops.spmm(X, A.rowptr, A.col, A.val, *_csr_t(A, need), A.N, A.avg_nnz_per_row, *_giant(A, need))
    return _Spmm.apply(X, A)


def feature_gemm(A: torch.Tensor, W: torch.Tensor, act=None) -> torch.Tensor:
    if _registered():
        return kernels.ops.feature_gemm(A, W, _lib.ACT_IDS[act])
    return _FeatureGemm.apply(A, W, act)


def _y_bf16(out_dtype) -> bool:
    if out_dtype not in (None, torch.float32, torch.bfloat16):
        raise RuntimeError(f"out_dtype must be None, torch.float32 or torch.bfloat16, got {out_dtype}")
    return out_dtype == torch.bfloat16


def spmm_gemm_bf16_supported(K: int, Nf: int) -> bool:
    return kernels.name == "hip" and kernels.spmm_gemm_bf16_supported(int(K), int(Nf))


def round_bf16(X: torch.Tensor) -> torch.Tensor:
    return kernels.ops.round_bf16(X)


def spmm_feature_gemm(A: BatchedCSR, X: torch.Tensor, W: torch.Tensor, act=None, fuse: Optional[bool] = None, out_dtype=None):
    K, Nf = X.shape[-1], W.shape[-1]
    y_bf16 = _y_bf16(out_dtype)
    if X.dtype == torch.bfloat16:
        if not spmm_gemm_bf16_supported(K, Nf):
            raise RuntimeError(f"the bf16-stored fused SpMM+GEMM does not support K={K}, Nf={Nf} "
                               "(K a multiple of 8 in [16,128], Nf <= 128)")
        if fuse is not None and not fuse:
            raise RuntimeError("a bf16-stored X has the fused launch only (fuse=False asks for the fp32 pair)")
        need = X.requires_grad and torch.is_grad_enabled()
        return kernels.ops.spmm_feature_gemm_bf16(X, W, A.rowptr, A.col, A.val, *_csr_t(A, need), A.N, A.avg_nnz_per_row,
                                                  _lib.ACT_IDS[act], y_bf16, 0)
    if y_bf16:
        raise RuntimeError("out_dtype=torch.bfloat16 needs an X stored in bf16; an fp32 X gives an fp32 Y")
    can = hasattr(kernels, "spmm_gemm_supported") and kernels.spmm_gemm_supported(K, Nf)
    if fuse is None:
        fuse = can
    if fuse and not can:
        raise RuntimeError(f"fused SpMM+GEMM does not support K={K}, Nf={Nf}")
    if fuse:
        if _registered():
            need = X.requires_grad and torch.is_grad_enabled()
            return kernels.ops.spmm_feature_gemm(X, W, A.rowptr, A.col, A.val, *_csr_t(A, need), A.N,
                                                 A.avg_nnz_per_row, _lib.ACT_IDS[act], 0, *_giant(A, need))
        return _SpmmGemm.apply(X, W, A, act)
    return feature_gemm(spmm(A, X), W, act=act)


@functools.lru_cache(maxsize=None)
def _layer12_widths_ok(K0: int, F: int, Nf: int) -> bool:
    return bool(_lib.load().tmgcn_layer12_supported(K0, F, Nf))


def layer12_supported(K0: int, F: int, Nf: int) -> bool:
    return kernels.name == "hip" and _layer12_widths_ok(int(K0), int(F), int(Nf))


def layer12(H: torch.Tensor, W1: torch.Tensor, act1, A: BatchedCSR, W2: torch.Tensor, act2=None, fuse: Optional[bool] = None):
    can = (W1.dim() == 2 and W2.dim() == 2 and H.dim() == 3 and not (H.requires_grad and torch.is_grad_enabled())
           and W1.dtype == torch.float32 and W2.dtype == torch.float32 and _registered()
           and layer12_supported(H.shape[-1], W1.shape[-1], W2.shape[-1]) and H.data_ptr() % 8 == 0)
    if fuse is None:
        fuse = can
    if fuse and not can:
        raise RuntimeError("layer12: operands do not allow the fused kernels")
    if not fuse:
        return spmm_feature_gemm(A, feature_gemm(H, W1, act=act1), W2, act=act2)
    need = torch.is_grad_enabled() and W1.requires_grad
    blk = A.row_blocks() if A.N >= 256 else None
    t_blk = None
    if need and A.N >= 256:
        At = A.transpose()
        if (At.avg_nnz_per_row < 4 or At.is_skewed()) and (At.row_blocks() is not None or At.avg_nnz_per_row >= 4):
            t_blk = At.row_block_runs()
    return kernels.ops.layer12(H, W1.contiguous(), W2.contiguous(), A.rowptr, A.col, A.val, *_csr_t(A, need), A.N, A.avg_nnz_per_row,
                               _lib.ACT_IDS[act1], _lib.ACT_IDS[act2], blk, t_blk)


def head_loss_sgd(AtXt: torch.Tensor, edges: EdgeIndex, W: torch.Tensor, U: torch.Tensor, target: torch.Tensor, weight: torch.Tensor,
                  ignore_index: int, buf_W: Optional[torch.Tensor], buf_U: Optional[torch.Tensor], lr: float, momentum: float = 0.0,
                  dampening: float = 0.0, weight_decay: float = 0.0, nesterov: bool = False, maximize: bool = False,
                  first_step: bool = False):
    R = AtXt.shape[0] * AtXt.shape[1]
    plan = head_loss_plan(edges, R, target, U.shape[-1], ignore_index)
# ... 182 lines not shown
```

Before: 5.851 billion.

## Fold dW computation into transposed SpMM-GEMM backward kernel via X^T slabs

Adds a fused backward kernel that computes dX = A^T dY W^T and, in the same tile loop, accumulates dW = X^T (A^T dY) into per-batch slab partials, followed by a slab reduction. The forward no longer materialises AX when this path applies; backward saves X instead and skips the separate bgemm_dW pass over AX. This removes an extra read of AX and one GEMM launch, but adds a workspace, a reduction kernel, and W streamed from memory inside the MFMA loop instead of held in registers. It applies only for K = Nf = 128, no activation, 2-D W, and cases that do not take the bx3 kernel.

```diff
diff --git a/include/tmgcn.h b/include/tmgcn.h
--- a/include/tmgcn.h
+++ b/include/tmgcn.h
@@ -76,6 +76,15 @@
                              float avg_nnz_per_row, const int64_t* giant_rows, const int32_t* giant_chunks,
                              int32_t n_giant, int32_t n_giant_chunks, float* giant_ws, int64_t giant_ws_bytes,
                              void* stream);
+
+int tmgcn_spmm_gemm_dw_supported(int32_t K, int32_t Nf, float avg_nnz_per_row, int32_t n_giant);
+int64_t tmgcn_spmm_gemm_dw_workspace_bytes(int64_t n_rows, int32_t N);
+int tmgcn_spmm_gemm_dw_f32(const int64_t* rowptr, const int32_t* col, const float* val, const float* dY,
+                           int64_t n_rows, int32_t N, int32_t K, const float* W, int32_t Nf, const float* Xt,
+                           float* dX, float* dW, int32_t grid_reserve, float avg_nnz_per_row,
+                           const int64_t* giant_rows, const int32_t* giant_chunks, int32_t n_giant,
+                           int32_t n_giant_chunks, float* giant_ws, int64_t giant_ws_bytes, void* workspace,
+                           int64_t workspace_bytes, void* stream);
 
 int tmgcn_spmm_gemm_bf16_supported(int32_t K, int32_t Nf);
 int tmgcn_spmm_gemm_bf16(const int64_t* rowptr, const int32_t* col, const float* val,
diff --git a/tm-gcn_amd/_lib.py b/tm-gcn_amd/_lib.py
--- a/tm-gcn_amd/_lib.py
+++ b/tm-gcn_amd/_lib.py
@@ -35,6 +35,10 @@
     "tmgcn_spmm_gemm_supported": (C.c_int, [_i32, _i32]),
     "tmgcn_spmm_gemm_f32": (C.c_int, [_p, _p, _p, _p, _i64, _i32, _i32, _p, _i32, _i32, _i64, _i64, _i32, _p, _p, _p, _i32, _p]),
     "tmgcn_spmm_gemm_f32_hint": (C.c_int, [_p, _p, _p, _p, _i64, _i32, _i32, _p, _i32, _i32, _i64, _i64, _i32, _p, _p, _p, _i32, C.c_float, _p]),
+    "tmgcn_spmm_gemm_dw_supported": (C.c_int, [_i32, _i32, C.c_float, _i32]),
+    "tmgcn_spmm_gemm_dw_workspace_bytes": (_i64, [_i64, _i32]),
+    "tmgcn_spmm_gemm_dw_f32": (C.c_int, [_p, _p, _p, _p, _i64, _i32, _i32, _p, _i32, _p, _p, _p, _i32, C.c_float,
+                                         _p, _p, _i32, _i32, _p, _i64, _p, _i64, _p]),
     "tmgcn_spmm_gemm_bf16_supported": (C.c_int, [_i32, _i32]),
     "tmgcn_spmm_gemm_bf16": (C.c_int, [_p, _p, _p, _p, _i64, _i32, _i32, _p, _i32, _i32, _i64, _i64, _i32, _p, _i32, _p, _p, _i32,
                                        C.c_float, _p]),
diff --git a/tm-gcn_amd/csrc/common.h b/tm-gcn_amd/csrc/common.h
--- a/tm-gcn_amd/csrc/common.h
+++ b/tm-gcn_amd/csrc/common.h
@@ -45,6 +45,8 @@
   __syncthreads();
   return *lds_flag != 0;
 }
+
+int launch_dw_slab_reduce(const float* slabs, float* dW, int64_t n_out, int32_t chunks, hipStream_t st);
 
 int launch_giant_partial(const char* who, const int64_t* rowptr, const int32_t* col, const float* val, const float* X, int32_t N,
                          int32_t F, const int64_t* giant_rows, const int32_t* giant_chunks, int32_t n_giant, int32_t n_giant_chunks,
diff --git a/tm-gcn_amd/csrc/gemm.hip b/tm-gcn_amd/csrc/gemm.hip
--- a/tm-gcn_amd/csrc/gemm.hip
+++ b/tm-gcn_amd/csrc/gemm.hip
@@ -1280,6 +1280,12 @@
   return check_launch("gemm_dw_reduce");
 }
 
+int tmgcn::launch_dw_slab_reduce(const float* slabs, float* dW, int64_t n_out, int32_t chunks, hipStream_t st) {
+  hipLaunchKernelGGL(gemm_dw_reduce_kernel, dim3((unsigned)((n_out + 63) / 64)), dim3(DWR_WAVES * 64), 0, st, slabs, dW, n_out,
+                     chunks, n_out);
+  return check_launch("gemm_dw_reduce");
+}
+
 extern "C" int tmgcn_gemm_dw_f32(const float* A, const float* dY, float* dW, int64_t R, int32_t K, int32_t Nf,
                                   int64_t rows_per_batch, int32_t algo, void* workspace, int64_t workspace_bytes,
                                   void* stream) {
diff --git a/tm-gcn_amd/csrc/spmm_gemm.hip b/tm-gcn_amd/csrc/spmm_gemm.hip
--- a/tm-gcn_amd/csrc/spmm_gemm.hip
+++ b/tm-gcn_amd/csrc/spmm_gemm.hip
@@ -35,6 +35,9 @@
   int64_t n_tiles;
   unsigned int* tile_counter;
   GiantPlan giant;
+  const float* Xt;
+  float* dw_slabs;
+  DwBatches dw_batches;
 };
 
 #ifdef TMGCN_FUSED_TRACE
@@ -52,6 +55,12 @@
   fused_tile_loop<FusedF32, LPR, U, NJ, US, false>(a, As, s_part, &s_tile, &s_row, FT_WORDS);
 }
 
+__global__ __launch_bounds__(256, TMGCN_FUSED_OCC) void spmm_gemm_dw_kernel(FusedArgs a) {
+  __shared__ float As[FBM * FLDA];
+  __shared__ float4 s_part[4 * 32];
+  __shared__ unsigned int s_tile, s_row;
+  fused_tile_loop<FusedF32Dw, 32, TMGCN_FUSED_U, 16, TMGCN_FUSED_US * TMGCN_FUSED_U, false>(a, As, s_part, &s_tile, &s_row, FT_WORDS);
+}
 
 typedef __bf16 bx_bf16x8 __attribute__((ext_vector_type(8)));
 typedef __bf16 bx_bf16x2 __attribute__((ext_vector_type(2)));
@@ -339,6 +348,10 @@
   return (K == 1 || K == 2 || K == 3 || K == 4 || K == 6 || K == 8) && Nf >= 1 && Nf <= 16;
 }
 
+static bool fused_takes_bx3(int32_t K, float avg_nnz_per_row, int32_t n_giant) {
+  return avg_nnz_per_row >= 0.f && avg_nnz_per_row < (float)TMGCN_BX3_MAX_DEG && n_giant == 0 && (K == 128 || K == 64);
+}
+
 }
 
 using namespace tmgcn;
@@ -364,7 +377,7 @@
   TMGCN_REQUIRE(n_rows % N == 0, "spmm_gemm: n_rows=%lld is not a multiple of N=%d", (long long)n_rows, N);
   if (fused_small_ok(K, Nf)) {
     FusedArgs s{rowptr, col, val, reinterpret_cast<const float4*>(X), n_rows, N, K, W, Nf, trans_w,
-                rows_per_batch, w_batch_stride, Y, AX, pre_act, act, TileMap{0, 0, 0, 0}, 0, nullptr, GiantPlan{nullptr, nullptr, nullptr, 0}};
+                rows_per_batch, w_batch_stride, Y, AX, pre_act, act, TileMap{0, 0, 0, 0}, 0, nullptr, GiantPlan{nullptr, nullptr, nullptr, 0}, nullptr, nullptr, DwBatches{}};
     int G = 8;
     if (avg_nnz_per_row >= 0.f) {
       G = 1;
@@ -383,7 +396,7 @@
   TMGCN_REQUIRE(reinterpret_cast<uintptr_t>(X) % 16 == 0 && (!AX || reinterpret_cast<uintptr_t>(AX) % 16 == 0),
                 "spmm_gemm: X / AX must be 16-byte aligned");
   FusedArgs a{rowptr, col, val, reinterpret_cast<const float4*>(X), n_rows, N, K, W, Nf, trans_w,
-              rows_per_batch, w_batch_stride, Y, AX, pre_act, act, TileMap{0, 0, 0, 0}, 0, nullptr, GiantPlan{nullptr, nullptr, nullptr, 0}};
+              rows_per_batch, w_batch_stride, Y, AX, pre_act, act, TileMap{0, 0, 0, 0}, 0, nullptr, GiantPlan{nullptr, nullptr, nullptr, 0}, nullptr, nullptr, DwBatches{}};
   if (n_giant > 0) {
     const int rc = launch_giant_partial("spmm_gemm (giant rows)", rowptr, col, val, X, N, K, giant_rows, giant_chunks, n_giant,
                                         n_giant_chunks, giant_ws, giant_ws_bytes, (hipStream_t)stream);
@@ -393,7 +406,7 @@
   hipStream_t st = (hipStream_t)stream;
   const int no_tiles = fused_plan_tiles("spmm_gemm", a, st);
   if (no_tiles) return no_tiles;
-  if (avg_nnz_per_row >= 0.f && avg_nnz_per_row < (float)TMGCN_BX3_MAX_DEG && n_giant == 0 && (K == 128 || K == 64)) {
+  if (fused_takes_bx3(K, avg_nnz_per_row, n_giant)) {
     if (K == 128) {
       int64_t gx = persistent_grid(spmm_gemm_bx3_kernel<32, TMGCN_FUSED_U, 4, TMGCN_BX3_US>, 512, 0, 2) - grid_reserve / 2;
       if (gx < 64) gx = 64;
@@ -435,6 +448,61 @@
   return check_launch("spmm_gemm");
 }
 
+extern "C" int tmgcn_spmm_gemm_dw_supported(int32_t K, int32_t Nf, float avg_nnz_per_row, int32_t n_giant) {
+  return (K == FKC && Nf == FKC && !fused_takes_bx3(K, avg_nnz_per_row, n_giant)) ? 1 : 0;
+}
+
+extern "C" int64_t tmgcn_spmm_gemm_dw_workspace_bytes(int64_t n_rows, int32_t N) {
+  if (n_rows <= 0 || N <= 0) return 0;
+  return make_dw_batches(make_tile_map(n_rows, N)).n_batches * (int64_t)(FKC * FKC * sizeof(float));
+}
+
+extern "C" int tmgcn_spmm_gemm_dw_f32(const int64_t* rowptr, const int32_t* col, const float* val, const float* dY,
+                                       int64_t n_rows, int32_t N, int32_t K, const float* W, int32_t Nf, const float* Xt,
+                                       float* dX, float* dW, int32_t grid_reserve, float avg_nnz_per_row,
+                                       const int64_t* giant_rows, const int32_t* giant_chunks, int32_t n_giant,
+                                       int32_t n_giant_chunks, float* giant_ws, int64_t giant_ws_bytes, void* workspace,
+                                       int64_t workspace_bytes, void* stream) {
+  const int bad = fused_check_args("spmm_gemm_dw", grid_reserve, n_rows, N, K, Nf,
+                                   tmgcn_spmm_gemm_dw_supported(K, Nf, avg_nnz_per_row, n_giant),
+                                   "(need K = Nf = 128 and a launch that takes the exact-f32 kernel: tmgcn_spmm_gemm_dw_supported); "
+                                   "use tmgcn_spmm_gemm_f32 + tmgcn_gemm_dw_f32", TMGCN_ACT_NONE, 0, 0);
+  if (bad) return bad;
+  TMGCN_REQUIRE(dW, "spmm_gemm_dw: null pointer");
+  hipStream_t st = (hipStream_t)stream;
+  if (n_rows == 0) {
+    TMGCN_REQUIRE(hipMemsetAsync(dW, 0, sizeof(float) * FKC * FKC, st) == hipSuccess, "spmm_gemm_dw: hipMemsetAsync failed");
+    return TMGCN_OK;
+  }
+  TMGCN_REQUIRE(rowptr && dY && W && Xt && dX, "spmm_gemm_dw: null pointer");
+  TMGCN_REQUIRE(n_rows % N == 0, "spmm_gemm_dw: n_rows=%lld is not a multiple of N=%d", (long long)n_rows, N);
+  TMGCN_REQUIRE(reinterpret_cast<uintptr_t>(dY) % 16 == 0 && reinterpret_cast<uintptr_t>(W) % 16 == 0 &&
+                    reinterpret_cast<uintptr_t>(workspace) % 16 == 0,
+                "spmm_gemm_dw: dY, W and the workspace must be 16-byte aligned");
+  const int64_t need = tmgcn_spmm_gemm_dw_workspace_bytes(n_rows, N);
+  const int small = check_workspace("spmm_gemm_dw", workspace, workspace_bytes, need);
+  if (small) return small;
+  FusedArgs a{rowptr, col, val, reinterpret_cast<const float4*>(dY), n_rows, N, K, W, Nf, 1, 0, 0, dX, nullptr, nullptr,
+              TMGCN_ACT_NONE, TileMap{0, 0, 0, 0}, 0, nullptr, GiantPlan{nullptr, nullptr, nullptr, 0}, Xt,
+              static_cast<float*>(workspace), DwBatches{}};
+  if (n_giant > 0) {
+    const int rc = launch_giant_partial("spmm_gemm_dw (giant rows)", rowptr, col, val, dY, N, K, giant_rows, giant_chunks, n_giant,
+                                        n_giant_chunks, giant_ws, giant_ws_bytes, st);
+    if (rc != TMGCN_OK) return rc;
+    a.giant = GiantPlan{giant_rows, giant_chunks, reinterpret_cast<const float4*>(giant_ws), n_giant};
+  }
+  const int no_tiles = fused_plan_tiles("spmm_gemm_dw", a, st);
+  if (no_tiles) return no_tiles;
+  a.dw_batches = make_dw_batches(a.tiles);
+  TMGCN_REQUIRE(a.dw_batches.n_batches < (int64_t)0x7fffffff, "spmm_gemm_dw: too many batches");
+  int64_t gx = persistent_grid_reserved(spmm_gemm_dw_kernel, 256, grid_reserve);
+  if (gx > a.dw_batches.n_batches) gx = a.dw_batches.n_batches;
+  hipLaunchKernelGGL(spmm_gemm_dw_kernel, dim3((unsigned)gx), dim3(256), 0, st, a);
+  const int rc = check_launch("spmm_gemm_dw");
+  if (rc) return rc;
+  return launch_dw_slab_reduce(static_cast<const float*>(workspace), dW, FKC * FKC, (int32_t)a.dw_batches.n_batches, st);
+}
+
 extern "C" int tmgcn_spmm_gemm_f32_hint(const int64_t* rowptr, const int32_t* col, const float* val,
                                          const float* X, int64_t n_rows, int32_t N, int32_t K,
                                          const float* W, int32_t Nf, int32_t trans_w,
diff --git a/tm-gcn_amd/csrc/spmm_gemm_tile.h b/tm-gcn_amd/csrc/spmm_gemm_tile.h
--- a/tm-gcn_amd/csrc/spmm_gemm_tile.h
+++ b/tm-gcn_amd/csrc/spmm_gemm_tile.h
@@ -19,6 +19,22 @@
 constexpr int FBM = 64;
 constexpr int FKC = 128;
 constexpr int FLDA = FKC + 4;
+
+#ifndef TMGCN_DW_BATCH
+#define TMGCN_DW_BATCH 16
+#endif
+#ifndef TMGCN_DW_XT_AHEAD
+#define TMGCN_DW_XT_AHEAD 16
+#endif
+#ifndef TMGCN_DW_W_AHEAD
+#define TMGCN_DW_W_AHEAD 3
+#endif
+constexpr int kDwBatch = TMGCN_DW_BATCH;
+constexpr int kDwLevels = 4;
+constexpr int kDwLevelCap = 1024;
+constexpr int kDwXtAhead = TMGCN_DW_XT_AHEAD;
+constexpr int kDwWAhead = TMGCN_DW_W_AHEAD;
+static_assert(kDwBatch >= (1 << kDwLevels) && (kDwBatch & (kDwBatch - 1)) == 0, "kDwBatch: a power of two, at least 16");
 
 __device__ __forceinline__ void store_y(float* p, float v) { store_f1(p, v); }
 __device__ __forceinline__ void store_y(uint16_t* p, float v) {
@@ -65,54 +81,153 @@
     else fused_store_half<GUARD, false, true>(acc, act, Yb, Pb, Nf, lane_off, rows_left);
   }
 }
-template <int NJ, class Args>
+template <int NJ, bool STREAM = false, class Args>
 __device__ __forceinline__ void fused_mfma_tile(const Args& a, const float* As, const float (&wreg)[NJ][4], int64_t row0,
                                                 int64_t row_end, int n0, int li, int lh) {
   if (n0 >= a.Nf) return;
   const float* Arow = &As[li * FLDA + 4 * lh];
   const int n = n0 + li;
+  const int act = STREAM ? (int)TMGCN_ACT_NONE : a.act;
+  float* const pre = STREAM ? nullptr : a.pre;
+  const float4* __restrict__ Wl = reinterpret_cast<const float4*>(a.W + (STREAM ? n * a.K + 4 * lh : 0));
 #pragma unroll
   for (int mb = 0; mb < FBM / 32; ++mb) {
     f32x16 acc;
 #pragma unroll
     for (int i = 0; i < 16; ++i) acc[i] = 0.f;
+    float4 wq[STREAM ? kDwWAhead : 1];
+    if constexpr (STREAM) {
+#pragma unroll
+      for (int j = 0; j < kDwWAhead; ++j) wq[j] = Wl[2 * j];
+    }
     float4 av_next = *reinterpret_cast<const float4*>(Arow + mb * 32 * FLDA);
 #pragma unroll
     for (int j = 0; j < NJ; ++j) {
       const float4 av = av_next;
       if (j + 1 < NJ) av_next = *reinterpret_cast<const float4*>(Arow + mb * 32 * FLDA + 8 * (j + 1));
-      acc = __builtin_amdgcn_mfma_f32_32x32x2f32(av.x, wreg[j][0], acc, 0, 0, 0);
-      acc = __builtin_amdgcn_mfma_f32_32x32x2f32(av.y, wreg[j][1], acc, 0, 0, 0);
-      acc = __builtin_amdgcn_mfma_f32_32x32x2f32(av.z, wreg[j][2], acc, 0, 0, 0);
-      acc = __builtin_amdgcn_mfma_f32_32x32x2f32(av.w, wreg[j][3], acc, 0, 0, 0);
+      if constexpr (STREAM) {
+        const float4 w = wq[j % kDwWAhead];
+        acc = __builtin_amdgcn_mfma_f32_32x32x2f32(av.x, w.x, acc, 0, 0, 0);
+        acc = __builtin_amdgcn_mfma_f32_32x32x2f32(av.y, w.y, acc, 0, 0, 0);
+        acc = __builtin_amdgcn_mfma_f32_32x32x2f32(av.z, w.z, acc, 0, 0, 0);
+        acc = __builtin_amdgcn_mfma_f32_32x32x2f32(av.w, w.w, acc, 0, 0, 0);
+        if (j + kDwWAhead < NJ) wq[j % kDwWAhead] = Wl[2 * (j + kDwWAhead)];
+      } else {
+        acc = __builtin_amdgcn_mfma_f32_32x32x2f32(av.x, wreg[j][0], acc, 0, 0, 0);
+        acc = __builtin_amdgcn_mfma_f32_32x32x2f32(av.y, wreg[j][1], acc, 0, 0, 0);
+        acc = __builtin_amdgcn_mfma_f32_32x32x2f32(av.z, wreg[j][2], acc, 0, 0, 0);
+        acc = __builtin_amdgcn_mfma_f32_32x32x2f32(av.w, wreg[j][3], acc, 0, 0, 0);
+      }
       __builtin_amdgcn_sched_barrier(0);
     }
     if (n < a.Nf) {
       const int64_t rbase = row0 + mb * 32;
       if constexpr (std::is_same<decltype(a.Y), float*>::value) {
         float* __restrict__ Yb = a.Y + rbase * a.Nf;
-        float* __restrict__ Pb = a.pre ? a.pre + rbase * a.Nf : nullptr;
+        float* __restrict__ Pb = pre ? pre + rbase * a.Nf : nullptr;
         const int lane_off = (4 * lh) * a.Nf + n;
-        if (rbase + 32 <= row_end) fused_store_half<false>(acc, a.act, Yb, Pb, a.Nf, lane_off, 32);
-        else fused_store_half<true>(acc, a.act, Yb, Pb, a.Nf, lane_off, (int)(row_end - rbase) - 4 * lh);
+        if (rbase + 32 <= row_end) fused_store_half<false>(acc, act, Yb, Pb, a.Nf, lane_off, 32);
+        else fused_store_half<true>(acc, act, Yb, Pb, a.Nf, lane_off, (int)(row_end - rbase) - 4 * lh);
       } else {
-        float* __restrict__ Pb = a.pre ? a.pre + rbase * a.Nf : nullptr;
+        float* __restrict__ Pb = pre ? pre + rbase * a.Nf : nullptr;
         const int lane_off = (4 * lh) * a.Nf + n;
         const int rows_left = rbase + 32 <= row_end ? 32 : (int)(row_end - rbase) - 4 * lh;
-        if (a.y_bf16) fused_store_half<true>(acc, a.act, static_cast<uint16_t*>(a.Y) + rbase * a.Nf, Pb, a.Nf, lane_off, rows_left);
-        else fused_store_half<true>(acc, a.act, static_cast<float*>(a.Y) + rbase * a.Nf, Pb, a.Nf, lane_off, rows_left);
+        if (a.y_bf16) fused_store_half<true>(acc, act, static_cast<uint16_t*>(a.Y) + rbase * a.Nf, Pb, a.Nf, lane_off, rows_left);
+        else fused_store_half<true>(acc, act, static_cast<float*>(a.Y) + rbase * a.Nf, Pb, a.Nf, lane_off, rows_left);
       }
     }
   }
+}
+
+
+struct DwBatches {
+  int64_t per, nb_unit, n_units, nb_main_last, main_last, lvl, n_batches;
+};
+__host__ __device__ __forceinline__ DwBatches make_dw_batches(const TileMap& m) {
+  DwBatches d;
+  d.per = m.tiles_per_unit;
+  d.n_units = m.n_tiles / m.tiles_per_unit;
+  d.nb_unit = (d.per + kDwBatch - 1) / kDwBatch;
+  d.lvl = d.per / kDwBatch < kDwLevelCap ? d.per / kDwBatch : kDwLevelCap;
+  d.main_last = d.per - (kDwBatch - (kDwBatch >> kDwLevels)) * d.lvl;
+  d.nb_main_last = (d.main_last + kDwBatch - 1) / kDwBatch;
+  d.n_batches = (d.n_units - 1) * d.nb_unit + d.nb_main_last + kDwLevels * d.lvl;
+  return d;
+}
+__host__ __device__ __forceinline__ void dw_batch_extent(const DwBatches& d, int64_t b, int64_t& t0, int64_t& t1) {
+  const int64_t unit = b / d.nb_unit < d.n_units - 1 ? b / d.nb_unit : d.n_units - 1;
+  int64_t j = b - unit * d.nb_unit, p0, p1, lim = d.per;
+  if (unit < d.n_units - 1 || j < d.nb_main_last) {
+    if (unit == d.n_units - 1) lim = d.main_last;
+    p0 = j * kDwBatch;
+    p1 = p0 + kDwBatch;
+  } else {
+    j -= d.nb_main_last;
+    const int64_t level = j / d.lvl, size = kDwBatch >> (level + 1);
+    p0 = d.main_last + (kDwBatch - 2 * size) * d.lvl + (j - level * d.lvl) * size;
+    p1 = p0 + size;
+  }
+  if (p1 > lim) p1 = lim;
+  t0 = unit * d.per + p0;
+  t1 = unit * d.per + p1;
+}
+
+template <bool ON>
+struct DwState {};
+template <>
+struct DwState<true> {
+  f32x16 c[4];
+  float xt[kDwXtAhead];
+  int64_t tile, end, batch;
+};
+
+__device__ __forceinline__ float dw_load_xt(const float* __restrict__ Xb, int n_tile_rows, int li, int lh, int s) {
+  const int rr = 2 * s + lh < n_tile_rows ? 2 * s + lh : n_tile_rows - 1;
+  return Xb[rr * FKC + li];
+}
+
+__device__ __forceinline__ void dw_mfma_tile(const float* __restrict__ Xb, int n_tile_rows, const float* As, DwState<true>& dw,
+                                             int li, int lh) {
+  const float* Grow = &As[lh * FLDA + 4 * li];
+  float4 g_next = *reinterpret_cast<const float4*>(Grow);
+#pragma unroll
+  for (int s = 0; s < FBM / 2; ++s) {
+    const float4 g = g_next;
+    if (s + 1 < FBM / 2) g_next = *reinterpret_cast<const float4*>(Grow + 2 * (s + 1) * FLDA);
+    const float x = 2 * s + lh < n_tile_rows ? dw.xt[s % kDwXtAhead] : 0.f;
+    dw.c[0] = __builtin_amdgcn_mfma_f32_32x32x2f32(x, g.x, dw.c[0], 0, 0, 0);
+    dw.c[1] = __builtin_amdgcn_mfma_f32_32x32x2f32(x, g.y, dw.c[1], 0, 0, 0);
+    dw.c[2] = __builtin_amdgcn_mfma_f32_32x32x2f32(x, g.z, dw.c[2], 0, 0, 0);
+    dw.c[3] = __builtin_amdgcn_mfma_f32_32x32x2f32(x, g.w, dw.c[3], 0, 0, 0);
+    if (s + kDwXtAhead < FBM / 2) dw.xt[s % kDwXtAhead] = dw_load_xt(Xb, n_tile_rows, li, lh, s + kDwXtAhead);
+    __builtin_amdgcn_sched_barrier(0);
+  }
+}
+
+__device__ __forceinline__ void dw_store_slab(float* __restrict__ slab, DwState<true>& dw, int n0, int li, int lh) {
+  float* __restrict__ d = slab + (n0 + 4 * lh) * FKC + 4 * li;
+#pragma unroll
+  for (int i = 0; i < 16; ++i) {
+    const int k = (i & 3) + 8 * (i >> 2);
+    *reinterpret_cast<float4*>(d + k * FKC) = make_float4(dw.c[0][i], dw.c[1][i], dw.c[2][i], dw.c[3][i]);
+  }
+#pragma unroll
+  for (int q = 0; q < 4; ++q)
+#pragma unroll
+    for (int i = 0; i < 16; ++i) dw.c[q][i] = 0.f;
 }
 
 struct FusedF32 {
   using Piece = PieceF32;
-  static constexpr bool kShortTiles = true, kGiantPlan = true;
+  static constexpr bool kShortTiles = true, kGiantPlan = true, kDw = false;
 };
 struct FusedBf16 {
   using Piece = PieceBf16;
-  static constexpr bool kShortTiles = false, kGiantPlan = false;
+  static constexpr bool kShortTiles = false, kGiantPlan = false, kDw = false;
+};
+struct FusedF32Dw {
+  using Piece = PieceF32;
+  static constexpr bool kShortTiles = true, kGiantPlan = true, kDw = true;
 };
 
 #ifdef TMGCN_FUSED_TRACE
@@ -201,6 +316,16 @@
   if (threadIdx.x == 0) *s_row = 4;
   HeavyScan heavy;
   heavy.init(a.rowptr, tm);
+  DwState<Pol::kDw> dw;
+  if constexpr (Pol::kDw) {
+    heavy.scanning = false;
+    dw.tile = dw.end = 0;
+    dw.batch = -1;
+#pragma unroll
+    for (int q = 0; q < 4; ++q)
+#pragma unroll
+      for (int i = 0; i < 16; ++i) dw.c[q][i] = 0.f;
+  }
 
 #ifdef TMGCN_FUSED_TRACE
   unsigned long long ft[16] = {0};
@@ -212,7 +337,17 @@
     int64_t tile = -1;
     if (heavy.scanning) tile = heavy.next(a.rowptr, tm, a.tile_counter + 1, s_tile, lane);
     const bool scanning = heavy.scanning;
-    if (!scanning) {
+    if constexpr (Pol::kDw) {
+      if (dw.tile == dw.end) {
+        if (dw.batch >= 0) dw_store_slab(a.dw_slabs + dw.batch * (FKC * FKC), dw, n0, lane & 31, lane >> 5);
+        if (threadIdx.x == 0) *s_tile = atomicAdd(a.tile_counter, 1u);
+        __syncthreads();
+        dw.batch = __builtin_amdgcn_readfirstlane(*s_tile);
+        if (dw.batch >= a.dw_batches.n_batches) break;
+        dw_batch_extent(a.dw_batches, dw.batch, dw.tile, dw.end);
+      }
+      tile = dw.tile++;
+    } else if (!scanning) {
       if (threadIdx.x == 0) *s_tile = atomicAdd(a.tile_counter, 1u);
       __syncthreads();
       tile = *s_tile;
@@ -224,17 +359,25 @@
     FT_STAMP(ft_b);
     TileRows rows;
     rows.load(a.rowptr, row0, row_end, lane);
-    if (!scanning && rows.entries > heavy.thr) {
+    if (!Pol::kDw && !scanning && rows.entries > heavy.thr) {
       __syncthreads();
       continue;
     }
     FT_WAIT();
     FT_STAMP(ft_c);
-    if (batch != cur_batch) {
+    if (!Pol::kDw && batch != cur_batch) {
       fused_load_w<NJ>(a, batch, n0, lane & 31, lane >> 5, wreg);
       cur_batch = batch;
     }
     fused_gather_tile<Pol, LPR, U, US, OFF32>(a, As, s_part, rows, row0, row_end, lane, wave, s_row);
+    if constexpr (Pol::kDw) {
+      if (row0 + FBM > row_end)
+        for (int i = (int)(row_end - row0) * FLDA + (int)threadIdx.x; i < FBM * FLDA; i += 256) As[i] = 0.f;
+      const float* __restrict__ Xb = a.Xt + row0 * FKC + n0;
+      const int n_tile_rows = row_end - row0 < FBM ? (int)(row_end - row0) : FBM;
+#pragma unroll
+      for (int s = 0; s < kDwXtAhead; ++s) dw.xt[s] = dw_load_xt(Xb, n_tile_rows, lane & 31, lane >> 5, s);
+    }
     FT_WAIT();
     FT_STAMP(ft_d);
     __syncthreads();
@@ -244,7 +387,12 @@
     {
       int lane_p = lane0;
       asm volatile("" : "+v"(lane_p));
-      fused_mfma_tile<NJ>(a, As, wreg, row0, row_end, n0, lane_p & 31, lane_p >> 5);
+      if constexpr (Pol::kDw) {
+        dw_mfma_tile(a.Xt + row0 * FKC + n0, row_end - row0 < FBM ? (int)(row_end - row0) : FBM, As, dw, lane_p & 31, lane_p >> 5);
+        fused_mfma_tile<NJ, true>(a, As, wreg, row0, row_end, n0, lane_p & 31, lane_p >> 5);
+      } else {
+        fused_mfma_tile<NJ>(a, As, wreg, row0, row_end, n0, lane_p & 31, lane_p >> 5);
+      }
     }
     __builtin_amdgcn_s_setprio(0);
     FT_STAMP(ft_f);
diff --git a/tm-gcn_amd/csrc/torch_ops.cpp b/tm-gcn_amd/csrc/torch_ops.cpp
--- a/tm-gcn_amd/csrc/torch_ops.cpp
+++ b/tm-gcn_amd/csrc/torch_ops.cpp
@@ -187,6 +187,34 @@
   spmm_gemm_launch(rowptr, col, val, aligned16(X), N, W, trans_w, act, Y, AX, pre, grid_reserve, avg_nnz_per_row, giant_rows,
                    giant_chunks);
   return {Y, AX, pre};
+}
+
+bool spmm_gemm_dw_supported(int64_t K, int64_t Nf, double avg_nnz_per_row, int64_t n_giant) {
+  return tmgcn_spmm_gemm_dw_supported((int32_t)K, (int32_t)Nf, (float)avg_nnz_per_row, (int32_t)n_giant) != 0;
+}
+std::tuple<Tensor, Tensor> spmm_gemm_dw(const Tensor& rowptr, const Tensor& col, const Tensor& val, const Tensor& dY, int64_t N,
+                                        const Tensor& W, const Tensor& Xt, int64_t grid_reserve, double avg_nnz_per_row,
+                                        const OptTensor& giant_rows, const OptTensor& giant_chunks) {
+  want(dY, "spmm_gemm_dw dY");
+  want(W, "spmm_gemm_dw W");
+  want(Xt, "spmm_gemm_dw Xt");
+  check_csr(rowptr, col, val, dY, N, "spmm_gemm_dw");
+  c10::DeviceGuard g(dY.device());
+  TORCH_CHECK(W.dim() == 2 && W.size(1) == dY.size(2) && Xt.dim() == 3 && Xt.size(0) == dY.size(0) && Xt.size(1) == N &&
+                  Xt.size(2) == W.size(0),
+              "spmm_gemm_dw: dY ", dY.sizes(), ", W ", W.sizes(), " and Xt ", Xt.sizes(), " do not match");
+  const Giant gi = giant_of(giant_rows, giant_chunks, dY, "spmm_gemm_dw");
+  const Tensor dYa = aligned16(dY), Wa = aligned16(W);
+  const int64_t n_rows = dY.size(0) * N;
+  const int64_t need = tmgcn_spmm_gemm_dw_workspace_bytes(n_rows, (int32_t)N);
+  Tensor ws = at::empty({need > 0 ? need : 1}, dY.options().dtype(at::kByte));
+  Tensor dX = at::empty({dY.size(0), N, W.size(0)}, dY.options()), dW = at::empty_like(W);
+  ok(tmgcn_spmm_gemm_dw_f32((const int64_t*)ptr(rowptr), (const int32_t*)ptr(col), (const float*)ptr(val), (const float*)ptr(dYa),
+                            n_rows, (int32_t)N, (int32_t)dY.size(2), (const float*)ptr(Wa), (int32_t)W.size(0),
+                            (const float*)ptr(Xt), (float*)ptr(dX), (float*)ptr(dW), (int32_t)grid_reserve, (float)avg_nnz_per_row,
+                            gi.rows, gi.chunks, gi.n, gi.m, gi.ws_ptr(), gi.ws_bytes(), ptr(ws), ws.numel(), stream_of(dY)),
+     "tmgcn_spmm_gemm_dw_f32");
+  return {dX, dW};
 }
 
 void spmm_gemm_out(const Tensor& rowptr, const Tensor& col, const Tensor& val, const Tensor& X, int64_t N,
@@ -986,10 +1014,14 @@
                         const OptTensor& g_rows, const OptTensor& g_chunks, const OptTensor& t_g_rows,
                         const OptTensor& t_g_chunks, bool need_x, bool need_w) {
     at::AutoDispatchBelowADInplaceOrView guard;
-    auto [Y, AX, pre] = spmm_gemm(rowptr, col, val, X, N, W, false, act, need_w, need_x || need_w, grid_reserve, avg, g_rows, g_chunks);
     const bool tg = need_x && t_g_rows.has_value() && t_g_chunks.has_value();
-    fused_save(ctx, "spmm_feature_gemm", W, AX, pre, t_rowptr, t_col, t_val, need_x,
+    const bool fold_dw = need_x && need_w && W.dim() == 2 && act == TMGCN_ACT_NONE &&
+                         spmm_gemm_dw_supported(W.size(1), W.size(0), avg, tg ? t_g_rows->numel() : 0);
+    auto [Y, AX, pre] = spmm_gemm(rowptr, col, val, X, N, W, false, act, need_w && !fold_dw, need_x || need_w, grid_reserve, avg,
+                                  g_rows, g_chunks);
+    fused_save(ctx, "spmm_feature_gemm", W, fold_dw ? X : AX, pre, t_rowptr, t_col, t_val, need_x,
                {tg ? *t_g_rows : none_like(X), tg ? *t_g_chunks : none_like(X)}, N, avg, act, grid_reserve);
+    ctx->saved_data["fold_dw"] = fold_dw;
     return Y;
   }
   static variable_list backward(AutogradContext* ctx, variable_list grads) {
@@ -1000,11 +1032,15 @@
     Tensor dY = grads[0].contiguous();
     if (act != TMGCN_ACT_NONE) dY = act_bwd(pre, dY, act);
     Tensor dX, dW;
-    if (ctx->needs_input_grad(0)) {
-      const bool tg = sv[6].numel() > 0;
-      dX = fused_dx_f32(ctx, sv, dY, tg ? OptTensor(sv[6]) : OptTensor(), tg ? OptTensor(sv[7]) : OptTensor());
+    const bool tg = ctx->needs_input_grad(0) && sv[6].numel() > 0;
+    if (ctx->saved_data["fold_dw"].toBool()) {
+      std::tie(dX, dW) = spmm_gemm_dw(sv[3], sv[4], sv[5], dY, ctx->saved_data["N"].toInt(), W, sv[1],
+                                      ctx->saved_data["reserve"].toInt(), ctx->saved_data["avg"].toDouble(),
+                                      tg ? OptTensor(sv[6]) : OptTensor(), tg ? OptTensor(sv[7]) : OptTensor());
+    } else {
+      if (ctx->needs_input_grad(0)) dX = fused_dx_f32(ctx, sv, dY, tg ? OptTensor(sv[6]) : OptTensor(), tg ? OptTensor(sv[7]) : OptTensor());
+      if (ctx->needs_input_grad(1)) dW = bgemm_dW(AX, dY, W.dim() == 3, TMGCN_DW_AUTO);
     }
-    if (ctx->needs_input_grad(1)) dW = bgemm_dW(AX, dY, W.dim() == 3, TMGCN_DW_AUTO);
     variable_list out(18);
     out[0] = dX;
     out[1] = dW;
@@ -1439,6 +1475,8 @@
   m.def("spmm_gemm(Tensor rowptr, Tensor col, Tensor val, Tensor X, int N, Tensor W, bool trans_w, int act, "
         "bool want_ax, bool want_pre, int grid_reserve, float avg_nnz_per_row=-1.0, Tensor? giant_rows=None, "
         "Tensor? giant_chunks=None) -> (Tensor, Tensor, Tensor)");
+  m.def("spmm_gemm_dw(Tensor rowptr, Tensor col, Tensor val, Tensor dY, int N, Tensor W, Tensor Xt, int grid_reserve, "
+        "float avg_nnz_per_row=-1.0, Tensor? giant_rows=None, Tensor? giant_chunks=None) -> (Tensor, Tensor)");
   m.def("spmm_gemm_out(Tensor rowptr, Tensor col, Tensor val, Tensor X, int N, Tensor W, bool trans_w, int act, "
         "Tensor(a!) Y, Tensor(b!)? AX, Tensor(c!)? pre, int grid_reserve, float avg_nnz_per_row=-1.0, Tensor? giant_rows=None, "
         "Tensor? giant_chunks=None) -> ()");
@@ -1463,6 +1501,7 @@
         "float weight_decay, bool nesterov, bool maximize, bool first_step) -> ()");
   m.def("head_loss_supported(int F, int C, int K) -> bool", &head_loss_supported);
   m.def("spmm_gemm_supported(int K, int Nf) -> bool", &spmm_gemm_supported);
+  m.def("spmm_gemm_dw_supported(int K, int Nf, float avg_nnz_per_row, int n_giant) -> bool", &spmm_gemm_dw_supported);
   m.def("edge_head_supported(int F, int C) -> bool", &edge_head_supported);
   m.def("abi_version() -> int", &abi_version);
   m.def("m_transform(Tensor X, Tensor M, int band_lo, int band_hi, int row_off, int col_off, int T_out, "
@@ -1540,6 +1579,7 @@
   m.impl("spmm_csr_batched", &spmm_csr_batched);
   m.impl("spmm_gemm", &spmm_gemm);
   m.impl("spmm_gemm_out", &spmm_gemm_out);
+  m.impl("spmm_gemm_dw", &spmm_gemm_dw);
   m.impl("spmm_gemm_bf16", &spmm_gemm_bf16);
   m.impl("bgemm", &bgemm);
   m.impl("bgemm_dW", &bgemm_dW);
diff --git a/tm-gcn_amd/ops.py b/tm-gcn_amd/ops.py
--- a/tm-gcn_amd/ops.py
+++ b/tm-gcn_amd/ops.py
@@ -264,6 +264,14 @@
             float(A.avg_nnz_per_row), *A.giant_plan()))
         return Y, (AX if AX.numel() else None), (pre if pre.numel() else None)
 
+    def spmm_gemm_dw_supported(self, A_T: BatchedCSR, K: int, Nf: int) -> bool:
+        rows = A_T.giant_plan()[0]
+        return bool(self.ops.spmm_gemm_dw_supported(int(K), int(Nf), float(A_T.avg_nnz_per_row), 0 if rows is None else rows.numel()))
+
+    def spmm_gemm_dw(self, A_T: BatchedCSR, dY: torch.Tensor, W: torch.Tensor, Xt: torch.Tensor, tag="spmm_gemm_T", grid_reserve=0):
+        return self._run(tag, dY.device, lambda: self.ops.spmm_gemm_dw(
+            A_T.rowptr, A_T.col, A_T.val, dY, A_T.N, W, Xt, int(grid_reserve), float(A_T.avg_nnz_per_row), *A_T.giant_plan()))
+
     def spmm_gemm_bf16_supported(self, K: int, Nf: int) -> bool:
         return bool(_lib.load().tmgcn_spmm_gemm_bf16_supported(K, Nf))
 
@@ -363,7 +371,12 @@
         ctx.A = A
         ctx.act = act if _lib.ACT_IDS[act] else None
         need_w = ctx.needs_input_grad[1]
-        Y, AX, pre = kernels.spmm_gemm(A, X, W, act=act, want_ax=need_w, want_pre=True)
+        ctx.fold_dw = bool(need_w and ctx.needs_input_grad[0] and W.dim() == 2 and ctx.act is None
+                           and hasattr(kernels, "spmm_gemm_dw")
+                           and kernels.spmm_gemm_dw_supported(A.transpose(), W.shape[1], W.shape[0]))
+        Y, AX, pre = kernels.spmm_gemm(A, X, W, act=act, want_ax=need_w and not ctx.fold_dw, want_pre=True)
+        if ctx.fold_dw:
+            AX = X
         ctx.save_for_backward(W, AX if AX is not None else torch.empty(0, device=X.device),
                               pre if pre is not None else torch.empty(0, device=X.device))
         return Y
@@ -375,6 +388,9 @@
         if ctx.act is not None:
             dY = kernels.act_bwd(pre, dY, ctx.act)
         dX = dW = None
+        if ctx.fold_dw:
+            dX, dW = kernels.spmm_gemm_dw(ctx.A.transpose(), dY, W, AX)
+            return dX, dW, None, None
         if ctx.needs_input_grad[0]:
             if kernels.spmm_gemm_supported(dY.shape[-1], W.shape[-2]):
                 dX, _, _ = kernels.spmm_gemm(ctx.A.transpose(), dY, W, trans_w=True, tag="spmm_gemm_T")
```

Result: slower. 5.536 billion (-5.4%).
